# cgisky1980/Qwen3-TTS-Rust

Measured on AMD Instinct MI355X. Metric: audio_sec_per_s, higher is better.
Workload: dtype bf16

## Files before the change

### include/q3tts.h

```cpp
#ifndef Q3TTS_H
#define Q3TTS_H

#include <stdint.h>

#ifdef __cplusplus
extern "C" {
#endif

#define Q3TTS_OK 0
#define Q3TTS_ERR_INVALID (-1)
#define Q3TTS_ERR_DEVICE (-2)
#define Q3TTS_ERR_OOM (-3)
#define Q3TTS_ERR_IO (-4)
#define Q3TTS_ERR_STATE (-5)
#define Q3TTS_ERR_UNSUPPORTED (-6)
#define Q3TTS_MAX_BATCH 256

#define Q3TTS_MAX_UPSAMPLE 4
#define Q3TTS_MAX_DEC_BLOCKS 8


typedef struct q3tts_model_config {
    int32_t t_n_layer, t_d_model, t_n_head, t_n_kv_head, t_head_dim, t_d_ffn, t_vocab;
    float t_rope_theta;
// ... 229 lines not shown
int q3tts_clone_audio_encode(q3tts_engine* e, const float* audio, int64_t n_samples, int64_t* codes, int32_t cap_frames,
                             int32_t* n_frames);
int q3tts_clone_speaker_encode(q3tts_engine* e, const float* audio, int64_t n_samples, float* spk_emb);
int q3tts_k_speaker_from_mel(q3tts_engine* e, const float* mel, int32_t n_frames, float* spk_emb);
int q3tts_k_audio_latent(q3tts_engine* e, const float* audio, int64_t n_samples, float* latent, int32_t cap_frames,
                         int32_t* n_frames);

typedef struct q3tts_tokenizer q3tts_tokenizer;
int q3tts_tokenizer_load(const char* tokenizer_json_path, q3tts_tokenizer** out, char* err, int32_t err_cap);
void q3tts_tokenizer_free(q3tts_tokenizer* t);
int32_t q3tts_tokenizer_vocab_size(const q3tts_tokenizer* t);
int q3tts_tokenizer_encode(const q3tts_tokenizer* t, const char* utf8, int64_t n_bytes, uint32_t* ids, int32_t cap,
                           int32_t* n_ids, char* err, int32_t err_cap);
int q3tts_tokenizer_decode(const q3tts_tokenizer* t, const uint32_t* ids, int32_t n, char* out, int64_t cap, int64_t* n_bytes,
                           char* err, int32_t err_cap);

int q3tts_k_gemm_exact(int32_t device, const float* x, int32_t B, int32_t K, const uint16_t* w_bf16, int32_t N,
                       const float* norm_w , float eps, const float* bias ,
                       int32_t epilogue , float* y, uint64_t* argmax_keys,
                       int32_t iters, float* mean_kernel_ms);
int q3tts_k_attention(int32_t device, const float* qkv , int32_t n_rows, int32_t pos0,
                      int32_t n_head, int32_t n_kv_head, int32_t head_dim, const float* q_norm_w, const float* k_norm_w,
                      float eps, float rope_theta, const int32_t* mrope_sections, float* out );
int q3tts_k_attention_decode(int32_t device, const float* qkv, int32_t n_slots, const int32_t* lens, int32_t n_ctx, int32_t n_head,
                             int32_t n_kv_head, int32_t head_dim, const float* q_norm_w, const float* k_norm_w, float eps, float rope_theta,
                             const int32_t* mrope_sections, int32_t policy, float* out_f32, uint16_t* out_bf16);
int q3tts_k_attention_runs(int32_t device, const float* qkv, int32_t n_runs, const int32_t* run_n, const int32_t* run_pos0, int32_t n_ctx,
                           int32_t n_head, int32_t n_kv_head, int32_t head_dim, const float* q_norm_w, const float* k_norm_w, float eps,
                           float rope_theta, const int32_t* mrope_sections, int32_t policy, int32_t out_form, void* out, float* out_scale,
                           uint16_t* k_cache, uint16_t* v_cache);
int q3tts_k_attention_decode_ex(int32_t device, const float* qkv, int32_t n_slots, const int32_t* lens, int32_t n_ctx, int32_t n_head,
                                int32_t n_kv_head, int32_t head_dim, const float* q_norm_w, const float* k_norm_w, float eps,
                                float rope_theta, const int32_t* mrope_sections, int32_t policy, int32_t row_indexed, int32_t out_form,
                                void* out, float* out_scale, uint16_t* k_cache, uint16_t* v_cache);
int q3tts_k_attention_pair(int32_t device, const float* qkv, int32_t n_slots, int32_t n_ctx, int32_t n_head, int32_t n_kv_head,
                           int32_t head_dim, const float* q_norm_w, const float* k_norm_w, float eps, float rope_theta,
                           const int32_t* mrope_sections, int32_t out_form, void* out, float* out_scale, uint16_t* k_cache, uint16_t* v_cache);
int q3tts_k_attend_pick(int32_t fused, int32_t gqa_ratio, int32_t n_ctx, int32_t n_seg, int32_t seg_max_n, int32_t seg_max_t,
                        int32_t n_kv_head, int32_t* kernel);
int q3tts_k_attention_runs_kv8(int32_t device, const float* qkv, int32_t n_runs, const int32_t* run_n, const int32_t* run_pos0, int32_t n_ctx,
                               int32_t n_head, int32_t n_kv_head, int32_t head_dim, const float* q_norm_w, const float* k_norm_w, float eps,
                               float rope_theta, const int32_t* mrope_sections, int32_t policy, int32_t out_form, void* out, float* out_scale,
                               int8_t* k_q, int8_t* v_q, uint16_t* k_d, uint16_t* v_d);
int q3tts_k_attention_decode_kv8(int32_t device, const float* qkv, int32_t n_slots, const int32_t* lens, int32_t n_ctx, int32_t n_head,
                                 int32_t n_kv_head, int32_t head_dim, const float* q_norm_w, const float* k_norm_w, float eps,
                                 float rope_theta, const int32_t* mrope_sections, int32_t policy, int32_t out_form, void* out,
                                 float* out_scale, int8_t* k_q, int8_t* v_q, uint16_t* k_d, uint16_t* v_d);
int q3tts_k_attend_pick_kv8(int32_t fused, int32_t gqa_ratio, int32_t n_ctx, int32_t n_seg, int32_t seg_max_n, int32_t seg_max_t,
                            int32_t n_kv_head, int32_t* kernel);
int q3tts_k_pred_table_row(q3tts_engine* e, int32_t q, int32_t code, float* out);
typedef struct q3tts_k_pred_step {
    int32_t n_rows, q, n_codebooks, n_key_parts, rows_q, d_embed, d_proj, max_steps_cap;
    const uint64_t* keys;
    const int32_t* active;
    const int32_t* n_frames;
    const float* codec_q;
    const float* pproj_q;
    const float* proj_b;
    float* fb;
    float* px;
    int32_t* codes;
} q3tts_k_pred_step;
int q3tts_k_pred_next(int32_t device, q3tts_k_pred_step* st, const float* norm_w, uint16_t* xb, float* ssp);
int q3tts_k_attention_gather(int32_t device, q3tts_k_pred_step* st, const float* table, const float* qkv, int32_t len, int32_t n_ctx,
                             int32_t n_head, int32_t n_kv_head, int32_t head_dim, const float* q_norm_w, const float* k_norm_w, float eps,
                             float rope_theta, const int32_t* mrope_sections, int32_t out_form, void* out, float* out_scale,
                             uint16_t* k_cache, uint16_t* v_cache);
int q3tts_k_sample(int32_t device, const float* logits, int32_t n, int32_t ld, int32_t limit, float temperature,
                   int32_t top_k, float top_p, const float* r_uniform, int32_t* out_ids);
int q3tts_k_talker_prefill(q3tts_engine* e, const float* embd, int32_t n_tok, float* hidden_out, float* logits_out);
int q3tts_k_talker_prefill_prefix(q3tts_engine* e, const q3tts_prefix* prefix, const float* embd, int32_t n_tok, float* hidden_out,
                                  float* logits_out);
int q3tts_k_prefix_read(const q3tts_prefix* x, void* k, void* v, int64_t cap, int64_t* bytes);
int q3tts_k_vocoder(q3tts_engine* e, const int32_t* codes, int32_t n_frames, int32_t chunk_frames, float* pcm_out,
                    int32_t* n_samples_out);
int q3tts_k_vocoder_latent(q3tts_engine* e, const int32_t* codes, int32_t n_frames, int32_t chunk_frames, float* out);
typedef struct q3tts_voc_tap {
    char name[32];
    int32_t dtype, layout, hist_rows, rows, channels, reserved;
    uint64_t offset;
} q3tts_voc_tap;
int q3tts_k_vocoder_taps(q3tts_engine* e, const int32_t* codes, int32_t n_frames, int32_t chunk_frames, int32_t tap_call, void* buf,
                         uint64_t buf_bytes, q3tts_voc_tap* recs, int32_t rec_cap, int32_t* n_recs);
int q3tts_k_vocoder_bench(q3tts_engine* e, int32_t n_slots, int32_t chunks, float* ms_per_chunk);
int q3tts_k_gguf_read(const char* path, const char* tensor, float* out, int64_t cap, int64_t* nelem, int64_t* dims4, int32_t* ggml_type);
int q3tts_k_gguf_meta(const char* path, const char* key, int32_t* value_type, int32_t* elem_type, int64_t* count, double* values,
                      int64_t values_cap, char* str, int64_t str_cap, int64_t* str_bytes);
int q3tts_k_probe(q3tts_engine* e, int32_t enable);
int q3tts_k_mfma_bf16(int32_t device, const uint16_t* a, const uint16_t* b, const float* c, float* d, int32_t n_cases, int32_t chain);
int q3tts_k_bgemm(int32_t device, const uint16_t* xb, int32_t B, int32_t K, const uint16_t* w_bf16, int32_t N, const float* ssp, int32_t ntiles,
                  int32_t d_norm, float eps, int32_t epilogue, const float* nw_next, float* y, uint16_t* yb, float* ssp_out, uint64_t* keys,
                  int32_t iters, float* mean_kernel_ms);
int q3tts_k_bgemm_policy(int32_t big);
int q3tts_k_attend_policy(int32_t decode, int32_t prefill);
int q3tts_k_pred_variant(q3tts_engine* e, int32_t force);
int q3tts_k_text_ready(int32_t n_text, int32_t closed, int32_t n_frames);
int q3tts_k_credit_ready(int64_t credit, int32_t n_frames);
int q3tts_k_request_rules(const q3tts_request* r, int32_t keep, int32_t keep_rows, char* msg, int32_t cap);
int q3tts_k_swap_arena(int64_t cap, const int64_t* ops, int32_t n, int64_t* offsets);
int q3tts_k_swap_phase_ms(const q3tts_session* s, double out[3]);
int q3tts_k_bgemm_pick(int32_t B, int32_t K, int32_t N, int32_t epilogue, int32_t w_once, int32_t q8, int32_t* out5);
int q3tts_k_bgemm_q8(int32_t device, const uint16_t* xb, int32_t B, int32_t K, const int8_t* q, const uint16_t* d_f16, int32_t N, const float* ssp,
                     int32_t ntiles, int32_t d_norm, float eps, int32_t epilogue, const float* nw_next, float* y, uint16_t* yb, float* ssp_out,
                     uint64_t* keys, int32_t iters, float* mean_kernel_ms);
int q3tts_k_bgemm_q8a8(int32_t device, const int8_t* aq, const float* ad, int32_t B, int32_t K, const int8_t* q, const uint16_t* d_f16, int32_t N,
                       const float* ssp, int32_t ntiles, int32_t d_norm, float eps, int32_t epilogue, const float* nw_next, float* y, int8_t* yq,
                       float* yd, float* ssp_out, int32_t iters, float* mean_kernel_ms);
int q3tts_k_bgemm_q8a8_argmax(int32_t device, const int8_t* aq, const float* ad, int32_t B, int32_t K, const int8_t* q, const uint16_t* d_f16, int32_t N,
                              const float* ssp, int32_t ntiles, int32_t d_norm, float eps, int32_t* ids_out);
int q3tts_k_bgemm_voc(int32_t device, const uint16_t* xb, int32_t B, int32_t K, const uint16_t* w_bf16, int32_t N, int32_t epilogue, const float* bias,
                      int32_t bias_n, const float* col_scale, int32_t seg_rows, int32_t gap_rows, float* y, uint16_t* yb, int32_t want_yb);
int q3tts_k_project(int32_t device, const float* x, int32_t rows, int32_t n_in, const float* w, const float* bias, int32_t n_out, const float* nw,
                    float* y, uint16_t* xb, float* ssp);
int q3tts_k_norm_inputs(int32_t device, const float* x, int32_t rows, int32_t d, const float* nw, uint16_t* xb, float* ssp);
int q3tts_k_alloc_upload(q3tts_engine* e, int64_t bytes, int64_t* mismatches);
int q3tts_k_pcm_pack(int32_t device, const float* src, int32_t rows, int64_t stride, const int32_t* ent_row, const int32_t* ent_first,
                     const int32_t* ent_count, const int64_t* ent_dst, int32_t n_ent, int32_t format, void* out, int64_t out_n);
int q3tts_k_resample_table(int32_t rate_in, int32_t rate_out, int32_t* L, int32_t* M, int32_t* H, float* tab, int64_t cap, int64_t* n);
int q3tts_k_pcm_resample(int32_t device, const float* src, int32_t rows, int64_t stride, const int32_t* row_len, const int32_t* row_final,
                         const int32_t* ent_row, const int32_t* ent_first, const int32_t* ent_count, const int64_t* ent_dst, int32_t n_ent,
                         int32_t rate_in, int32_t rate_out, int32_t format, void* out, int64_t out_n, int32_t iters, float* mean_ms);
int q3tts_k_tempo_counts(int64_t n, int32_t permille, int64_t* N, int64_t* D);
int q3tts_k_pcm_tempo(int32_t device, const float* src, int32_t rows, int64_t stride, const int32_t* lens, int32_t n_steps, const int32_t* row_final,
                      int32_t permille, float* out, int64_t out_stride, int32_t* n_valid, int32_t* delta, int64_t delta_stride, int32_t iters, float* mean_ms);
int q3tts_k_row_buckets(int32_t max_batch, int32_t* out, int32_t cap);
int q3tts_k_bucket_steps(const q3tts_engine* e, int64_t* out, int32_t cap);
int q3tts_k_prefix_stats(const q3tts_engine* e, int64_t* out2);
int q3tts_k_engine_footprint(const q3tts_engine_config* cfg, int64_t* bytes);
int q3tts_k_device_bytes(const q3tts_engine* e, int64_t* bytes);
int q3tts_k_rng_f32(uint64_t seed, int32_t n, float* out);

#define Q3TTS_BREAK_END 0
#define Q3TTS_BREAK_HARD 1
#define Q3TTS_BREAK_CLAUSE 2
#define Q3TTS_BREAK_SENTENCE 3
#define Q3TTS_BREAK_PARAGRAPH 4
typedef struct q3tts_text_span { int64_t begin, end; int32_t kind; } q3tts_text_span;
int q3tts_text_split(const char* utf8, int64_t n_bytes, int32_t target_bytes , int32_t max_bytes ,
                     q3tts_text_span* spans, int32_t cap, int32_t* n_spans, char* err, int32_t err_cap);

typedef struct q3tts_join_opts {
    int32_t trim;
    float threshold;
    int32_t keep;
    int32_t fade;
    int32_t pause_ms[5];
} q3tts_join_opts;

typedef struct q3tts_long_segment { const uint32_t* ids; int32_t n_ids; int32_t kind; int32_t max_steps ; } q3tts_long_segment;
typedef struct q3tts_long_opts { q3tts_join_opts join; int32_t speed_permille ; int32_t output_rate ; } q3tts_long_opts;
typedef struct q3tts_long_info {
    int32_t status, n_frames, hit_eos; int64_t n_native, lo, hi;
    int64_t begin, end;
    int64_t out_begin, out_end;
} q3tts_long_info;
typedef struct q3tts_long_result { int32_t status, n_segments, n_truncated , sample_rate; int64_t n_samples; float* pcm ;
    q3tts_long_info* info; float generate_ms, join_ms, total_ms; } q3tts_long_result;
void q3tts_long_default_opts(q3tts_long_opts*);
int q3tts_generate_long(q3tts_engine* e, const q3tts_request* tmpl, const q3tts_prompt_desc* voice, const q3tts_prefix* prefix,
                        const q3tts_long_segment* segs, int32_t n_segs, const q3tts_long_opts* opts, q3tts_long_result* out);
void q3tts_long_result_free(q3tts_long_result*);
int q3tts_pcm_join(q3tts_engine* e, const float* const* clips, const int64_t* n, const int32_t* kinds, int32_t n_clips,
                   const q3tts_join_opts* opts, float* out, int64_t cap, int64_t* n_out, int64_t* edges );
int q3tts_k_pcm_edges(int32_t device, const float* src, int32_t rows, int64_t stride, const int32_t* lens, float threshold, int32_t* edges,
                      int32_t iters, float* mean_ms);
int q3tts_k_pcm_join(int32_t device, const float* src, int32_t rows, int64_t stride, const int32_t* lens, const int32_t* kinds, const int32_t* edges,
// ... 7 lines not shown
```

### qwen3-tts-rust_amd/csrc/q3_vocoder.hip

```cpp
#include <algorithm>
#include <cmath>
#include <map>
#include <set>
#include <tuple>
#include <vector>

#include "q3_engine.h"

typedef __bf16 bf16x8 __attribute__((ext_vector_type(8)));

#define VOC_MAX_NS 64
#define VOC_FCAP 4

enum { VC_CODEBOOK = 0, VC_PRE = 32, VC_TFM = 40, VC_FINAL_NORM = 60, VC_UP = 64, VC_DEC_IN = 72, VC_BLK = 80, VC_OUT = 120 };
enum { VW_W = 0, VW_B = 1, VW_IN_NORM = 2, VW_Q = 3, VW_K = 4, VW_V = 5, VW_O = 6, VW_LS_ATTN = 7, VW_POST_NORM = 8, VW_GATE = 9,
       VW_UP = 10, VW_DOWN = 11, VW_LS_MLP = 12, VW_DW_W = 13, VW_DW_B = 14, VW_LN_W = 15, VW_LN_B = 16, VW_PW1 = 17, VW_PW1_B = 18,
       VW_PW2 = 19, VW_PW2_B = 20, VW_GAMMA = 21, VW_ALPHA = 22, VW_BETA = 23, VW_W2 = 24, VW_B2 = 25, VW_ALPHA2 = 26, VW_BETA2 = 27 };
#define VTID(l, w) Q3_TID(Q3G_VOC, l, w)

struct VCall {
    int ns, nf;
    int slot[VOC_MAX_NS];
    int pos[VOC_MAX_NS];
};

struct VConv { int ntap = 1, dil = 1, cin = 0, nout = 0, bias_n = 0; uint16_t* w = nullptr; float* b = nullptr; };
struct VRows { float* p = nullptr; size_t stride = 0; int off = 0; int bf16 = 0;
               VRows as_bf16() const { return {p, stride, off, 1}; } };
struct VBuf { float* p = nullptr; float* hist = nullptr; int H = 0, C = 0, Tcap = 0; int bf16 = 0;
              size_t stride() const { return (size_t)(H + Tcap) * C; }
              VRows rows() const { return {p, stride(), H * C, bf16}; }
              static VRows flat(float* q, int T, int C) { return {q, (size_t)T * C, 0, 0}; } };

struct VLayer { float *in_norm, *post_norm, *ls_attn, *ls_mlp; VConv q, k, v, o, gate, up, down;
                uint4 *qkv_t = nullptr, *o_t = nullptr, *gu_t = nullptr, *down_t = nullptr;
                VConv qkv, gu; };
struct VUp { VConv ct, pw1, pw2; float *dw_w, *dw_b, *ln_w, *ln_b, *gamma; int r; VBuf dw_in;
             uint4 *ct_t = nullptr, *pw1_t = nullptr, *pw2_t = nullptr; };
struct VRes { float *ea, *ib, *ea2, *ib2; VConv c1, c2; VBuf c1_in; };
struct VBlk { float *ea, *ib; VConv ct; VRes res[3]; int r, cin, cout; VBuf ct_in; };

struct VLaunch {
    bool polite = false;
    bool no_ring = false, no_tap = false, no_fuse = false;
    bool out_old = false, attn_old = false;
    long tap_min = 128;
    auto tie() const { return std::tie(polite, no_ring, no_tap, tap_min, no_fuse, out_old, attn_old); }
    bool operator<(const VLaunch& o) const { return tie() < o.tie(); }
};
typedef std::tuple<int, int, VLaunch> VCallKey;
static size_t voc_lds_floor(const VLaunch& vl, size_t lds) { return vl.polite ? std::max(lds, (size_t)81 * 1024) : lds; }

struct VTapSink { uint8_t* buf = nullptr; size_t cap = 0, used = 0; q3tts_voc_tap* recs = nullptr; int rec_cap = 0, n = 0; bool overflow = false; };

struct Q3Voc {
    q3tts_vocoder_config c;
    VTapSink* taps = nullptr;
    int spf = 1, B = 0, RW = 0;
    std::vector<float*> cb; const float** cb_dev = nullptr;
    VConv pre; VBuf pre_in;
    std::vector<VLayer> L; float* final_norm = nullptr;
    std::vector<VUp> U;
    VConv dec_in; VBuf dec_in_in;
    std::vector<VBlk> Bk;
    float *oea = nullptr, *oib = nullptr, *out_w = nullptr, *out_b = nullptr; VBuf out_in; int out_c = 0;
    float *kring = nullptr, *vring = nullptr;
    float* rope = nullptr; int rope_rows = 0;
    struct ZeroEnt { char* base; unsigned long long bytes; };
    ZeroEnt* zero_tab = nullptr; int n_zero = 0;
    bool tfm_bg = false;
    bool up_bg = false; uint16_t* upb = nullptr;
    float *x = nullptr, *xn = nullptr, *xnb = nullptr, *qkv = nullptr, *att = nullptr, *g = nullptr;
    float *t1 = nullptr, *t2 = nullptr;
    float* pcm = nullptr; size_t pcm_stride = 0;
    std::vector<int> frames_done, last_flag;
    VCall* call_dev = nullptr;
    VCall* call_host = nullptr; hipEvent_t call_ev[16] = {}; unsigned call_i = 0;
    std::map<VCallKey, hipGraphExec_t> call_graphs;
    std::set<VCallKey> call_seen;
    std::vector<void*> allocs;
};

enum VEpi { VEPI_STORE = 0, VEPI_SCALE_ADD = 1, VEPI_ADD = 2, VEPI_GELU = 3, VEPI_SWIGLU = 4 };
struct VGemm {
    const float* x; size_t x_stride; int x_off;
    int T, M;
    VConv c;
    float* y; size_t y_stride; int y_off;
    const float* scale;
    int scale_n;
    int epi;
    int store;
    int a_bf16;
    int y_bf16;
    float* y2; size_t y2_stride; int y2_off;
    const float *ea, *ib; int snake_n;
    int y2_bf16;
    int chunked;
};
__device__ __forceinline__ void vstep(const VGemm& g, int step, int kpt, int& tap, int& k0) {
    if (g.chunked) { const int ch = step / g.c.ntap; tap = step - ch * g.c.ntap; k0 = ch << 5; }
    else { tap = step / kpt; k0 = (step - tap * kpt) << 5; }
}

__device__ __forceinline__ float gelu_erf(float x) { return 0.5f * x * (1.0f + erff(x * 0.70710678118654752f)); }

__device__ __forceinline__ void vepi(const VGemm& g, float v, int s, int t, int n, float yold) {
    const int nout = g.c.nout;
    if (g.c.b) v += g.c.b[n % g.c.bias_n];
    float* yp = g.y + (size_t)s * g.y_stride + g.y_off + (size_t)t * nout + n;
    if (g.epi == 1) v = yold + g.scale[n % g.scale_n] * v;
    else if (g.epi == 2) v = yold + v;
    else if (g.epi == 3) v = gelu_erf(v);
    if (g.store) *yp = v;
    if (g.y2) {
        const int c = n % g.snake_n;
        const float sn = __sinf(v * g.ea[c]);
        const float sv = v + g.ib[c] * (sn * sn);
        const size_t o2 = (size_t)s * g.y2_stride + g.y2_off + (size_t)t * nout + n;
        if (g.y2_bf16) ((__bf16*)g.y2)[o2] = (__bf16)sv; else g.y2[o2] = sv;
    }
}

#define VS_PF 8
template <int NJ, bool ABF>
__global__ __launch_bounds__(256) void k_vgemm_small(VGemm g) {
    const int wave = threadIdx.x >> 6, lane = threadIdx.x & 63;
    const int m0 = blockIdx.y * 64 + wave * 16, n0 = blockIdx.x * (NJ * 16);
    if (m0 >= g.M) return;
    const int lr = lane & 15, kq = lane >> 4;
    const int cin = g.c.cin, nout = g.c.nout, kpt = cin >> 5, steps = g.c.ntap * kpt;
    const float* xrow; const uint16_t* xrow16;
    {
        int m = m0 + lr; if (m >= g.M) m = g.M - 1;
        const int s = m / g.T, t = m - s * g.T;
        const size_t eo = (size_t)s * g.x_stride + g.x_off + (size_t)t * cin + kq * 8;
        xrow = g.x + eo; xrow16 = (const uint16_t*)g.x + eo;
    }
    const uint16_t* wrow[NJ];
#pragma unroll
    for (int j = 0; j < NJ; ++j) { int n = n0 + j * 16 + lr; if (n >= nout) n = nout - 1; wrow[j] = g.c.w + (size_t)n * cin + kq * 8; }
    float4 ra[VS_PF][ABF ? 1 : 2]; uint4 rb[VS_PF][NJ];
    f32x4 acc[NJ];
#pragma unroll
    for (int j = 0; j < NJ; ++j) acc[j] = (f32x4){0.f, 0.f, 0.f, 0.f};
#define VS_ISSUE(slot_, step_)                                                                        \
    do {                                                                                              \
        const int st__ = min((step_), steps - 1);                                                     \
        int tap__, k0__; vstep(g, st__, kpt, tap__, k0__);                                            \
        const long sh__ = (long)(g.c.ntap - 1 - tap__) * g.c.dil * cin - k0__;                          \
        if (ABF) ra[slot_][0] = *(const float4*)(xrow16 - sh__);                                      \
        else { ra[slot_][0] = *(const float4*)(xrow - sh__); ra[slot_][ABF ? 0 : 1] = *(const float4*)(xrow - sh__ + 4); } \
        const size_t wo__ = (size_t)tap__ * nout * cin + k0__;                                        \
        _Pragma("unroll") for (int jj__ = 0; jj__ < NJ; ++jj__) rb[slot_][jj__] = *(const uint4*)(wrow[jj__] + wo__); \
    } while (0)
#pragma unroll
    for (int j = 0; j < VS_PF; ++j) VS_ISSUE(j, j);
    __builtin_amdgcn_sched_barrier(0);
    for (int s0 = 0; s0 < steps; s0 += VS_PF) {
#pragma unroll
        for (int j = 0; j < VS_PF; ++j) {
            const int step = s0 + j;
            const float live = step < steps ? 1.0f : 0.0f;
            bf16x8 a;
            if (ABF) {
                float4 v0 = ra[j][0];
                if (step >= steps) v0 = make_float4(0.f, 0.f, 0.f, 0.f);
                a = *(const bf16x8*)&v0;
            } else {
                const float4 v0 = ra[j][0], v1 = ra[j][ABF ? 0 : 1];
                a[0] = (__bf16)(v0.x * live); a[1] = (__bf16)(v0.y * live); a[2] = (__bf16)(v0.z * live); a[3] = (__bf16)(v0.w * live);
                a[4] = (__bf16)(v1.x * live); a[5] = (__bf16)(v1.y * live); a[6] = (__bf16)(v1.z * live); a[7] = (__bf16)(v1.w * live);
            }
            bf16x8 bfr[NJ];
#pragma unroll
            for (int jj = 0; jj < NJ; ++jj) { const uint4 u = rb[j][jj]; bfr[jj] = *(const bf16x8*)&u; }
            __builtin_amdgcn_sched_barrier(0);
            VS_ISSUE(j, step + VS_PF);
            __builtin_amdgcn_sched_barrier(0);
#pragma unroll
            for (int jj = 0; jj < NJ; ++jj) acc[jj] = __builtin_amdgcn_mfma_f32_16x16x32_bf16(a, bfr[jj], acc[jj], 0, 0, 0);
        }
    }
#undef VS_ISSUE
#pragma unroll
    for (int e = 0; e < 4; ++e) {
        const int m = m0 + 4 * kq + e;
        if (m >= g.M) continue;
        const int s = m / g.T, t = m - s * g.T;
        if (NJ == 2 && g.epi == 4) {
            const int n = blockIdx.x * 16 + lr;
            if (n0 + 16 + lr < nout) {
                const float gt = acc[0][e], up = acc[NJ - 1][e];
                const float sv = (gt / (1.0f + expf(-gt))) * up;
                const size_t yo = (size_t)s * g.y_stride + g.y_off + (size_t)t * (nout >> 1) + n;
                if (g.y_bf16) ((__bf16*)g.y)[yo] = (__bf16)sv; else g.y[yo] = sv;
            }
        } else {
#pragma unroll
            for (int j = 0; j < NJ; ++j) {
                const int n = n0 + j * 16 + lr;
// ... 78 lines not shown
    __syncthreads();
    for (int step = 0; step < steps; step += 2) {
        sstore(R0, 1);
        gload(R0, step + 3);
        VT_COMPUTE(0);
        Q3_LDS_BARRIER();
        sstore(R1, 0);
        gload(R1, step + 4);
        VT_COMPUTE(1);
        Q3_LDS_BARRIER();
    }
    const bool rmw = g.epi == 1 || g.epi == 2;
#pragma unroll
    for (int i = 0; i < 4; ++i) {
        float yv[4][NJ];
        if (rmw) {
#pragma unroll
            for (int e = 0; e < 4; ++e) {
                const int m = min(m0 + wm * 64 + i * 16 + 4 * kq + e, g.M - 1);
                const int s = m / g.T, t = m - s * g.T;
                const float* yp = g.y + (size_t)s * g.y_stride + g.y_off + (size_t)t * nout;
#pragma unroll
                for (int j = 0; j < NJ; ++j) yv[e][j] = yp[min(n0 + wn * NJ * 16 + j * 16 + lr, nout - 1)];
            }
        }
#pragma unroll
        for (int e = 0; e < 4; ++e) {
            const int m = m0 + wm * 64 + i * 16 + 4 * kq + e;
            if (m >= g.M) continue;
            const int s = m / g.T, t = m - s * g.T;
#pragma unroll
            for (int j = 0; j < NJ; ++j) {
                const int n = n0 + wn * NJ * 16 + j * 16 + lr;
                if (n < nout) vepi(g, acc[i][j][e], s, t, n, rmw ? yv[e][j] : 0.0f);
            }
        }
    }
}

template <int BN, int ROWS, int NTHR, bool LITE>
__device__ __forceinline__ void vepi_tile(const VGemm& g, const float* Ot, const int* rinfo, int n0) {
    constexpr int LDO = BN + 4, C4 = BN / 4, RPP = NTHR / C4, PER = (ROWS + RPP - 1) / RPP, PB = 8;
    const int tid = threadIdx.x, cg = tid % C4, r0 = tid / C4, nout = g.c.nout, n = n0 + cg * 4;
    const bool act = r0 < RPP && n < nout;
    const int epi = g.epi;
    const bool rmw = epi == 2 || (!LITE && epi == 1), has_b = g.c.b != nullptr, has_y2 = g.y2 != nullptr;
    float b4[4], sc4[4], ea4[4], ib4[4];
    {
        const int nc = min(n, nout - 4);
        auto base = [&](int P) { return P >= nout ? nc : nc % P; };
        auto at = [&](const float* p, int P, int b0, int q) { return (P & 3) == 0 ? p[b0 + q] : p[(nc + q) % P]; };
        const int bb = has_b ? base(g.c.bias_n) : 0, bs = (!LITE && epi == 1) ? base(g.scale_n) : 0, bk = has_y2 ? base(g.snake_n) : 0;
#pragma unroll
        for (int q = 0; q < 4; ++q) {
            b4[q] = has_b ? at(g.c.b, g.c.bias_n, bb, q) : 0.0f;
            sc4[q] = (!LITE && epi == 1) ? at(g.scale, g.scale_n, bs, q) : 1.0f;
            ea4[q] = has_y2 ? at(g.ea, g.snake_n, bk, q) : 0.0f;
            ib4[q] = has_y2 ? at(g.ib, g.snake_n, bk, q) : 0.0f;
        }
    }
    const float* ybase = g.y + g.y_off + n;
    for (int u0 = 0; u0 < PER; u0 += PB) {
        float4 yo[PB]; int info[PB];
#pragma unroll
        for (int u = 0; u < PB; ++u) {
            const int row = r0 + (u0 + u) * RPP;
            info[u] = (act && u0 + u < PER && row < ROWS) ? rinfo[row] : -1;
            if (rmw && info[u] >= 0) yo[u] = *(const float4*)(ybase + (size_t)(info[u] >> 20) * g.y_stride + (size_t)(info[u] & 0xFFFFF) * nout);
        }
#pragma unroll
        for (int u = 0; u < PB; ++u) {
            if (info[u] < 0) continue;
            const int row = r0 + (u0 + u) * RPP, sl = info[u] >> 20, t = info[u] & 0xFFFFF;
            const float4 a4 = *(const float4*)&Ot[(size_t)row * LDO + cg * 4];
            float v[4] = {a4.x, a4.y, a4.z, a4.w};
            const float yv[4] = {rmw ? yo[u].x : 0.f, rmw ? yo[u].y : 0.f, rmw ? yo[u].z : 0.f, rmw ? yo[u].w : 0.f};
            float sv[4];
#pragma unroll
            for (int q = 0; q < 4; ++q) {
                if (has_b) v[q] += b4[q];
                if (!LITE && epi == 1) v[q] = yv[q] + sc4[q] * v[q];
                else if (epi == 2) v[q] = yv[q] + v[q];
                else if (!LITE && epi == 3) v[q] = gelu_erf(v[q]);
                if (has_y2) {
                    const float sn = __sinf(v[q] * ea4[q]);
                    sv[q] = v[q] + ib4[q] * (sn * sn);
                }
            }
            if (g.store) *(float4*)(g.y + g.y_off + n + (size_t)sl * g.y_stride + (size_t)t * nout) = make_float4(v[0], v[1], v[2], v[3]);
            if (has_y2) {
                const size_t o2 = (size_t)sl * g.y2_stride + g.y2_off + (size_t)t * nout + n;
                if (g.y2_bf16) {
                    __bf16 hh[4] = {(__bf16)sv[0], (__bf16)sv[1], (__bf16)sv[2], (__bf16)sv[3]};
                    *(uint2*)((__bf16*)g.y2 + o2) = *(const uint2*)hh;
                } else *(float4*)(g.y2 + o2) = make_float4(sv[0], sv[1], sv[2], sv[3]);
            }
        }
    }
}

#ifdef Q3_VOC_STAMPS
__device__ unsigned long long g_ring_stamps[4][8];
#define VG_STAMP(i_) do { if (NJ == 3 && vg_wg >= 0 && threadIdx.x == 0) g_ring_stamps[vg_wg][i_] = __builtin_amdgcn_s_memrealtime(); } while (0)
#else
#define VG_STAMP(i_) do { } while (0)
#endif
template <int NJ, int VR_NS>
__global__ __launch_bounds__(256) void k_vgemm_ring(VGemm g) {
#ifdef Q3_VOC_STAMPS
    const int vg_wg = blockIdx.x == 1 && blockIdx.y == 100 ? 0 : (blockIdx.x == 0 && blockIdx.y == 700 ? 1 : (blockIdx.x == 2 && blockIdx.y == 1200 ? 2 : -1));
#endif
    VG_STAMP(0);
    constexpr int BN = NJ * 32, LA = 2, LB = (BN / 16 + 3) / 4, L = LA + LB;
    constexpr int STAGE = (128 + BN) * 64;
    extern __shared__ __attribute__((aligned(16))) char ring[];
    const int tid = threadIdx.x, wave = tid >> 6, lane = tid & 63;
    const int wm = wave >> 1, wn = wave & 1, lr = lane & 15, kq = lane >> 4;
    int bx = blockIdx.x, by = blockIdx.y;
    {
        const int total = gridDim.x * gridDim.y;
        if ((total & 7) == 0) {
            const int id = blockIdx.x + gridDim.x * blockIdx.y, t = (id & 7) * (total >> 3) + (id >> 3);
            bx = t % gridDim.x; by = t / gridDim.x;
        }
    }
    const int m0 = by * 128, n0 = bx * BN;
    const int cin = g.c.cin, nout = g.c.nout, kpt = cin >> 5, steps = g.c.ntap * kpt;
    const int lrow = lane >> 2;
    const uint16_t* arow[LA]; int achunk[LA];
#pragma unroll
    for (int i = 0; i < LA; ++i) {
        const int row = (wave * LA + i) * 16 + lrow;
        int m = m0 + row; if (m >= g.M) m = g.M - 1;
        const int s = m / g.T, t = m - s * g.T;
        achunk[i] = ((lane & 3) ^ VR_SW(row)) * 8;
        arow[i] = (const uint16_t*)g.x + (size_t)s * g.x_stride + g.x_off + (size_t)t * cin + achunk[i];
    }
    const uint16_t* brow[LB]; int bgrp[LB];
#pragma unroll
    for (int i = 0; i < LB; ++i) {
        bgrp[i] = min(wave * LB + i, BN / 16 - 1);
        const int row = bgrp[i] * 16 + lrow;
        int n = n0 + row; if (n >= nout) n = nout - 1;
        brow[i] = g.c.w + (size_t)n * cin + ((lane & 3) ^ VR_SW(row)) * 8;
    }
    auto issue = [&](int step) {
        int tap, k0; vstep(g, step, kpt, tap, k0);
        const long sh = (long)(g.c.ntap - 1 - tap) * g.c.dil * cin - k0;
        char* st = ring + (size_t)(step % VR_NS) * STAGE;
#pragma unroll
        for (int i = 0; i < LA; ++i)
            __builtin_amdgcn_global_load_lds((const __attribute__((address_space(1))) void*)(arow[i] - sh),
                                             (__attribute__((address_space(3))) void*)(st + (wave * LA + i) * 1024), 16, 0, 0);
        const size_t wo = (size_t)tap * nout * cin + k0;
#pragma unroll
        for (int i = 0; i < LB; ++i)
            __builtin_amdgcn_global_load_lds((const __attribute__((address_space(1))) void*)(brow[i] + wo),
                                             (__attribute__((address_space(3))) void*)(st + 128 * 64 + bgrp[i] * 1024), 16, 0, 0);
    };
    f32x4 acc[4][NJ];
#pragma unroll
    for (int i = 0; i < 4; ++i)
#pragma unroll
        for (int j = 0; j < NJ; ++j) acc[i][j] = (f32x4){0.f, 0.f, 0.f, 0.f};
    int aoff[4], boff[NJ];
#pragma unroll
    for (int i = 0; i < 4; ++i) { const int R = wm * 64 + i * 16 + lr; aoff[i] = R * 64 + ((kq ^ VR_SW(R)) << 4); }
#pragma unroll
    for (int j = 0; j < NJ; ++j) { const int R = wn * NJ * 16 + j * 16 + lr; boff[j] = 128 * 64 + R * 64 + ((kq ^ VR_SW(R)) << 4); }
#pragma unroll
// ... 105 lines not shown
        const int st = min(step, steps - 1), ch = st / NTAP, tap = st - ch * NTAP;
#pragma unroll
        for (int h = 0; h < BP; ++h)
            __builtin_amdgcn_global_load_lds((const __attribute__((address_space(1))) void*)(bp[h] + (size_t)tap * nout * cin + ch * 32),
                                             (__attribute__((address_space(3))) void*)(Bring + (step % NS) * (BN * 64) + (wave * BP + h) * 16 * 64), 16, 0, 0);
    };
    f32x4 acc[4][4];
#pragma unroll
    for (int i = 0; i < 4; ++i)
#pragma unroll
        for (int j = 0; j < 4; ++j) acc[i][j] = (f32x4){0.f, 0.f, 0.f, 0.f};
    const int arow0 = sub * RA + wm * 64 + lr;
    int boff[4];
#pragma unroll
    for (int j = 0; j < 4; ++j) { const int R = wn * 64 + j * 16 + lr; boff[j] = R * 64 + ((kq ^ ((R >> 1) & 3)) << 4); }
    issue_a(0);
#pragma unroll
    for (int p = 0; p < LA; ++p) { issue_b(2 * p); issue_b(2 * p + 1); }
    for (int c0 = 0; c0 < nchunk; c0 += 2) {
#pragma unroll
        for (int j = 0; j < 7; ++j) {
            if (j == 0) vc_waitcnt<vc_wait(0, LA, BP)>();
            else if (j == 1) vc_waitcnt<vc_wait(1, LA, BP)>();
            else if (j == 2) vc_waitcnt<vc_wait(2, LA, BP)>();
            else if (j == 3) vc_waitcnt<vc_wait(3, LA, BP)>();
            else if (j == 4) vc_waitcnt<vc_wait(4, LA, BP)>();
            else if (j == 5) vc_waitcnt<vc_wait(5, LA, BP)>();
            else vc_waitcnt<vc_wait(6, LA, BP)>();
            Q3_LDS_BARRIER();
            const int s0 = c0 * NTAP + 2 * j;
            if (j == 0) issue_a(c0 + 1);
            if (j == 4) issue_a(c0 + 2);
            issue_b(s0 + 2 * LA); issue_b(s0 + 2 * LA + 1);
#pragma unroll
            for (int h = 0; h < 2; ++h) {
                const int sl = 2 * j + h, cc = sl >= NTAP ? 1 : 0, tap = sl - cc * NTAP;
                const char* img = tlds + cc * abytes;
                const char* st = Bring + ((s0 + h) % NS) * (BN * 64);
                bf16x8 a_[4], b_[4];
#pragma unroll
                for (int i = 0; i < 4; ++i) { const int R = arow0 + i * 16 + tap * dil; a_[i] = *(const bf16x8*)(img + R * 64 + ((kq ^ ((R >> 1) & 3)) << 4)); }
#pragma unroll
                for (int jj = 0; jj < 4; ++jj) b_[jj] = *(const bf16x8*)(st + boff[jj]);
#pragma unroll
                for (int i = 0; i < 4; ++i)
#pragma unroll
                    for (int jj = 0; jj < 4; ++jj) acc[i][jj] = __builtin_amdgcn_mfma_f32_16x16x32_bf16(a_[i], b_[jj], acc[i][jj], 0, 0, 0);
            }
        }
    }
    asm volatile("s_waitcnt vmcnt(0)" ::: "memory");
    constexpr int LDO = BN + 4, ROWS = 128 * NSUB;
    float* Ot = (float*)tlds;
    __syncthreads();
#pragma unroll
    for (int i = 0; i < 4; ++i)
#pragma unroll
        for (int j = 0; j < 4; ++j)
#pragma unroll
            for (int e = 0; e < 4; ++e) Ot[(size_t)(sub * 128 + wm * 64 + i * 16 + 4 * kq + e) * LDO + wn * 64 + j * 16 + lr] = acc[i][j][e];
    int* rinfo = (int*)(Ot + ROWS * LDO);
    if (tid < ROWS) {
        const int q = by * NSUB + (tid >> 7), sl = q / tps, t = ((q - sl * tps) << 7) + (tid & 127);
        rinfo[tid] = (q < nsub && t < g.T) ? (sl << 20) | t : -1;
    }
    __syncthreads();
    if (g.epi == 0 || g.epi == 2) vepi_tile<BN, ROWS, 64 * NW, true>(g, Ot, rinfo, n0);
    else vepi_tile<BN, ROWS, 64 * NW, false>(g, Ot, rinfo, n0);
}
template <int NSUB>
static void launch_vconv_tap(const VLaunch& vl, hipStream_t s, const VGemm& g) {
    constexpr int NS = NSUB == 2 ? 12 : 8;
    const int halo = (g.c.ntap - 1) * g.c.dil, RA = (128 + halo + 15) & ~15;
    const size_t lds_main = (size_t)2 * NSUB * RA * 64 + (size_t)NS * 128 * 64, lds_out = (size_t)128 * NSUB * (128 + 4) * 4 + 128 * NSUB * 4;
    const size_t lds = voc_lds_floor(vl, std::max(lds_main, lds_out));
    static Q3PerDevice pd;
    pd.ensure(1, []() { hipFuncSetAttribute((const void*)k_vconv_tap<7, NSUB>, hipFuncAttributeMaxDynamicSharedMemorySize, 160 * 1024 - 1024); });
    const int tps = (g.T + 127) / 128, nsub = (g.M / g.T) * tps;
    hipLaunchKernelGGL((k_vconv_tap<7, NSUB>), dim3(g.c.nout / 128, (nsub + NSUB - 1) / NSUB), dim3(256 * NSUB), lds, s, g);
}

struct VResUnit {
    const float* xin; size_t xin_stride;
    int T, dil;
    const uint16_t *w1, *w2; const float *b1, *b2;
    const float *ea2, *ib2;
    float* o; size_t o_stride; int store_o;
    float* y2; size_t y2_stride; int y2_off; const float *ea3, *ib3;
};
#if defined(Q3_STAMPS) || defined(Q3_VOC_STAMPS)
__device__ unsigned long long g_voc_stamps[2][4][16];
#define VR_STAMP(i_) do { if (stamp_wg >= 0 && threadIdx.x == 0) g_voc_stamps[NT == 12 ? 0 : 1][stamp_wg][i_] = __builtin_amdgcn_s_memrealtime(); } while (0)
#else
#define VR_STAMP(i_) do { } while (0)
#endif
#define VR_BARRIER() __syncthreads()
template <int NT, int MT, int NWV>
__global__ __launch_bounds__(64 * NWV) void k_voc_resunit(VResUnit g) {
#if defined(Q3_STAMPS) || defined(Q3_VOC_STAMPS)
    const int stamp_wg = (blockIdx.y == 5 && (blockIdx.x == 3 || blockIdx.x == 20)) ? (blockIdx.x == 3 ? 0 : 1) : ((blockIdx.y == 40 && blockIdx.x == 11) ? 2 : -1);
#endif
    VR_STAMP(0);
    constexpr int C = NT * 16, KS = C / 32, R = 64 * MT, LDA = C + 16, S1 = 7 * KS, S = 8 * KS;
    constexpr int NTHR = 64 * NWV, BROWS = NTHR / 4, BPASS = (C + BROWS - 1) / BROWS;
    extern __shared__ __attribute__((aligned(16))) __bf16 lds[];
    const int halo = 6 * g.dil;
    __bf16* At = lds;
    __bf16* Zt = lds;
    __bf16* Bs = At + (size_t)(R + halo) * LDA;
    const int tid = threadIdx.x, wave = tid >> 6, lane = tid & 63, lr = lane & 15, kq = lane >> 4;
    const int sidx = blockIdx.y, t0 = blockIdx.x * R, T = g.T;
    const int bn = tid >> 2, bpart = tid & 3;
#define VR_DECL(X_) uint4 X_##0, X_##1, X_##2; X_##0 = X_##1 = X_##2 = make_uint4(0, 0, 0, 0)
    VR_DECL(ra); VR_DECL(rb); VR_DECL(rc); VR_DECL(rd);
#define VR_GLOADB(X_, step_)                                                                                            \
    do {                                                                                                                \
        const int st__ = min((step_), S - 1);                                                                           \
        const uint16_t* base__ = (st__ < S1 ? g.w1 + (size_t)(st__ / KS) * C * C + (st__ % KS) * 32 : g.w2 + (st__ - S1) * 32) + bpart * 8; \
        X_##0 = *(const uint4*)(base__ + (size_t)min(bn, C - 1) * C);                                                    \
        if (BPASS > 1) X_##1 = *(const uint4*)(base__ + (size_t)min(bn + BROWS, C - 1) * C);                                \
        if (BPASS > 2) X_##2 = *(const uint4*)(base__ + (size_t)min(bn + 2 * BROWS, C - 1) * C);                               \
    } while (0)
#define VR_SSTOREB(X_, buf_)                                                                                            \
    do {                                                                                                                \
        __bf16* d__ = &Bs[((size_t)(buf_) * C + bn) * 32 + ((bpart ^ VR_SW(bn)) << 3)];       \
        if (bn < C) *(uint4*)d__ = X_##0;                                                                               \
        if (BPASS > 1 && bn + BROWS < C) *(uint4*)(d__ + BROWS * 32) = X_##1;                                                 \
        if (BPASS > 2 && bn + 2 * BROWS < C) *(uint4*)(d__ + 2 * BROWS * 32) = X_##2;                                               \
    } while (0)
    VR_GLOADB(ra, 0);
    VR_STAMP(1);
    {
        const uint16_t* xp = (const uint16_t*)g.xin + (size_t)sidx * g.xin_stride + (size_t)t0 * C;
        const int nrow = R + halo, c8 = C / 8, total = nrow * c8;
        for (int base = tid; base < total; base += 12 * NTHR) {
            uint4 v[12];
#pragma unroll
            for (int u = 0; u < 12; ++u) {
                const int i = min(base + u * NTHR, total - 1), r = i / c8, c = (i - r * c8) * 8;
                v[u] = *(const uint4*)(xp + (size_t)min(r, T + halo - 1 - t0) * C + c);
            }
#pragma unroll
            for (int u = 0; u < 12; ++u) {
                const int i = base + u * NTHR;
                if (i < total) {
                    const int r = i / c8, c = (i - r * c8) * 8;
                    const bool live = t0 + r < T + halo;
                    *(uint4*)(At + (size_t)r * LDA + c) = live ? v[u] : make_uint4(0, 0, 0, 0);
                }
            }
        }
    }
    VR_SSTOREB(ra, 0);
    constexpr int LK = BPASS > 2 ? 3 : 4;
    VR_GLOADB(rb, 1); VR_GLOADB(rc, 2);
    if (LK == 4) { VR_GLOADB(rd, 3); VR_GLOADB(ra, 4); } else { VR_GLOADB(ra, 3); }
    __syncthreads();
    VR_STAMP(2);
    constexpr int WN = ((MT == 1 || NWV == 8) && NT >= 8) ? 2 : 1, MTW = (R / 16) / (NWV / WN), NTW = NT / WN;
    f32x4 acc[MTW][NTW];
#pragma unroll
    for (int i = 0; i < MTW; ++i)
#pragma unroll
        for (int j = 0; j < NTW; ++j) acc[i][j] = (f32x4){0.f, 0.f, 0.f, 0.f};
    const int wrow0 = (wave / WN) * MTW * 16, ncol0 = (wave % WN) * NTW * 16;
#define VR_BETWEEN()                                                                                                    \
    do {                                                                                                                \
        _Pragma("unroll") for (int i = 0; i < MTW; ++i)                                                                  \
            _Pragma("unroll") for (int j = 0; j < NTW; ++j) {                                                            \
                const int n = ncol0 + j * 16 + lr;                                                                      \
                const float bb = g.b1[n], ea = g.ea2[n], ib = g.ib2[n];                                                 \
                _Pragma("unroll") for (int e = 0; e < 4; ++e) {                                                         \
                    const float v = acc[i][j][e] + bb;                                                                  \
                    const float sn = __sinf(v * ea);                                                                    \
                    Zt[(size_t)(wrow0 + i * 16 + 4 * kq + e) * LDA + n] = (__bf16)(v + ib * (sn * sn));                 \
                    acc[i][j][e] = 0.0f;                                                                                \
                }                                                                                                       \
            }                                                                                                           \
        VR_BARRIER();                                                                                                \
    } while (0)
#define VR_STEP(step_, X_)                                                    \
    do {                                                                                                                \
        const int sp__ = (step_), buf__ = sp__ & 1, tap__ = sp__ / KS, koff__ = (sp__ - tap__ * KS) * 32;               \
        const int rowoff__ = sp__ < S1 ? tap__ * g.dil : 0;      \
        bf16x8 a__[MTW], b__[NTW];                                                                                      \
        _Pragma("unroll") for (int i = 0; i < MTW; ++i)                                                                  \
            a__[i] = *(const bf16x8*)&At[(size_t)(wrow0 + i * 16 + lr + rowoff__) * LDA + koff__ + kq * 8];             \
        _Pragma("unroll") for (int j = 0; j < NTW; ++j)                                                                  \
            b__[j] = *(const bf16x8*)&Bs[((size_t)buf__ * C + ncol0 + j * 16 + lr) * 32 + ((kq ^ VR_SW(lr)) << 3)];     \
        _Pragma("unroll") for (int i = 0; i < MTW; ++i)                                                                  \
            _Pragma("unroll") for (int j = 0; j < NTW; ++j)                                                              \
                acc[i][j] = __builtin_amdgcn_mfma_f32_16x16x32_bf16(a__[i], b__[j], acc[i][j], 0, 0, 0);                \
        VR_SSTOREB(X_, buf__ ^ 1);                                                                                      \
        VR_GLOADB(X_, sp__ + 1 + LK);                                                                                        \
        VR_BARRIER();                                                                                                \
    } while (0)
    static_assert(S % LK == 0, "the step loop is unrolled by the number of register sets");
    for (int step0 = 0; step0 < S; step0 += LK) {
#define VR_SUB(u_, X_)                                                                                                  \
        if ((S1 % LK) == (u_) && step0 + (u_) == S1) {                                                                  \
            VR_STAMP(3); VR_BETWEEN(); VR_STAMP(4);                                                                     \
        }                                                                                                               \
        VR_STEP(step0 + (u_), X_)
        if (LK == 4) { VR_SUB(0, rb); VR_SUB(1, rc); VR_SUB(2, rd); VR_SUB(3, ra); }
        else { VR_SUB(0, rb); VR_SUB(1, rc); VR_SUB(2, ra); }
    }
#undef VR_SUB
#undef VR_BETWEEN
    VR_STAMP(5);
#undef VR_STEP
#undef VR_GLOADB
#undef VR_SSTOREB
#undef VR_DECL
    constexpr int LDO = C + 4;
    float* Ot = (float*)lds;
#pragma unroll
    for (int i = 0; i < MTW; ++i)
#pragma unroll
        for (int j = 0; j < NTW; ++j) {
            const int n = ncol0 + j * 16 + lr;
            const float bb = g.b2[n];
#pragma unroll
            for (int e = 0; e < 4; ++e) Ot[(size_t)(wrow0 + i * 16 + 4 * kq + e) * LDO + n] = acc[i][j][e] + bb;
        }
    __syncthreads();
    {
        constexpr int c4n = C / 4, RPP = NTHR / c4n, PER = (R + RPP - 1) / RPP;
        float* ob = g.o + (size_t)sidx * g.o_stride;
        __bf16* yb = (__bf16*)g.y2 + (size_t)sidx * g.y2_stride + g.y2_off;
        const int cg = tid % c4n, r0 = tid / c4n, c = cg * 4;
        const bool act = r0 < RPP;
        const float4 ea = *(const float4*)(g.ea3 + c), ib = *(const float4*)(g.ib3 + c);
        constexpr int PB = PER < 13 ? PER : 13;
        for (int p0 = 0; p0 < PER; p0 += PB) {
            float4 ov[PB];
#pragma unroll
            for (int u = 0; u < PB; ++u) {
                const int row = min(r0 + (p0 + u) * RPP, R - 1);
                ov[u] = *(const float4*)(ob + (size_t)min(t0 + row, T - 1) * C + c);
            }
#pragma unroll
            for (int u = 0; u < PB; ++u) {
                const int row = r0 + (p0 + u) * RPP, t = t0 + row;
                if (!act || p0 + u >= PER || row >= R || t >= T) continue;
                const float4 a = *(const float4*)&Ot[(size_t)row * LDO + c];
                float4 v; v.x = ov[u].x + a.x; v.y = ov[u].y + a.y; v.z = ov[u].z + a.z; v.w = ov[u].w + a.w;
                if (g.store_o) *(float4*)(ob + (size_t)t * C + c) = v;
                float sn; __bf16 h[4];
                sn = __sinf(v.x * ea.x); h[0] = (__bf16)(v.x + ib.x * (sn * sn));
                sn = __sinf(v.y * ea.y); h[1] = (__bf16)(v.y + ib.y * (sn * sn));
                sn = __sinf(v.z * ea.z); h[2] = (__bf16)(v.z + ib.z * (sn * sn));
                sn = __sinf(v.w * ea.w); h[3] = (__bf16)(v.w + ib.w * (sn * sn));
                *(uint2*)(yb + (size_t)t * C + c) = *(const uint2*)h;
            }
        }
    }
    VR_STAMP(6);
}

__global__ void k_voc_embed(const VCall* __restrict__ clp, const int* codes, int max_steps_cap, int ncb_model, const float* const* cb, int ncb, int cbs, int cd,
                            float* out, size_t out_stride, int out_off) {
    const VCall& cl = *clp;
    const int s = blockIdx.y, t = blockIdx.x;
    const int slot = cl.slot[s], frame = min(cl.pos[s] + t, max_steps_cap - 1);
    const int* cp = codes + ((size_t)slot * max_steps_cap + frame) * ncb_model;
    constexpr int QB = 16;
    for (int q0 = 0; q0 < ncb; q0 += QB) {
        const float* row[QB];
#pragma unroll
        for (int u = 0; u < QB; ++u) {
            const int q = min(q0 + u, ncb - 1);
            int code = cp[q];
            code = code < 0 ? 0 : (code >= cbs ? cbs - 1 : code);
            row[u] = cb[q] + (size_t)code * cd;
        }
        for (int i = threadIdx.x; i < cd; i += blockDim.x) {
            float v[QB];
#pragma unroll
            for (int u = 0; u < QB; ++u) v[u] = row[u][i];
            float* op = out + (size_t)s * out_stride + out_off + (size_t)t * cd + i;
            float acc = q0 ? *op : 0.0f;
#pragma unroll
            for (int u = 0; u < QB; ++u) if (q0 + u < ncb) acc += v[u];
            *op = acc;
        }
    }
}

__global__ void k_voc_rows_bf16(const float* src, size_t src_stride, uint16_t* dst, size_t dst_stride, int n) {
    const int s = blockIdx.y, i = (blockIdx.x * blockDim.x + threadIdx.x) * 4;
    if (i >= n) return;
    const float4 v = *(const float4*)(src + (size_t)s * src_stride + i);
    __bf16 h[4] = {(__bf16)v.x, (__bf16)v.y, (__bf16)v.z, (__bf16)v.w};
    *(uint2*)(dst + (size_t)s * dst_stride + i) = *(const uint2*)h;
}

template <class E>
__global__ void k_voc_hist(const VCall* __restrict__ clp, E* work, size_t stride, E* hist, int H, int C, int T, int save) {
    const VCall& cl = *clp;
    const int s = blockIdx.y, slot = cl.slot[s];
    const size_t n = (size_t)H * C;
    E* w = work + (size_t)s * stride + (save ? (size_t)T * C : 0);
    E* h = hist + (size_t)slot * n;
    for (size_t i = (size_t)blockIdx.x * blockDim.x + threadIdx.x; i < n; i += (size_t)gridDim.x * blockDim.x) {
        if (save) h[i] = w[i]; else w[i] = h[i];
    }
}

struct VHistTab {
    int n;
    struct Ent { char* work; char* hist; unsigned long long stride_b, block_b, tail_b; } e[24];
};
__global__ void k_voc_hist_all(const VCall* __restrict__ clp, VHistTab tab, int save) {
    const VCall& cl = *clp;
    const VHistTab::Ent z = tab.e[blockIdx.z];
    const int s = blockIdx.y, slot = cl.slot[s];
    uint32_t* w = (uint32_t*)(z.work + (size_t)s * z.stride_b + (save ? z.tail_b : 0));
    uint32_t* h = (uint32_t*)(z.hist + (size_t)slot * z.block_b);
    const size_t n = z.block_b / 4;
    for (size_t i = (size_t)blockIdx.x * blockDim.x + threadIdx.x; i < n; i += (size_t)gridDim.x * blockDim.x) {
        if (save) h[i] = w[i]; else w[i] = h[i];
    }
}

__global__ __launch_bounds__(64) void k_voc_rmsnorm(const float* x, const float* w, float eps, int d, float* y, int out_bf16) {
    const int r = blockIdx.x, lane = threadIdx.x;
    const float* xr = x + (size_t)r * d;
    float ss = 0.0f;
    for (int i0 = lane; i0 < d; i0 += 8 * 64) {
        float v[8];
#pragma unroll
        for (int u = 0; u < 8; ++u) v[u] = xr[min(i0 + u * 64, d - 1)];
#pragma unroll
        for (int u = 0; u < 8; ++u) if (i0 + u * 64 < d) ss += v[u] * v[u];
    }
#pragma unroll
    for (int m = 32; m >= 1; m >>= 1) ss += __shfl_xor(ss, m);
    const float rinv = 1.0f / sqrtf(ss / (float)d + eps);
    for (int i0 = lane; i0 < d; i0 += 8 * 64) {
        float v[8], wv[8];
#pragma unroll
        for (int u = 0; u < 8; ++u) { const int i = min(i0 + u * 64, d - 1); v[u] = xr[i]; wv[u] = w[i]; }
#pragma unroll
        for (int u = 0; u < 8; ++u)
            if (i0 + u * 64 < d) {
                const float o = (v[u] * rinv) * wv[u];
                if (out_bf16 == 2) ((__bf16*)y)[q3_atile_off(r, i0 + u * 64, d >> 5)] = (__bf16)o;
                else if (out_bf16) ((__bf16*)y)[(size_t)r * d + i0 + u * 64] = (__bf16)o;
                else y[(size_t)r * d + i0 + u * 64] = o;
            }
    }
}

__global__ __launch_bounds__(64 * VOC_FCAP) void k_voc_attn(const VCall* __restrict__ clp, const float* qkv, float* kring, float* vring, const float* rope,
                                                            int H, int hd, int RW, int W, float* att, int tiled) {
    __shared__ float sc_s[VOC_FCAP][512];
    __shared__ float qs_s[VOC_FCAP][128];
    const VCall& cl = *clp;
    const int s = blockIdx.y, h = blockIdx.x, t = threadIdx.x >> 6, lane = threadIdx.x & 63, HH = H * hd, half = hd >> 1;
    const int slot = cl.slot[s], T = cl.nf;
    float* kr = kring + (size_t)slot * RW * HH + h * hd;
    float* vr = vring + (size_t)slot * RW * HH + h * hd;
    float* sc = sc_s[t]; float* qs = qs_s[t];
    const float scale = 1.0f / sqrtf((float)hd);
    const int pos = cl.pos[s] + t, m = s * T + t;
    {
        const float* qp = qkv + (size_t)m * 3 * HH + h * hd;
        const float* kp0 = qp + HH; const float* vp = qp + 2 * HH;
        if (lane < half) {
            const float2 csn = ((const float2*)rope)[(size_t)pos * half + lane];
            const float cs = csn.x, sn = csn.y;
            float a = qp[lane], b = qp[lane + half];
            qs[lane] = a * cs - b * sn; qs[lane + half] = b * cs + a * sn;
            a = kp0[lane]; b = kp0[lane + half];
            float* kd = kr + (size_t)(pos % RW) * HH;
            kd[lane] = a * cs - b * sn; kd[lane + half] = b * cs + a * sn;
        }
        for (int i = lane; i < hd; i += 64) vr[(size_t)(pos % RW) * HH + i] = vp[i];
    }
    __syncthreads();
    const int j0 = pos - W + 1 > 0 ? pos - W + 1 : 0, nk = pos - j0 + 1;
    for (int j = lane; j < nk; j += 64) {
        const float4* kp = (const float4*)(kr + (size_t)((j0 + j) % RW) * HH);
        float a = 0.0f;
        for (int i0 = 0; i0 < hd; i0 += 64) {
            float4 kk[16];
#pragma unroll
            for (int u = 0; u < 16; ++u) kk[u] = kp[min(i0 / 4 + u, hd / 4 - 1)];
#pragma unroll
            for (int u = 0; u < 16; ++u)
                if (i0 + 4 * u < hd) {
                    const float* qp2 = qs + i0 + 4 * u;
                    a += qp2[0] * kk[u].x; a += qp2[1] * kk[u].y; a += qp2[2] * kk[u].z; a += qp2[3] * kk[u].w;
                }
// ... 197 lines not shown
#pragma unroll
                    for (int c = 0; c < 8; ++c) acc[o] = fmaf(xv[c], wr[tap][c], acc[o]);
                }
            }
        }
#pragma unroll
        for (int o = 0; o < 8; ++o) part[k * R + g * 8 + o] = acc[o];
    }
    __syncthreads();
    if (tid < R && t0 + tid < T) {
        float r = 0.0f;
        for (int kk = 0; kk < NS; ++kk) r += part[kk * R + tid];
        r += b[0];
        pcm[(size_t)slot * pcm_stride + (size_t)cl.pos[s] * spf + t0 + tid] = fminf(1.0f, fmaxf(-1.0f, r));
    }
}

template <class T>
static int valloc(q3tts_engine* e, Q3Voc* v, T** p, size_t n) {
    void* q = nullptr;
    const int rc = q3_dev_alloc_zeroed(e, &q, n * sizeof(T) + 256);
    if (rc != Q3TTS_OK) return rc;
    v->allocs.push_back(q);
    *p = (T*)q;
    return Q3TTS_OK;
}
#define VTRY(x) do { int rc__ = (x); if (rc__ != Q3TTS_OK) return rc__; } while (0)

static int gen_vec(q3tts_engine* e, Q3Voc* v, float** p, uint32_t tid, size_t n, float base, float std) {
    VTRY(valloc(e, v, p, n));
    q3_launch_fill_f32(*p, n, e->cfg.synth_seed, tid, base, std / Q3_IH4_STD, 0, e->stream);
    return Q3TTS_OK;
}
__global__ void k_fill_bf16(uint16_t* dst, size_t n, uint64_t seed, uint32_t tid, float scale) {
    for (size_t i = (size_t)blockIdx.x * blockDim.x + threadIdx.x; i < n; i += (size_t)gridDim.x * blockDim.x)
        dst[i] = q3_bf16(q3_synth(seed, tid, i, scale));
}
static int gen_conv(q3tts_engine* e, Q3Voc* v, VConv* c, int comp, int ww, int wb, int ntap, int dil, int cin, int nout, int bias_n, float gain) {
    c->ntap = ntap; c->dil = dil; c->cin = cin; c->nout = nout; c->bias_n = bias_n;
    const size_t n = (size_t)ntap * nout * cin;
    VTRY(valloc(e, v, &c->w, n));
    const float scale = (gain / sqrtf((float)(ntap * cin))) / Q3_IH4_STD;
    hipLaunchKernelGGL(k_fill_bf16, dim3((unsigned)std::min<size_t>((n + 255) / 256, 65536)), dim3(256), 0, e->stream, c->w, n,
                       e->cfg.synth_seed, VTID(comp, ww), scale);
    c->b = nullptr;
    if (bias_n) VTRY(gen_vec(e, v, &c->b, VTID(comp, wb), bias_n, 0.0f, 0.02f));
    return Q3TTS_OK;
}
static int gen_snake(q3tts_engine* e, Q3Voc* v, uint32_t ta, uint32_t tb, int C, float** ea, float** ib) {
    std::vector<float> a(C), b(C);
    const float scale = 0.1f / Q3_IH4_STD;
    for (int i = 0; i < C; ++i) {
        const float al = 0.0f + q3_synth(e->cfg.synth_seed, ta, i, scale), be = 0.0f + q3_synth(e->cfg.synth_seed, tb, i, scale);
        a[i] = (float)exp((double)al); b[i] = (float)(1.0 / (exp((double)be) + 1e-9));
    }
    VTRY(valloc(e, v, ea, (size_t)C)); VTRY(valloc(e, v, ib, (size_t)C));
    Q3_HIP(e, hipMemcpy(*ea, a.data(), (size_t)C * 4, hipMemcpyHostToDevice));
    Q3_HIP(e, hipMemcpy(*ib, b.data(), (size_t)C * 4, hipMemcpyHostToDevice));
    return Q3TTS_OK;
}
static int mk_buf(q3tts_engine* e, Q3Voc* v, VBuf* b, int H, int C, int Tcap, int bf16 = 0) {
    b->H = H; b->C = C; b->Tcap = Tcap; b->bf16 = bf16;
    VTRY(valloc(e, v, &b->p, (size_t)VOC_MAX_NS * b->stride()));
    VTRY(valloc(e, v, &b->hist, (size_t)v->B * std::max(1, H) * C));
    return Q3TTS_OK;
}

int q3_voc_samples_per_frame(const q3tts_engine* e) { return e->voc ? e->voc->spf : 0; }

int q3_voc_create(q3tts_engine* e) {
    const q3tts_vocoder_config& c = e->cfg.vocoder;
#define REQ(cond) do { if (!(cond)) return q3_set_err(e, Q3TTS_ERR_INVALID, "vocoder config check failed: " #cond); } while (0)
    REQ(c.n_codebooks >= 1 && c.n_codebooks <= 16 && c.n_codebooks <= e->cfg.model.n_codebooks);
    REQ(c.codebook_dim % 32 == 0 && c.latent_dim % 32 == 0 && c.d_ffn % 32 == 0 && (c.n_head * c.head_dim) % 32 == 0);
    REQ(c.d_ffn % 16 == 0);
    REQ(c.head_dim <= 128 && c.head_dim % 4 == 0 && c.sliding_window >= 1 && c.sliding_window + VOC_FCAP <= 512);
    REQ(c.n_upsample >= 0 && c.n_upsample <= Q3TTS_MAX_UPSAMPLE && c.n_dec_blocks >= 1 && c.n_dec_blocks <= Q3TTS_MAX_DEC_BLOCKS);
    REQ(c.pre_conv_kernel >= 1 && c.lookahead_frames >= 0);
    { int ch = c.decoder_dim; for (int b = 0; b < c.n_dec_blocks; ++b) { REQ(ch % 64 == 0); ch /= 2; } REQ(ch >= 1); }
#undef REQ
    Q3Voc* v = new Q3Voc();
    e->voc = v;
    v->c = c; v->B = e->B;
    const int d = c.latent_dim, HH = c.n_head * c.head_dim;
    v->RW = c.sliding_window + VOC_FCAP;
    v->cb.resize(c.n_codebooks);
    for (int q = 0; q < c.n_codebooks; ++q) {
        VTRY(valloc(e, v, &v->cb[q], (size_t)c.codebook_size * c.codebook_dim));
        q3_launch_fill_f32(v->cb[q], (size_t)c.codebook_size * c.codebook_dim, e->cfg.synth_seed, VTID(VC_CODEBOOK + q, VW_W), 0.0f,
                           (1.0f / sqrtf(16.0f)) / Q3_IH4_STD, 1, e->stream);
    }
    { float** cd = nullptr; VTRY(valloc(e, v, &cd, (size_t)16)); v->cb_dev = (const float**)cd;
      Q3_HIP(e, hipMemcpy((void*)cd, v->cb.data(), sizeof(float*) * c.n_codebooks, hipMemcpyHostToDevice)); }
    VTRY(gen_conv(e, v, &v->pre, VC_PRE, VW_W, VW_B, c.pre_conv_kernel, 1, c.codebook_dim, d, d, 1.0f));
    VTRY(mk_buf(e, v, &v->pre_in, c.pre_conv_kernel - 1, c.codebook_dim, VOC_FCAP));
    v->L.resize(c.n_layer);
    for (int l = 0; l < c.n_layer; ++l) {
        VLayer& y = v->L[l]; const int comp = VC_TFM + l;
        VTRY(gen_vec(e, v, &y.in_norm, VTID(comp, VW_IN_NORM), d, 1.0f, 0.05f));
        VTRY(gen_vec(e, v, &y.post_norm, VTID(comp, VW_POST_NORM), d, 1.0f, 0.05f));
        VTRY(gen_vec(e, v, &y.ls_attn, VTID(comp, VW_LS_ATTN), d, c.layer_scale_init, 0.1f * c.layer_scale_init));
        VTRY(gen_vec(e, v, &y.ls_mlp, VTID(comp, VW_LS_MLP), d, c.layer_scale_init, 0.1f * c.layer_scale_init));
        VTRY(gen_conv(e, v, &y.q, comp, VW_Q, 0, 1, 1, d, HH, 0, 1.0f)); VTRY(gen_conv(e, v, &y.k, comp, VW_K, 0, 1, 1, d, HH, 0, 1.0f));
        VTRY(gen_conv(e, v, &y.v, comp, VW_V, 0, 1, 1, d, HH, 0, 1.0f)); VTRY(gen_conv(e, v, &y.o, comp, VW_O, 0, 1, 1, HH, d, 0, 1.0f));
        VTRY(gen_conv(e, v, &y.gate, comp, VW_GATE, 0, 1, 1, d, c.d_ffn, 0, 1.0f)); VTRY(gen_conv(e, v, &y.up, comp, VW_UP, 0, 1, 1, d, c.d_ffn, 0, 1.0f));
        VTRY(gen_conv(e, v, &y.down, comp, VW_DOWN, 0, 1, 1, c.d_ffn, d, 0, 1.0f));
        y.qkv = y.q; y.qkv.nout = 3 * HH;
        VTRY(valloc(e, v, &y.qkv.w, (size_t)3 * HH * d));
        Q3_HIP(e, hipMemcpyAsync(y.qkv.w, y.q.w, (size_t)HH * d * 2, hipMemcpyDeviceToDevice, e->stream));
        Q3_HIP(e, hipMemcpyAsync(y.qkv.w + (size_t)HH * d, y.k.w, (size_t)HH * d * 2, hipMemcpyDeviceToDevice, e->stream));
        Q3_HIP(e, hipMemcpyAsync(y.qkv.w + (size_t)2 * HH * d, y.v.w, (size_t)HH * d * 2, hipMemcpyDeviceToDevice, e->stream));
        y.gu = y.gate; y.gu.nout = 2 * c.d_ffn;
        VTRY(valloc(e, v, &y.gu.w, (size_t)2 * c.d_ffn * d));
        Q3_HIP(e, hipMemcpy2DAsync(y.gu.w, (size_t)32 * d * 2, y.gate.w, (size_t)16 * d * 2, (size_t)16 * d * 2, c.d_ffn / 16, hipMemcpyDeviceToDevice, e->stream));
        Q3_HIP(e, hipMemcpy2DAsync(y.gu.w + (size_t)16 * d, (size_t)32 * d * 2, y.up.w, (size_t)16 * d * 2, (size_t)16 * d * 2, c.d_ffn / 16, hipMemcpyDeviceToDevice, e->stream));
    }
    v->tfm_bg = d % 256 == 0 && HH % 256 == 0 && c.d_ffn % 256 == 0 && (3 * HH) % 16 == 0 && c.d_ffn % 32 == 0;
    if (v->tfm_bg)
        for (int l = 0; l < c.n_layer; ++l) {
            VLayer& y = v->L[l];
            VTRY(valloc(e, v, &y.qkv_t, (size_t)3 * HH * d / 8)); VTRY(valloc(e, v, &y.o_t, (size_t)d * HH / 8));
            VTRY(valloc(e, v, &y.gu_t, (size_t)2 * c.d_ffn * d / 8)); VTRY(valloc(e, v, &y.down_t, (size_t)d * c.d_ffn / 8));
            Q3Fill f{};
            f.mode = 0; f.row0 = 0;
            f.dst = y.qkv_t; f.N = 3 * HH; f.K = d; f.rows = 3 * HH; f.src_a = y.qkv.w; q3_launch_fill_tiled(f, e->stream);
            f.dst = y.o_t; f.N = d; f.K = HH; f.rows = d; f.src_a = y.o.w; q3_launch_fill_tiled(f, e->stream);
            f.dst = y.down_t; f.N = d; f.K = c.d_ffn; f.rows = d; f.src_a = y.down.w; q3_launch_fill_tiled(f, e->stream);
            f.mode = 1; f.dst = y.gu_t; f.N = 2 * c.d_ffn; f.K = d; f.src_a = y.gate.w; f.src_b = y.up.w; q3_launch_fill_tiled(f, e->stream);
        }
    {
        v->rope_rows = e->cfg.max_steps_cap + VOC_FCAP;
        const int half = c.head_dim / 2;
        std::vector<float> tab((size_t)v->rope_rows * half * 2);
        for (int i = 0; i < half; ++i) {
            const double inv = pow((double)c.rope_theta, -2.0 * (double)i / (double)c.head_dim);
            for (int p = 0; p < v->rope_rows; ++p) {
                const double ang = (double)p * inv;
                tab[((size_t)p * half + i) * 2] = (float)cos(ang); tab[((size_t)p * half + i) * 2 + 1] = (float)sin(ang);
            }
        }
        VTRY(valloc(e, v, &v->rope, tab.size()));
        Q3_HIP(e, hipMemcpy(v->rope, tab.data(), tab.size() * 4, hipMemcpyHostToDevice));
    }
    VTRY(gen_vec(e, v, &v->final_norm, VTID(VC_FINAL_NORM, VW_W), d, 1.0f, 0.05f));
    int rows = VOC_FCAP;
    v->spf = 1;
    v->U.resize(c.n_upsample);
    for (int s = 0; s < c.n_upsample; ++s) {
        VUp& p = v->U[s]; const int comp = VC_UP + s, r = c.upsample_ratios[s]; p.r = r; v->spf *= r;
        VTRY(gen_conv(e, v, &p.ct, comp, VW_W, VW_B, 1, 1, d, r * d, d, 1.0f));
        rows *= r;
        VTRY(mk_buf(e, v, &p.dw_in, 6, d, rows));
        VTRY(gen_vec(e, v, &p.dw_w, VTID(comp, VW_DW_W), (size_t)7 * d, 0.0f, 0.3f)); VTRY(gen_vec(e, v, &p.dw_b, VTID(comp, VW_DW_B), d, 0.0f, 0.02f));
        VTRY(gen_vec(e, v, &p.ln_w, VTID(comp, VW_LN_W), d, 1.0f, 0.05f)); VTRY(gen_vec(e, v, &p.ln_b, VTID(comp, VW_LN_B), d, 0.0f, 0.02f));
        VTRY(gen_conv(e, v, &p.pw1, comp, VW_PW1, VW_PW1_B, 1, 1, d, 4 * d, 4 * d, 1.0f));
        VTRY(gen_conv(e, v, &p.pw2, comp, VW_PW2, VW_PW2_B, 1, 1, 4 * d, d, d, 1.0f));
        if (d % 256 == 0) {
            v->up_bg = true;
            VTRY(valloc(e, v, &p.ct_t, (size_t)r * d * d / 8)); VTRY(valloc(e, v, &p.pw1_t, (size_t)4 * d * d / 8)); VTRY(valloc(e, v, &p.pw2_t, (size_t)4 * d * d / 8));
            Q3Fill f{}; f.mode = 0; f.row0 = 0;
            f.dst = p.ct_t; f.N = r * d; f.K = d; f.rows = r * d; f.src_a = p.ct.w; q3_launch_fill_tiled(f, e->stream);
            f.dst = p.pw1_t; f.N = 4 * d; f.K = d; f.rows = 4 * d; f.src_a = p.pw1.w; q3_launch_fill_tiled(f, e->stream);
            f.dst = p.pw2_t; f.N = d; f.K = 4 * d; f.rows = d; f.src_a = p.pw2.w; q3_launch_fill_tiled(f, e->stream);
        }
        VTRY(gen_vec(e, v, &p.gamma, VTID(comp, VW_GAMMA), d, 0.1f, 0.01f));
    }
    VTRY(gen_conv(e, v, &v->dec_in, VC_DEC_IN, VW_W, VW_B, 7, 1, d, c.decoder_dim, c.decoder_dim, 1.0f));
    VTRY(mk_buf(e, v, &v->dec_in_in, 6, d, rows, 1));
    size_t scratch = (size_t)rows * std::max(4 * d, c.decoder_dim);
    v->Bk.resize(c.n_dec_blocks);
    int ch = c.decoder_dim;
    for (int b = 0; b < c.n_dec_blocks; ++b) {
        VBlk& k = v->Bk[b]; const int comp = VC_BLK + 4 * b, r = c.dec_rates[b]; k.r = r; k.cin = ch; k.cout = ch / 2; v->spf *= r;
        VTRY(gen_snake(e, v, VTID(comp, VW_ALPHA), VTID(comp, VW_BETA), ch, &k.ea, &k.ib));
        VTRY(gen_conv(e, v, &k.ct, comp, VW_W, VW_B, 2, 1, ch, r * k.cout, k.cout, 1.0f));
        VTRY(mk_buf(e, v, &k.ct_in, 1, ch, rows, 1));
        rows *= r;
        scratch = std::max(scratch, (size_t)rows * k.cout);
        const int dil[3] = {1, 3, 9};
        for (int u = 0; u < 3; ++u) {
            VRes& s = k.res[u]; const int rc = comp + 1 + u;
            VTRY(gen_snake(e, v, VTID(rc, VW_ALPHA), VTID(rc, VW_BETA), k.cout, &s.ea, &s.ib));
            VTRY(gen_conv(e, v, &s.c1, rc, VW_W, VW_B, 7, dil[u], k.cout, k.cout, k.cout, 0.5f));
            VTRY(mk_buf(e, v, &s.c1_in, 6 * dil[u], k.cout, rows, 1));
            VTRY(gen_snake(e, v, VTID(rc, VW_ALPHA2), VTID(rc, VW_BETA2), k.cout, &s.ea2, &s.ib2));
            VTRY(gen_conv(e, v, &s.c2, rc, VW_W2, VW_B2, 1, 1, k.cout, k.cout, k.cout, 0.5f));
        }
        ch = k.cout;
    }
    v->out_c = ch;
    VTRY(gen_snake(e, v, VTID(VC_OUT, VW_ALPHA), VTID(VC_OUT, VW_BETA), ch, &v->oea, &v->oib));
    VTRY(valloc(e, v, &v->out_w, (size_t)7 * ch)); VTRY(gen_vec(e, v, &v->out_b, VTID(VC_OUT, VW_B), 1, 0.0f, 0.02f));
    q3_launch_fill_f32(v->out_w, (size_t)7 * ch, e->cfg.synth_seed, VTID(VC_OUT, VW_W), 0.0f, (0.1f / sqrtf((float)(7 * ch))) / Q3_IH4_STD, 1, e->stream);
    VTRY(mk_buf(e, v, &v->out_in, 6, ch, rows, 1));
    const size_t M = (size_t)VOC_MAX_NS * VOC_FCAP;
    VTRY(valloc(e, v, &v->x, M * d)); VTRY(valloc(e, v, &v->xn, M * d)); VTRY(valloc(e, v, &v->xnb, M * d)); VTRY(valloc(e, v, &v->qkv, M * 3 * HH));
    VTRY(valloc(e, v, &v->att, M * HH)); VTRY(valloc(e, v, &v->g, M * c.d_ffn));
    VTRY(valloc(e, v, &v->kring, (size_t)c.n_layer * v->B * v->RW * HH)); VTRY(valloc(e, v, &v->vring, (size_t)c.n_layer * v->B * v->RW * HH));
    VTRY(valloc(e, v, &v->t1, (size_t)VOC_MAX_NS * scratch)); VTRY(valloc(e, v, &v->t2, (size_t)VOC_MAX_NS * scratch));
    if (v->up_bg) { size_t rows_up = (size_t)VOC_MAX_NS * VOC_FCAP; for (auto& u : v->U) rows_up *= u.r; VTRY(valloc(e, v, &v->upb, rows_up * d)); }
    v->pcm_stride = (size_t)(e->cfg.max_steps_cap + VOC_FCAP) * v->spf;
    VTRY(valloc(e, v, &v->pcm, (size_t)v->B * v->pcm_stride));
    v->frames_done.assign(v->B, 0); v->last_flag.assign(v->B, 0);
    VTRY(valloc(e, v, &v->call_dev, 1));
    Q3_HIP(e, hipHostMalloc((void**)&v->call_host, 16 * sizeof(VCall)));
    Q3_HIP(e, hipStreamSynchronize(e->stream));
    return Q3TTS_OK;
}

void q3_voc_destroy(q3tts_engine* e) {
    Q3Voc* v = e->voc;
    if (!v) return;
    for (auto& kv : v->call_graphs) hipGraphExecDestroy(kv.second);
    for (auto& ev : v->call_ev) if (ev) hipEventDestroy(ev);
    if (v->call_host) hipHostFree(v->call_host);
    for (void* p : v->allocs) hipFree(p);
    delete v;
    e->voc = nullptr;
}

static std::vector<Q3SlotBlock> voc_hist_blocks(const Q3Voc* v) {
    std::vector<Q3SlotBlock> tab;
    auto add = [&](const VBuf& b) { if (b.H > 0) { const unsigned long long n = (unsigned long long)b.H * b.C * (b.bf16 ? 2 : 4); tab.push_back({(char*)b.hist, n, n}); } };
    add(v->pre_in);
    for (auto& u : v->U) add(u.dw_in);
    add(v->dec_in_in);
    for (auto& b : v->Bk) { add(b.ct_in); for (auto& r : b.res) add(r.c1_in); }
    add(v->out_in);
    return tab;
}
void q3_voc_slot_blocks(q3tts_engine* e, std::vector<Q3SlotBlock>& out) {
    const Q3Voc* v = e->voc;
    out = voc_hist_blocks(v);
    const unsigned long long ring = (unsigned long long)v->RW * v->c.n_head * v->c.head_dim * 4;
    for (int l = 0; l < v->c.n_layer; ++l)
        for (float* r : {v->kring, v->vring}) out.push_back({(char*)r + (unsigned long long)l * v->B * ring, ring, ring});
}
void q3_voc_host_state(q3tts_engine* e, int slot, int* frames_done, int* last_flag, bool set) {
    Q3Voc* v = e->voc;
    if (set) { v->frames_done[slot] = *frames_done; v->last_flag[slot] = *last_flag; }
    else { *frames_done = v->frames_done[slot]; *last_flag = v->last_flag[slot]; }
}

__global__ void k_voc_zero(const Q3Voc::ZeroEnt* tab, int slot) {
    const Q3Voc::ZeroEnt z = tab[blockIdx.x];
    uint32_t* p = (uint32_t*)(z.base + (size_t)slot * z.bytes);
    const size_t n = z.bytes / 4;
    for (size_t i = (size_t)blockIdx.y * blockDim.x + threadIdx.x; i < n; i += (size_t)gridDim.y * blockDim.x) p[i] = 0u;
}
int q3_voc_reset(q3tts_engine* e, int slot) {
    Q3Voc* v = e->voc;
    if (!v) return Q3TTS_OK;
    if (!v->zero_tab) {
        std::vector<Q3Voc::ZeroEnt> tab;
        for (const Q3SlotBlock& h : voc_hist_blocks(v)) tab.push_back({h.base, h.bytes});
        v->n_zero = (int)tab.size();
        VTRY(valloc(e, v, &v->zero_tab, tab.size()));
        Q3_HIP(e, hipMemcpy(v->zero_tab, tab.data(), tab.size() * sizeof(Q3Voc::ZeroEnt), hipMemcpyHostToDevice));
    }
    if (v->n_zero) hipLaunchKernelGGL(k_voc_zero, dim3(v->n_zero, 4), dim3(256), 0, e->stream, v->zero_tab, slot);
    v->frames_done[slot] = 0; v->last_flag[slot] = 0;
    q3_tempo_forget(e, slot);
    return Q3TTS_OK;
}

struct VSnake { VRows to; const float* ea = nullptr; const float* ib = nullptr; int n = 1; };
static VSnake snake_into(const VBuf& dst, const float* ea, const float* ib, int C) { return {dst.rows(), ea, ib, C}; }
struct VOpt {
    const float* scale = nullptr; int scale_n = 1;
    VSnake snake;
    int store = 1;
    VOpt& layer_scale(const float* v, int n) { scale = v; scale_n = n; return *this; }
    VOpt& snake_to(const VSnake& k) { snake = k; return *this; }
    VOpt& no_store() { store = 0; return *this; }
};
static bool vconv_chunked(const VConv& c) { return c.ntap == 7 && c.cin % 64 == 0 && c.cin >= 256; }
static bool voc_ring_ok(const VLaunch& vl, const VGemm& g) { return !vl.no_ring && g.c.nout % 4 == 0 && g.y_off % 4 == 0 && g.y_stride % 4 == 0 && g.y2_off % 4 == 0 && g.y2_stride % 4 == 0; }
template <int NJ>
static void launch_vgemm_small(hipStream_t s, const VGemm& g) {
    const dim3 grid((g.c.nout + 16 * NJ - 1) / (16 * NJ), (g.M + 63) / 64);
    if (g.a_bf16) hipLaunchKernelGGL((k_vgemm_small<NJ, true>), grid, dim3(256), 0, s, g);
    else hipLaunchKernelGGL((k_vgemm_small<NJ, false>), grid, dim3(256), 0, s, g);
}
template <int NJ>
static void launch_vgemm_tile(const VLaunch& vl, hipStream_t s, const VGemm& g) {
    const dim3 grid((g.c.nout + 32 * NJ - 1) / (32 * NJ), (g.M + 127) / 128);
    if (g.a_bf16 && voc_ring_ok(vl, g)) launch_vgemm_ring<NJ>(vl, s, g, grid);
    else if (g.a_bf16) hipLaunchKernelGGL((k_vgemm_lds<NJ, true>), grid, dim3(256), 0, s, g);
    else hipLaunchKernelGGL((k_vgemm_lds<NJ, false>), grid, dim3(256), 0, s, g);
}
static void vgemm(const VLaunch& vl, hipStream_t s, const VConv& c, const VRows& x, int ns, int T, const VRows& y, VEpi epi = VEPI_STORE, const VOpt& o = VOpt()) {
    VGemm g; g.x = x.p; g.x_stride = x.stride; g.x_off = x.off; g.T = T; g.M = ns * T; g.c = c; g.y = y.p; g.y_stride = y.stride; g.y_off = y.off;
    g.scale = o.scale; g.scale_n = o.scale_n; g.epi = epi; g.store = o.store; g.a_bf16 = x.bf16; g.y_bf16 = y.bf16;
    g.y2 = o.snake.to.p; g.y2_stride = o.snake.to.stride; g.y2_off = o.snake.to.off; g.ea = o.snake.ea; g.ib = o.snake.ib; g.snake_n = o.snake.n; g.y2_bf16 = o.snake.to.bf16;
    g.chunked = vconv_chunked(c) ? 1 : 0;
    const long tap_wgs = (long)(c.nout / 128) * ((ns * ((T + 127) / 128) + 1) / 2);
    if (g.chunked && g.a_bf16 && !vl.no_tap && voc_ring_ok(vl, g) && c.nout % 128 == 0 && 6 * c.dil <= 64 && epi != VEPI_SWIGLU &&
        ((T + 127) / 128) * 128 * 3 <= T * 4 &&
        tap_wgs >= vl.tap_min) {
        if (vl.polite) launch_vconv_tap<1>(vl, s, g); else launch_vconv_tap<2>(vl, s, g);
    } else if (g.M <= 512 || epi == VEPI_SWIGLU) {
        const long wg32 = (long)((c.nout + 31) / 32) * ((g.M + 63) / 64);
        if (epi != VEPI_SWIGLU && wg32 < 256) launch_vgemm_small<1>(s, g); else launch_vgemm_small<2>(s, g);
    } else if (c.nout % 128 != 0 && c.nout % 96 == 0) launch_vgemm_tile<3>(vl, s, g);
    else if (c.nout % 64 == 0 && (long)((c.nout + 127) / 128) * ((g.M + 127) / 128) < 192) launch_vgemm_tile<2>(vl, s, g);
    else launch_vgemm_tile<4>(vl, s, g);
}
static bool resunit_ok(const VLaunch& vl, int C) { return !vl.no_fuse && (C == 32 || C == 64 || C == 96 || C == 128 || C == 192); }
template <int NT, int MT, int NWV = 4>
static void launch_resunit_t(const VLaunch& vl, hipStream_t s, const VResUnit& g, int ns) {
    constexpr int C = NT * 16, R = 64 * MT, LDA = C + 16;
    const size_t lds = voc_lds_floor(vl, std::max(((size_t)(R + 6 * g.dil) * LDA + (size_t)2 * C * 32) * 2, (size_t)R * (C + 4) * 4));
    static Q3PerDevice pd;
    pd.ensure(1, []() { hipFuncSetAttribute((const void*)k_voc_resunit<NT, MT, NWV>, hipFuncAttributeMaxDynamicSharedMemorySize, 160 * 1024 - 1024); });
    hipLaunchKernelGGL((k_voc_resunit<NT, MT, NWV>), dim3((g.T + R - 1) / R, ns), dim3(64 * NWV), lds, s, g);
}
static void launch_resunit(const VLaunch& vl, hipStream_t s, const VRes& r, int ns, int T, int C, float* o, int store_o, const VSnake& sk) {
    VResUnit g;
    g.xin = r.c1_in.p; g.xin_stride = r.c1_in.stride(); g.T = T; g.dil = r.c1.dil;
    g.w1 = r.c1.w; g.w2 = r.c2.w; g.b1 = r.c1.b; g.b2 = r.c2.b; g.ea2 = r.ea2; g.ib2 = r.ib2;
    g.o = o; g.o_stride = (size_t)T * C; g.store_o = store_o;
    g.y2 = sk.to.p; g.y2_stride = sk.to.stride; g.y2_off = sk.to.off; g.ea3 = sk.ea; g.ib3 = sk.ib;
    switch (C) {
        case 32: launch_resunit_t<2, 4>(vl, s, g, ns); break;
        case 64: launch_resunit_t<4, 3>(vl, s, g, ns); break;
        case 96: launch_resunit_t<6, 2>(vl, s, g, ns); break;
        case 128: launch_resunit_t<8, 1>(vl, s, g, ns); break;
        default: if (vl.polite) launch_resunit_t<12, 1>(vl, s, g, ns); else launch_resunit_t<12, 2, 8>(vl, s, g, ns); break;
    }
}
static void hist(hipStream_t s, const VCall& cl, const VCall* cld, VBuf& b, int T, int save) {
    if (b.H == 0) return;
    const size_t n = (size_t)b.H * b.C;
    const dim3 grid((unsigned)std::min<size_t>((n + 255) / 256, 64), cl.ns);
    if (b.bf16) hipLaunchKernelGGL((k_voc_hist<uint16_t>), grid, dim3(256), 0, s, cld, (uint16_t*)b.p, b.stride(), (uint16_t*)b.hist, b.H, b.C, T, save);
    else hipLaunchKernelGGL((k_voc_hist<float>), grid, dim3(256), 0, s, cld, b.p, b.stride(), b.hist, b.H, b.C, T, save);
}
static void hist_all(hipStream_t s, const VCall& cl, const VCall* cld, Q3Voc* v, int nf, int save) {
    VHistTab tab; tab.n = 0;
    auto add = [&](const VBuf& b, int T, bool with_save) {
        if (b.H == 0 || (save && !with_save) || tab.n >= 24) return;
        const size_t es = b.bf16 ? 2 : 4;
        tab.e[tab.n++] = {(char*)b.p, (char*)b.hist, (unsigned long long)(b.stride() * es), (unsigned long long)((size_t)b.H * b.C * es), (unsigned long long)((size_t)T * b.C * es)};
    };
    int T = nf;
    add(v->pre_in, T, true);
    for (auto& p : v->U) { T *= p.r; add(p.dw_in, T, false); }
    add(v->dec_in_in, T, true);
    for (auto& k : v->Bk) { add(k.ct_in, T, true); T *= k.r; for (auto& r : k.res) add(r.c1_in, T, true); }
    add(v->out_in, T, true);
    if (tab.n) hipLaunchKernelGGL(k_voc_hist_all, dim3(16, cl.ns, tab.n), dim3(256), 0, s, cld, tab, save);
}
static void voc_launch_attn(const VLaunch& vl, hipStream_t s, const VCall* cld, Q3Voc* v, float* kr, float* vr, int ns, int nf, int tiled) {
    const q3tts_vocoder_config& c = v->c;
    const size_t lds = (size_t)(c.sliding_window + nf - 1) * (2 * c.head_dim + 1) * sizeof(float);
    if (!vl.attn_old && c.head_dim <= 64 && c.head_dim % 4 == 0 && lds <= 48 * 1024) {
        hipLaunchKernelGGL(k_voc_attn_lds, dim3(c.n_head, ns), dim3(64 * nf), lds, s, cld, v->qkv, kr, vr, v->rope, c.n_head, c.head_dim, v->RW, c.sliding_window, v->att, tiled);
        return;
    }
    hipLaunchKernelGGL(k_voc_attn, dim3(c.n_head, ns), dim3(64 * nf), 0, s, cld, v->qkv, kr, vr, v->rope, c.n_head, c.head_dim, v->RW, c.sliding_window, v->att, tiled);
}
enum VTapKind { VT_F32, VT_BF16, VT_BF16_TILED };
static void vtap_rows(Q3Voc* v, hipStream_t s, const void* p, VTapKind kind, int H, int T, int C, const char* fmt, int a, int b) {
    VTapSink* k = v->taps;
    if (!k || k->overflow) return;
    const int dtype = kind != VT_F32, layout = kind == VT_BF16_TILED;
    const size_t rows = layout ? (size_t)((H + T + 15) / 16) * 16 : (size_t)(H + T), bytes = rows * C * (dtype ? 2 : 4);
    if (k->n >= k->rec_cap || k->used + bytes > k->cap) { k->overflow = true; return; }
    q3tts_voc_tap& r = k->recs[k->n++];
    memset(&r, 0, sizeof(r));
    snprintf(r.name, sizeof(r.name), fmt, a, b);
    r.dtype = dtype; r.layout = layout; r.hist_rows = H; r.rows = T; r.channels = C; r.offset = k->used;
    if (hipMemcpyAsync(k->buf + k->used, p, bytes, hipMemcpyDeviceToHost, s) != hipSuccess) k->overflow = true;
    k->used += (bytes + 15) & ~(size_t)15;
}
static void vtap(Q3Voc* v, hipStream_t s, const void* p, VTapKind kind, int T, int C, const char* fmt, int a = 0, int b = 0) {
    vtap_rows(v, s, p, kind, 0, T, C, fmt, a, b);
}
static void vtap_buf(Q3Voc* v, hipStream_t s, const VBuf& b, int T, const char* fmt, int a = 0, int c = 0) {
    vtap_rows(v, s, b.p, b.bf16 ? VT_BF16 : VT_F32, b.H, T, b.C, fmt, a, c);
}
struct VBg : Q3BGemm {
    VBg(const void* a_, int rows, const uint4* w_, int K_, int N_, int epi_) : Q3BGemm{} { a = (const uint16_t*)a_; B = rows; w = w_; K = K_; N = N_; epi = epi_; }
    VBg& to(float* y_, int ldy_) { y = y_; ldy = ldy_; return *this; }
    VBg& to_slots(const VRows& r, int T, int ldy_) { y = r.p + r.off; ldy = ldy_; seg_rows = T; seg_stride = r.stride; return *this; }
    VBg& to_tiled(void* p) { yb = (uint16_t*)p; return *this; }
    VBg& bias_of(const VConv& c) { bias = c.b; bias_n = c.bias_n; return *this; }
    VBg& scaled(const float* cs) { col_scale = cs; return *this; }
};
static int vbgemm(q3tts_engine* e, hipStream_t s, const Q3BGemm& g, const char* msg) {
    return q3_launch_bgemm(g, s) ? q3_set_err(e, Q3TTS_ERR_INVALID, msg) : Q3TTS_OK;
}

static void voc_embed_pre(q3tts_engine* e, const VLaunch& vl, const VCall& cl, hipStream_t s) {
    Q3Voc* v = e->voc; const q3tts_vocoder_config& c = v->c;
    hipLaunchKernelGGL(k_voc_embed, dim3(cl.nf, cl.ns), dim3(128), 0, s, v->call_dev, e->codes, e->cfg.max_steps_cap, e->cfg.model.n_codebooks, v->cb_dev,
                       c.n_codebooks, c.codebook_size, c.codebook_dim, v->pre_in.p, v->pre_in.stride(), v->pre_in.H * v->pre_in.C);
    vgemm(vl, s, v->pre, v->pre_in.rows(), cl.ns, cl.nf, VBuf::flat(v->x, cl.nf, c.latent_dim));
}
static int voc_tfm_layer(q3tts_engine* e, const VLaunch& vl, const VCall& cl, hipStream_t s, int l) {
    Q3Voc* v = e->voc; const q3tts_vocoder_config& c = v->c; VLayer& L = v->L[l];
    const int d = c.latent_dim, HH = c.n_head * c.head_dim, M = cl.ns * cl.nf, one_slot = 1, tiled = v->tfm_bg ? 1 : 0;
    float* kr = v->kring + (size_t)l * v->B * v->RW * HH; float* vr = v->vring + (size_t)l * v->B * v->RW * HH;
    const VRows x = VBuf::flat(v->x, M, d), xnb = VBuf::flat(v->xnb, M, d).as_bf16(), att = VBuf::flat(v->att, M, HH).as_bf16();
    const VRows g = VBuf::flat(v->g, M, c.d_ffn).as_bf16();
    hipLaunchKernelGGL(k_voc_rmsnorm, dim3(M), dim3(64), 0, s, v->x, L.in_norm, c.rms_eps, d, v->xnb, tiled ? 2 : 1);
    if (tiled) VTRY(vbgemm(e, s, VBg(v->xnb, M, L.qkv_t, d, 3 * HH, Q3_EPI_STORE).to(v->qkv, 3 * HH), "vocoder: qkv GEMM shape"));
    else vgemm(vl, s, L.qkv, xnb, one_slot, M, VBuf::flat(v->qkv, M, 3 * HH));
    voc_launch_attn(vl, s, v->call_dev, v, kr, vr, cl.ns, cl.nf, tiled);
    if (tiled) VTRY(vbgemm(e, s, VBg(v->att, M, L.o_t, HH, d, Q3_EPI_RESID).to(v->x, d).scaled(L.ls_attn), "vocoder: o GEMM shape"));
    else vgemm(vl, s, L.o, att, one_slot, M, x, VEPI_SCALE_ADD, VOpt().layer_scale(L.ls_attn, d));
    hipLaunchKernelGGL(k_voc_rmsnorm, dim3(M), dim3(64), 0, s, v->x, L.post_norm, c.rms_eps, d, v->xnb, tiled ? 2 : 1);
    if (tiled) VTRY(vbgemm(e, s, VBg(v->xnb, M, L.gu_t, d, 2 * c.d_ffn, Q3_EPI_SWIGLU).to_tiled(v->g), "vocoder: gate/up GEMM shape"));
    else vgemm(vl, s, L.gu, xnb, one_slot, M, g, VEPI_SWIGLU);
    if (tiled) VTRY(vbgemm(e, s, VBg(v->g, M, L.down_t, c.d_ffn, d, Q3_EPI_RESID).to(v->x, d).scaled(L.ls_mlp), "vocoder: down GEMM shape"));
    else vgemm(vl, s, L.down, g, one_slot, M, x, VEPI_SCALE_ADD, VOpt().layer_scale(L.ls_mlp, d));
    return Q3TTS_OK;
}
static int voc_up_stage(q3tts_engine* e, const VLaunch& vl, const VCall& cl, hipStream_t s, size_t ui, VRows& cur, int& T) {
    Q3Voc* v = e->voc; VUp& p = v->U[ui];
    const int ns = cl.ns, d = v->c.latent_dim, i = (int)ui, bg = v->up_bg ? 1 : 0;
    const VTapKind kind = bg ? VT_BF16_TILED : VT_F32;
    const uint16_t* a_in = ui ? v->upb : (const uint16_t*)v->xnb;
    const VRows raw = p.dw_in.rows();
    vtap(v, s, bg ? (const void*)a_in : (const void*)(cur.p + cur.off), kind, T, d, "up%d.in", i);
    if (bg) VTRY(vbgemm(e, s, VBg(a_in, ns * T, p.ct_t, d, p.r * d, Q3_EPI_STORE).bias_of(p.ct).to_slots(raw, T, p.r * d), "vocoder: upsample ConvTranspose GEMM shape"));
    else vgemm(vl, s, p.ct, cur, ns, T, raw);
    T *= p.r;
    vtap_buf(v, s, p.dw_in, T, "up%d.raw", i);
    hipLaunchKernelGGL(k_voc_dw_ln, dim3(T, ns), dim3(64), (size_t)d * 4, s, p.dw_in.p, p.dw_in.stride(), p.dw_in.H, T, d, p.dw_w, p.dw_b, p.ln_w, p.ln_b, v->t1, bg);
    vtap(v, s, v->t1, kind, T, d, "up%d.ln", i);
    hist(s, cl, v->call_dev, p.dw_in, T, 1);
    if (bg) VTRY(vbgemm(e, s, VBg(v->t1, ns * T, p.pw1_t, d, 4 * d, Q3_EPI_GELU).bias_of(p.pw1).to_tiled(v->t2), "vocoder: pointwise-1 GEMM shape"));
    else vgemm(vl, s, p.pw1, VBuf::flat(v->t1, T, d), ns, T, VBuf::flat(v->t2, T, 4 * d), VEPI_GELU);
    vtap(v, s, v->t2, kind, T, 4 * d, "up%d.gelu", i);
    if (bg) {
        VBg r(v->t2, ns * T, p.pw2_t, 4 * d, d, Q3_EPI_RESID);
        r.bias_of(p.pw2).scaled(p.gamma).to_slots(raw, T, d).to_tiled(ui + 1 < v->U.size() ? v->upb : nullptr);
        VTRY(vbgemm(e, s, r, "vocoder: pointwise-2 GEMM shape"));
    } else vgemm(vl, s, p.pw2, VBuf::flat(v->t2, T, 4 * d), ns, T, raw, VEPI_SCALE_ADD, VOpt().layer_scale(p.gamma, d));
    vtap_buf(v, s, p.dw_in, T, "up%d.out", i);
    cur = raw;
    return Q3TTS_OK;
}
static VSnake snake_next(Q3Voc* v, size_t bi, int u) {
    VBlk& k = v->Bk[bi];
    if (u < 2) return snake_into(k.res[u + 1].c1_in, k.res[u + 1].ea, k.res[u + 1].ib, k.cout);
    if (bi + 1 < v->Bk.size()) { VBlk& nx = v->Bk[bi + 1]; return snake_into(nx.ct_in, nx.ea, nx.ib, k.cout); }
    return snake_into(v->out_in, v->oea, v->oib, k.cout);
}
static void voc_dec_blocks(q3tts_engine* e, const VLaunch& vl, const VCall& cl, hipStream_t s, const VRows& cur, int& T) {
    Q3Voc* v = e->voc;
    const int ns = cl.ns, d = v->c.latent_dim;
    hipLaunchKernelGGL(k_voc_rows_bf16, dim3((unsigned)(((size_t)T * d / 4 + 255) / 256), ns), dim3(256), 0, s, cur.p + cur.off, cur.stride,
                       (uint16_t*)v->dec_in_in.p + (size_t)v->dec_in_in.H * d, v->dec_in_in.stride(), T * d);
    int ch = v->c.decoder_dim;
    float* z = v->t1; float* o = v->t2;
    vgemm(vl, s, v->dec_in, v->dec_in_in.rows(), ns, T, VBuf::flat(z, T, ch), VEPI_STORE,
          VOpt().snake_to(snake_into(v->Bk[0].ct_in, v->Bk[0].ea, v->Bk[0].ib, ch)).no_store());
    for (size_t bi = 0; bi < v->Bk.size(); ++bi) {
        VBlk& k = v->Bk[bi]; const int b = (int)bi;
        vgemm(vl, s, k.ct, k.ct_in.rows(), ns, T, VBuf::flat(o, T * k.r, k.cout), VEPI_STORE, VOpt().snake_to(snake_into(k.res[0].c1_in, k.res[0].ea, k.res[0].ib, k.cout)));
        T *= k.r; ch = k.cout;
        vtap(v, s, o, VT_F32, T, ch, "b%d.o_ct", b);
        for (int u = 0; u < 3; ++u) {
            VRes& r = k.res[u];
            const VSnake next = snake_next(v, bi, u);
            const int store_o = u < 2 ? 1 : 0;
            if (resunit_ok(vl, ch)) launch_resunit(vl, s, r, ns, T, ch, o, store_o, next);
            else {
                const VRows zf = VBuf::flat(z, T, ch), zb = zf.as_bf16(), orows = VBuf::flat(o, T, ch);
                vgemm(vl, s, r.c1, r.c1_in.rows(), ns, T, zf, VEPI_STORE, VOpt().snake_to({zb, r.ea2, r.ib2, ch}).no_store());
                vtap(v, s, z, VT_BF16, T, ch, "b%d.r%d.z", b, u);
                VOpt opt; opt.snake = next; opt.store = store_o;
                vgemm(vl, s, r.c2, zb, ns, T, orows, VEPI_ADD, opt);
            }
            if (store_o) vtap(v, s, o, VT_F32, T, ch, "b%d.r%d.o", b, u);
        }
    }
}
static void voc_out(q3tts_engine* e, const VLaunch& vl, const VCall& cl, hipStream_t s, int T) {
    Q3Voc* v = e->voc; const VCall* cld = v->call_dev;
    const int ns = cl.ns, ch = v->out_c;
    if (ch % 8 == 0 && ch / 8 <= 32 && !vl.out_old) {
        const int NS = ch / 8, G = std::min(16, 256 / NS), R = G * 8;
        static Q3PerDevice pd8;
        pd8.ensure(1, []() { hipFuncSetAttribute((const void*)k_voc_out8, hipFuncAttributeMaxDynamicSharedMemorySize, 96 * 1024); });
        hipLaunchKernelGGL(k_voc_out8, dim3((T + R - 1) / R, ns), dim3(256), (size_t)(R + 6) * (ch * 2 + 16) + (size_t)NS * R * 4, s,   cld, (const uint16_t*)v->out_in.p,
                           v->out_in.stride(), v->out_in.H, T, ch, v->out_w, v->out_b, v->pcm, v->pcm_stride, v->spf, G);
    } else
        hipLaunchKernelGGL(k_voc_out, dim3((T + 63) / 64, ns), dim3(256), (size_t)(70 * (ch + 1) + 7 * ch) * 4, s, cld, v->out_in.p, v->out_in.stride(), v->out_in.H, T, ch, v->out_w, v->out_b,
                           v->pcm, v->pcm_stride, v->spf);
}
static int voc_call_body(q3tts_engine* e, const VLaunch& vl, const VCall& cl, hipStream_t s) {
    Q3Voc* v = e->voc;
    const q3tts_vocoder_config& c = v->c;
    const int nf = cl.nf, d = c.latent_dim, M = cl.ns * nf;
    hist_all(s, cl, v->call_dev, v, nf, 0);
    voc_embed_pre(e, vl, cl, s);
    for (int l = 0; l < c.n_layer; ++l) VTRY(voc_tfm_layer(e, vl, cl, s, l));
    hipLaunchKernelGGL(k_voc_rmsnorm, dim3(M), dim3(64), 0, s, v->x, v->final_norm, c.rms_eps, d, v->up_bg ? v->xnb : v->xn, v->up_bg ? 2 : 0);
    VRows cur = VBuf::flat(v->xn, nf, d); int T = nf;
    for (size_t ui = 0; ui < v->U.size(); ++ui) VTRY(voc_up_stage(e, vl, cl, s, ui, cur, T));
    {
        static const int exp_skip = getenv("Q3TTS_EXP_VOC_SKIP") ? atoi(getenv("Q3TTS_EXP_VOC_SKIP")) : 0;
        if (exp_skip == 2) { Q3_HIP(e, hipGetLastError()); return Q3TTS_OK; }
    }
    const int Tup = T;
    voc_dec_blocks(e, vl, cl, s, cur, T);
    voc_out(e, vl, cl, s, T);
    if (v->taps) {
        int Tb = Tup;
        vtap_buf(v, s, v->dec_in_in, Tb, "dec_in.in");
        for (size_t bi = 0; bi < v->Bk.size(); ++bi) {
            VBlk& k = v->Bk[bi];
            vtap_buf(v, s, k.ct_in, Tb, "b%d.ct_in", (int)bi);
            Tb *= k.r;
            for (int u = 0; u < 3; ++u) vtap_buf(v, s, k.res[u].c1_in, Tb, "b%d.r%d.c1_in", (int)bi, u);
        }
        vtap_buf(v, s, v->out_in, Tb, "out.in");
        vtap(v, s, v->pcm + (size_t)cl.slot[0] * v->pcm_stride + (size_t)cl.pos[0] * v->spf, VT_F32, Tb, 1, "pcm");
    }
    hist_all(s, cl, v->call_dev, v, nf, 1);
    Q3_HIP(e, hipGetLastError());
    return Q3TTS_OK;
}

static int voc_call(q3tts_engine* e, const VCall& cl, hipStream_t s, bool polite_call) {
    Q3Voc* v = e->voc;
    {
        const unsigned i = v->call_i++ & 15;
        if (v->call_ev[i]) Q3_HIP(e, hipEventSynchronize(v->call_ev[i]));
        else Q3_HIP(e, hipEventCreateWithFlags(&v->call_ev[i], hipEventDisableTiming));
        v->call_host[i] = cl;
        Q3_HIP(e, hipMemcpyAsync(v->call_dev, &v->call_host[i], sizeof(VCall), hipMemcpyHostToDevice, s));
        Q3_HIP(e, hipEventRecord(v->call_ev[i], s));
    }
    VLaunch vl;
    auto on = [](const char* name) { const char* ev = getenv(name); return ev && atoi(ev); };
    const char* pol = getenv("Q3TTS_VOC_POLITE"); const char* tmin = getenv("Q3TTS_VOC_TAP_MIN");
    vl.polite = pol ? atoi(pol) != 0 : polite_call;
    vl.no_ring = on("Q3TTS_VOC_NORING"); vl.no_tap = on("Q3TTS_VOC_NOTAP"); vl.no_fuse = on("Q3TTS_VOC_NOFUSE"); vl.attn_old = on("Q3TTS_VOC_ATTN_OLD");
    vl.tap_min = tmin ? atol(tmin) : 128;
    vl.out_old = getenv("Q3TTS_VOC_OUT_OLD") != nullptr;
    static const bool no_graph = [] { const char* ev = getenv("Q3TTS_VOC_NO_GRAPH"); return ev && atoi(ev); }();
    if (no_graph || v->taps) return voc_call_body(e, vl, cl, s);
    const VCallKey key(cl.ns, cl.nf, vl);
    auto it = v->call_graphs.find(key);
    if (it == v->call_graphs.end()) {
        if (v->call_seen.insert(key).second) return voc_call_body(e, vl, cl, s);
        hipGraph_t graph = nullptr; hipGraphExec_t exec = nullptr;
        Q3_HIP(e, hipStreamBeginCapture(s, hipStreamCaptureModeThreadLocal));
        const int rc = voc_call_body(e, vl, cl, s);
        const hipError_t er = hipStreamEndCapture(s, &graph);
        if (rc != Q3TTS_OK) { if (graph) hipGraphDestroy(graph); return rc; }
        if (er != hipSuccess || !graph) return q3_set_err(e, Q3TTS_ERR_DEVICE, std::string("vocoder call capture: ") + hipGetErrorString(er));
        const hipError_t ei = hipGraphInstantiate(&exec, graph, nullptr, nullptr, 0);
        hipGraphDestroy(graph);
        if (ei != hipSuccess) return q3_set_err(e, Q3TTS_ERR_DEVICE, std::string("vocoder call graph: ") + hipGetErrorString(ei));
        it = v->call_graphs.emplace(key, exec).first;
    }
    Q3_HIP(e, hipGraphLaunch(it->second, s));
    return Q3TTS_OK;
}

int q3_voc_decode(q3tts_engine* e, int slot, int f0, int nf, int is_last, hipStream_t s) {
    Q3Voc* v = e->voc;
    if (!v) return q3_set_err(e, Q3TTS_ERR_STATE, "engine has no vocoder");
    if (f0 != v->frames_done[slot]) return q3_set_err(e, Q3TTS_ERR_STATE, "vocoder frames must be consumed in order");
    while (nf > 0) {
        const int n = std::min(nf, VOC_FCAP);
        VCall cl; memset(&cl, 0, sizeof(cl));
        cl.ns = 1; cl.nf = n; cl.slot[0] = slot; cl.pos[0] = v->frames_done[slot];
        VTRY(voc_call(e, cl, s, false));
        v->frames_done[slot] += n; nf -= n;
    }
    if (is_last) v->last_flag[slot] = 1;
    return Q3TTS_OK;
}
int q3_voc_decode_batch(q3tts_engine* e, const int* slots, const int* real, int ns, int nf, hipStream_t s, int beside_decoder) {
    Q3Voc* v = e->voc;
    if (!v) return q3_set_err(e, Q3TTS_ERR_STATE, "engine has no vocoder");
    if (ns <= 0 || ns > v->B || nf <= 0 || nf > VOC_FCAP) return q3_set_err(e, Q3TTS_ERR_INVALID, "vocoder batch shape");
    for (int g0 = 0; g0 < ns; g0 += VOC_MAX_NS) {
        const int n = std::min(ns - g0, VOC_MAX_NS);
        VCall cl; memset(&cl, 0, sizeof(cl));
        cl.ns = n; cl.nf = nf;
        for (int i = 0; i < n; ++i) { cl.slot[i] = slots[g0 + i]; cl.pos[i] = v->frames_done[slots[g0 + i]]; }
        VTRY(voc_call(e, cl, s, beside_decoder && n >= 16));
        for (int i = g0; i < g0 + n; ++i) v->frames_done[slots[i]] += real ? real[i] : nf;
    }
    return Q3TTS_OK;
}
void q3_voc_mark_last(q3tts_engine* e, int slot) { if (e->voc) e->voc->last_flag[slot] = 1; }

float* q3_voc_pcm(q3tts_engine* e, int slot) { return e->voc->pcm + (size_t)slot * e->voc->pcm_stride; }
size_t q3_voc_pcm_stride(const q3tts_engine* e) { return e->voc ? e->voc->pcm_stride : 0; }
int q3_voc_samples(q3tts_engine* e, int slot) {
    Q3Voc* v = e->voc;
    int fr = v->frames_done[slot];
    if (!v->last_flag[slot]) fr = std::max(0, fr - v->c.lookahead_frames);
    return fr * v->spf;
}

struct VDriveCall { int index, f0, n; bool last; };
static const int VOC_DRIVE_STOP = 1;
template <class Step>
static int voc_drive(q3tts_engine* e, const int32_t* codes, int n_frames, int chunk_frames, bool args_ok, Step step) {
    Q3_NOT_IN_SESSION(e);
    if (!e || !codes || !args_ok || n_frames <= 0) return q3_set_err(e, Q3TTS_ERR_INVALID, "null argument");
    if (!e->voc) return q3_set_err(e, Q3TTS_ERR_STATE, "engine created with with_vocoder = 0");
    if (n_frames > e->cfg.max_steps_cap) return q3_set_err(e, Q3TTS_ERR_INVALID, "n_frames exceeds max_steps_cap");
    Q3_HIP(e, hipSetDevice(e->cfg.device));
    hipStream_t s = e->stream;
    Q3_HIP(e, hipMemcpyAsync(e->codes, codes, sizeof(int32_t) * (size_t)n_frames * e->cfg.model.n_codebooks, hipMemcpyHostToDevice, s));
    VTRY(q3_voc_reset(e, 0));
    const int chunk = chunk_frames > 0 ? chunk_frames : n_frames;
    int rc = Q3TTS_OK; VDriveCall c = {0, 0, 0, false};
    for (int f = 0; f < n_frames && rc == Q3TTS_OK; f += chunk) {
        const int end = std::min(f + chunk, n_frames);
        for (c.f0 = f; c.f0 < end && rc == Q3TTS_OK; c.f0 += c.n, ++c.index) {
            c.n = std::min(VOC_FCAP, end - c.f0); c.last = c.f0 + c.n >= n_frames;
            rc = step(c, false);
            if (rc == Q3TTS_OK) rc = q3_voc_decode(e, 0, c.f0, c.n, c.last, s);
            if (rc == Q3TTS_OK) rc = step(c, true);
        }
    }
    const hipError_t er = hipStreamSynchronize(s);
    if (rc < 0) return rc;
    Q3_HIP(e, er);
    return rc;
}

extern "C" int q3tts_k_vocoder(q3tts_engine* e, const int32_t* codes, int32_t n_frames, int32_t chunk_frames, float* pcm_out, int32_t* n_samples_out) {
    int ns = 0;
    VTRY(voc_drive(e, codes, n_frames, chunk_frames, pcm_out && n_samples_out, [&](const VDriveCall& c, bool after) {
        if (!after || !c.last) return Q3TTS_OK;
        ns = q3_voc_samples(e, 0);
        Q3_HIP(e, hipMemcpyAsync(pcm_out, q3_voc_pcm(e, 0), sizeof(float) * (size_t)ns, hipMemcpyDeviceToHost, e->stream));
        return Q3TTS_OK;
    }));
    *n_samples_out = ns;
    return Q3TTS_OK;
}

extern "C" int q3tts_k_vocoder_latent(q3tts_engine* e, const int32_t* codes, int32_t n_frames, int32_t chunk_frames, float* out) {
    return voc_drive(e, codes, n_frames, chunk_frames, out != nullptr, [&](const VDriveCall& c, bool after) {
        const int d = e->voc->c.latent_dim;
        if (after) Q3_HIP(e, hipMemcpyAsync(out + (size_t)c.f0 * d, e->voc->x, sizeof(float) * (size_t)c.n * d, hipMemcpyDeviceToHost, e->stream));
        return Q3TTS_OK;
    });
}

extern "C" int q3tts_k_vocoder_taps(q3tts_engine* e, const int32_t* codes, int32_t n_frames, int32_t chunk_frames, int32_t tap_call, void* buf,
                                    uint64_t buf_bytes, q3tts_voc_tap* recs, int32_t rec_cap, int32_t* n_recs) {
    VTapSink sink; sink.buf = (uint8_t*)buf; sink.cap = (size_t)buf_bytes; sink.recs = recs; sink.rec_cap = rec_cap;
    bool tapped = false;
    const int rc = voc_drive(e, codes, n_frames, chunk_frames, buf && recs && n_recs && tap_call >= 0, [&](const VDriveCall& c, bool after) {
        if (c.index != tap_call) return Q3TTS_OK;
        if (!after) { e->voc->taps = &sink; tapped = true; }
        return after ? VOC_DRIVE_STOP : Q3TTS_OK;
    });
    if (tapped) e->voc->taps = nullptr;
    if (rc < 0) return rc;
    if (rc != VOC_DRIVE_STOP) return q3_set_err(e, Q3TTS_ERR_INVALID, "tap_call is past the last call of this drive");
    if (sink.overflow) return q3_set_err(e, Q3TTS_ERR_INVALID, "tap buffer or record table too small");
    *n_recs = sink.n;
    return Q3TTS_OK;
}

#if defined(Q3_STAMPS) || defined(Q3_VOC_STAMPS)
static void voc_print_stamps() {
    unsigned long long st[2][4][16];
    if (hipMemcpyFromSymbol(st, HIP_SYMBOL(g_voc_stamps), sizeof(st)) != hipSuccess) return;
    for (int k = 0; k < 2; ++k)
        for (int w = 0; w < 3; ++w)
            fprintf(stderr, "resunit stamps (%s) wg %d (100 MHz ticks from entry): first weights requested %llu | input staged + barrier %llu | conv1 done %llu | snake tile done %llu | conv2 done %llu | stores issued %llu\n",
                    k == 0 ? "192 channels" : "96 channels", w, st[k][w][1] - st[k][w][0], st[k][w][2] - st[k][w][0], st[k][w][3] - st[k][w][0], st[k][w][4] - st[k][w][0], st[k][w][5] - st[k][w][0], st[k][w][6] - st[k][w][0]);
}
#endif
extern "C" int q3tts_k_vocoder_bench(q3tts_engine* e, int32_t n_slots, int32_t chunks, float* ms_per_chunk) {
    Q3_NOT_IN_SESSION(e);
    if (!e || !ms_per_chunk || n_slots <= 0 || chunks <= 0) return q3_set_err(e, Q3TTS_ERR_INVALID, "vocoder bench: bad argument");
    if (!e->voc) return q3_set_err(e, Q3TTS_ERR_STATE, "engine created with with_vocoder = 0");
    if (n_slots > e->B || (chunks + 2) * 4 > e->cfg.max_steps_cap) return q3_set_err(e, Q3TTS_ERR_INVALID, "vocoder bench: shape exceeds the engine's");
    Q3_HIP(e, hipSetDevice(e->cfg.device));
    const int ncb = e->cfg.model.n_codebooks, cap = e->cfg.max_steps_cap, cbs = e->cfg.vocoder.codebook_size;
    hipStream_t s = e->stream;
    std::vector<int32_t> codes((size_t)n_slots * cap * ncb);
    uint64_t st = 0x9E3779B97F4A7C15ULL;
    for (auto& c : codes) { st = q3_mix64(st + 0x1234567); c = (int32_t)(st % (uint64_t)cbs); }
    Q3_HIP(e, hipMemcpyAsync(e->codes, codes.data(), codes.size() * 4, hipMemcpyHostToDevice, s));
    Q3_HIP(e, hipStreamSynchronize(s));
    std::vector<int> slots(n_slots);
    for (int i = 0; i < n_slots; ++i) { slots[i] = i; VTRY(q3_voc_reset(e, i)); }
    for (int w = 0; w < 2; ++w) VTRY(q3_voc_decode_batch(e, slots.data(), nullptr, n_slots, 4, s, 0));
    Q3_HIP(e, hipEventRecord(e->ev0, s));
    for (int c = 0; c < chunks; ++c) VTRY(q3_voc_decode_batch(e, slots.data(), nullptr, n_slots, 4, s, 0));
    Q3_HIP(e, hipEventRecord(e->ev2, s));
    Q3_HIP(e, hipStreamSynchronize(s));
    float ms = 0.0f;
    Q3_HIP(e, hipEventElapsedTime(&ms, e->ev0, e->ev2));
    *ms_per_chunk = ms / (float)chunks;
#if defined(Q3_STAMPS) || defined(Q3_VOC_STAMPS)
    voc_print_stamps();
#endif
#ifdef Q3_VOC_STAMPS
    {
        unsigned long long st[4][8];
        if (hipMemcpyFromSymbol(st, HIP_SYMBOL(g_ring_stamps), sizeof(st)) == hipSuccess)
            for (int w = 0; w < 3; ++w)
                fprintf(stderr, "ring<3> stamps wg %d (10 ns ticks from entry): prologue issued %llu | first stage in LDS %llu | main loop done %llu | tile in LDS %llu | stores issued %llu | stores done %llu\n",
                        w, st[w][1] - st[w][0], st[w][2] - st[w][0], st[w][3] - st[w][0], st[w][4] - st[w][0], st[w][5] - st[w][0], st[w][6] - st[w][0]);
    }
#endif
    for (int i = 0; i < n_slots; ++i) VTRY(q3_voc_reset(e, i));
    return Q3TTS_OK;
}
```

### qwen3-tts-rust_amd/q3tts/_abi.py

```python
import ctypes as C
import os

HERE = os.path.dirname(os.path.abspath(__file__))
PKG_ROOT = os.path.dirname(HERE)
REPO_ROOT = os.path.dirname(PKG_ROOT)
LIB_PATH = os.path.join(PKG_ROOT, "csrc", "libq3tts.so")

Q3TTS_MAX_UPSAMPLE = 4
Q3TTS_MAX_DEC_BLOCKS = 8


class ModelConfig(C.Structure):
    _fields_ = [
        ("t_n_layer", C.c_int32), ("t_d_model", C.c_int32), ("t_n_head", C.c_int32), ("t_n_kv_head", C.c_int32),
        ("t_head_dim", C.c_int32), ("t_d_ffn", C.c_int32), ("t_vocab", C.c_int32),
        ("t_rope_theta", C.c_float),
        ("t_mrope_sections", C.c_int32 * 4),
        ("p_n_layer", C.c_int32), ("p_d_model", C.c_int32), ("p_n_head", C.c_int32), ("p_n_kv_head", C.c_int32),
        ("p_head_dim", C.c_int32), ("p_d_ffn", C.c_int32),
        ("p_rope_theta", C.c_float),
        ("n_codebooks", C.c_int32), ("codebook_size", C.c_int32),
        ("rms_eps", C.c_float),
        ("d_embed", C.c_int32), ("text_vocab", C.c_int32), ("codec0_rows", C.c_int32), ("codecq_rows", C.c_int32),
        ("sample_limit", C.c_int32), ("eos_code", C.c_int32), ("tts_pad_id", C.c_int32),
    ]


class VocoderConfig(C.Structure):
    _fields_ = [
        ("n_codebooks", C.c_int32), ("codebook_size", C.c_int32), ("codebook_dim", C.c_int32),
        ("latent_dim", C.c_int32), ("pre_conv_kernel", C.c_int32),
        ("n_layer", C.c_int32), ("n_head", C.c_int32), ("head_dim", C.c_int32), ("d_ffn", C.c_int32),
        ("sliding_window", C.c_int32),
        ("rope_theta", C.c_float), ("rms_eps", C.c_float), ("layer_scale_init", C.c_float),
        ("n_upsample", C.c_int32), ("upsample_ratios", C.c_int32 * Q3TTS_MAX_UPSAMPLE),
        ("decoder_dim", C.c_int32), ("n_dec_blocks", C.c_int32), ("dec_rates", C.c_int32 * Q3TTS_MAX_DEC_BLOCKS),
        ("lookahead_frames", C.c_int32), ("sample_rate", C.c_int32),
    ]


class EngineConfig(C.Structure):
    _fields_ = [
        ("model", ModelConfig), ("vocoder", VocoderConfig),
        ("device", C.c_int32), ("max_batch", C.c_int32), ("n_ctx", C.c_int32), ("max_steps_cap", C.c_int32),
        ("with_vocoder", C.c_int32),
        ("synth_seed", C.c_uint64),
        ("weights_path", C.c_char_p),
        ("talker_q8_0", C.c_int32),
        ("vocoder_flush_tail", C.c_int32),
        ("predictor_q8_0", C.c_int32),
    ]
    _tail_fields_ = ("kv_q8_0",)

    @property
    def kv_q8_0(self):
        return C.c_int32.from_buffer(self, C.sizeof(EngineConfig) - 4).value

    @kv_q8_0.setter
    def kv_q8_0(self, v):
        C.c_int32.from_buffer(self, C.sizeof(EngineConfig) - 4).value = int(v)


assert EngineConfig.predictor_q8_0.offset + 8 == C.sizeof(EngineConfig) and C.sizeof(EngineConfig) % 8 == 0, "q3tts_engine_config: kv_q8_0 no longer sits in the tail"
ENGINE_CONFIG_FIELD_ORDER = [f[0] for f in EngineConfig._fields_] + list(EngineConfig._tail_fields_)
KV_Q8_0_OFFSET = C.sizeof(EngineConfig) - 4


class PromptDesc(C.Structure):
    _fields_ = [
        ("text_ids", C.POINTER(C.c_uint32)), ("n_text", C.c_int32),
        ("instruct_ids", C.POINTER(C.c_uint32)), ("n_instruct", C.c_int32),
        ("lang_id", C.c_int32), ("spk_id", C.c_int32),
        ("spk_emb", C.POINTER(C.c_float)),
        ("ref_codes", C.POINTER(C.c_int32)), ("n_ref_frames", C.c_int32),
        ("ref_text_ids", C.POINTER(C.c_uint32)), ("n_ref_text", C.c_int32),
    ]


class Request(C.Structure):
    _fields_ = [
        ("prompt_embd", C.POINTER(C.c_float)), ("n_tok", C.c_int32),
        ("text_stream", C.c_int32),
        ("prompt", C.POINTER(PromptDesc)),
        ("use_engine_sampler", C.c_int32),
        ("temperature", C.c_float), ("top_k", C.c_int32), ("top_p", C.c_float), ("has_seed", C.c_int32),
        ("text_open", C.c_int32),
        ("seed", C.c_uint64),
        ("max_steps", C.c_int32), ("min_frames", C.c_int32), ("force_eos_at", C.c_int32), ("want_pcm", C.c_int32),
        ("prefix", C.c_void_p),
    ]


class Result(C.Structure):
    _fields_ = [
        ("status", C.c_int32), ("n_frames", C.c_int32), ("hit_eos", C.c_int32),
        ("codes", C.POINTER(C.c_int32)), ("pcm", C.POINTER(C.c_float)),
        ("n_samples", C.c_int32), ("sample_rate", C.c_int32),
        ("first_chunk_ms", C.c_float), ("total_ms", C.c_float),
    ]


class VocTap(C.Structure):
    _fields_ = [
        ("name", C.c_char * 32), ("dtype", C.c_int32), ("layout", C.c_int32), ("hist_rows", C.c_int32), ("rows", C.c_int32),
        ("channels", C.c_int32), ("reserved", C.c_int32), ("offset", C.c_uint64),
    ]


class SessionEvent(C.Structure):
    _fields_ = [
        ("id", C.c_uint64), ("kind", C.c_int32), ("status", C.c_int32), ("pcm", C.c_void_p), ("n_samples", C.c_int32),
        ("is_final", C.c_int32), ("result", Result),
    ]


EV_NONE, EV_CHUNK, EV_DONE, EV_FAILED, EV_CANCELLED = 0, 1, 2, 3, 4
EV_PREFIX = 5
PCM_F32, PCM_I16 = 0, 1
SESSION_RING_DEPTH = 4


class Timings(C.Structure):
    _fields_ = [
        ("prefill_ms", C.c_float), ("decode_ms", C.c_float), ("vocoder_ms", C.c_float), ("total_ms", C.c_float),
        ("frame_step_ms", C.c_float), ("probe_kernel_ms", C.c_float),
        ("frame_steps", C.c_int64), ("algo_bytes_per_step", C.c_int64), ("algo_flops_per_step", C.c_int64),
        ("mean_live_slots", C.c_float), ("mean_rows", C.c_float), ("probe_count", C.c_int64), ("probe_empty_ms", C.c_float),
        ("mean_ctx_tokens", C.c_float),
    ]


class NodeTimings(C.Structure):
    _fields_ = [("generate_ms", C.c_float), ("gather_ms", C.c_float), ("total_ms", C.c_float), ("gathered_bytes", C.c_int64), ("n_devices", C.c_int32)]


class CloneConfig(C.Structure):
    _fields_ = [
        ("mel_dim", C.c_int32),
        ("se_channels", C.c_int32 * 5), ("se_kernels", C.c_int32 * 5), ("se_dilations", C.c_int32 * 5),
        ("se_attn_channels", C.c_int32), ("se_res2net_scale", C.c_int32), ("se_se_channels", C.c_int32), ("se_dim", C.c_int32),
        ("ae_filters", C.c_int32), ("ae_kernel", C.c_int32), ("ae_res_kernel", C.c_int32), ("ae_last_kernel", C.c_int32),
        ("ae_n_ratios", C.c_int32), ("ae_ratios", C.c_int32 * 4),
        ("ae_hidden", C.c_int32), ("ae_n_layer", C.c_int32), ("ae_n_head", C.c_int32), ("ae_head_dim", C.c_int32),
        ("ae_d_ffn", C.c_int32), ("ae_window", C.c_int32),
        ("ae_rope_theta", C.c_float), ("ae_ln_eps", C.c_float), ("ae_layer_scale", C.c_float),
        ("ae_down_stride", C.c_int32), ("ae_vq_dim", C.c_int32), ("ae_n_codebooks", C.c_int32), ("ae_codebook_size", C.c_int32),
    ]


SYMBOLS = [
    "q3tts_default_config", "q3tts_engine_create", "q3tts_engine_destroy", "q3tts_last_error", "q3tts_set_sampler",
    "q3tts_set_max_steps", "q3tts_build_prompt", "q3tts_free", "q3tts_generate", "q3tts_generate_batch",
    "q3tts_result_free", "q3tts_stream_begin", "q3tts_stream_poll", "q3tts_stream_end",
    "q3tts_get_timings", "q3tts_k_gemm_exact", "q3tts_k_attention", "q3tts_k_attention_decode", "q3tts_k_sample", "q3tts_k_talker_prefill",
    "q3tts_k_vocoder", "q3tts_k_vocoder_latent", "q3tts_k_vocoder_taps", "q3tts_k_vocoder_bench", "q3tts_set_device_pcm", "q3tts_get_device_pcm", "q3tts_k_rng_f32", "q3tts_k_probe", "q3tts_k_gguf_read", "q3tts_mel_frames", "q3tts_mel",
    "q3tts_clone_default_config", "q3tts_clone_init", "q3tts_clone_audio_frames", "q3tts_clone_audio_encode",
    "q3tts_clone_speaker_encode", "q3tts_k_speaker_from_mel", "q3tts_k_audio_latent",
    "q3tts_node_create", "q3tts_node_destroy", "q3tts_node_generate_batch", "q3tts_node_get_timings", "q3tts_node_last_error", "q3tts_node_size", "q3tts_node_engine", "q3tts_node_shard", "q3tts_k_bgemm_q8", "q3tts_k_bgemm_q8a8_argmax", "q3tts_k_bgemm_q8a8", "q3tts_k_alloc_upload", "q3tts_k_bgemm_policy", "q3tts_k_attend_policy", "q3tts_k_bgemm_pick", "q3tts_k_mfma_bf16", "q3tts_k_bgemm", "q3tts_k_bgemm_voc", "q3tts_k_project", "q3tts_k_norm_inputs", "q3tts_tokenizer_load", "q3tts_tokenizer_free", "q3tts_tokenizer_vocab_size", "q3tts_tokenizer_encode", "q3tts_tokenizer_decode",
    "q3tts_session_create", "q3tts_session_submit", "q3tts_session_cancel", "q3tts_session_next", "q3tts_session_close",
    "q3tts_session_last_error", "q3tts_k_pcm_pack",
    "q3tts_prefix_create", "q3tts_prefix_rows", "q3tts_prefix_destroy", "q3tts_k_talker_prefill_prefix",
    "q3tts_config_from_model_dir", "q3tts_k_gguf_meta",
    "q3tts_set_predictor_sampler", "q3tts_get_predictor_sampler", "q3tts_set_repetition_penalty", "q3tts_get_repetition_penalty",
    "q3tts_k_pred_variant",
    "q3tts_set_output_rate", "q3tts_get_output_rate", "q3tts_resample", "q3tts_k_resample_table", "q3tts_k_pcm_resample",
    "q3tts_session_append_text", "q3tts_k_text_ready",
    "q3tts_k_attention_runs", "q3tts_k_attention_decode_ex", "q3tts_k_attention_pair", "q3tts_k_attend_pick",
    "q3tts_k_attention_runs_kv8", "q3tts_k_attention_decode_kv8", "q3tts_k_attend_pick_kv8",
    "q3tts_k_pred_table_row", "q3tts_k_pred_next", "q3tts_k_attention_gather",
    "q3tts_k_row_buckets", "q3tts_k_bucket_steps", "q3tts_k_device_bytes", "q3tts_k_engine_footprint", "q3tts_k_prefix_stats",
    "q3tts_session_prefix_create", "q3tts_session_submit_keep_voice", "q3tts_session_prefix_release", "q3tts_session_clone",
    "q3tts_prefix_state", "q3tts_k_prefix_read",
    "q3tts_session_submit_paced", "q3tts_session_grant", "q3tts_session_set_swap", "q3tts_session_swap_stats",
    "q3tts_k_credit_ready", "q3tts_k_swap_arena", "q3tts_k_swap_phase_ms",
    "q3tts_k_request_rules",
    "q3tts_set_speed", "q3tts_get_speed", "q3tts_time_stretch", "q3tts_k_tempo_counts", "q3tts_k_pcm_tempo",
    "q3tts_text_split", "q3tts_long_default_opts", "q3tts_generate_long", "q3tts_long_result_free", "q3tts_pcm_join",
    "q3tts_k_pcm_edges", "q3tts_k_pcm_join",
]

BREAK_END, BREAK_HARD, BREAK_CLAUSE, BREAK_SENTENCE, BREAK_PARAGRAPH = 0, 1, 2, 3, 4
JOIN_W = 240
LONG_MAX_SEGMENTS = 1024


class TextSpan(C.Structure):
    _fields_ = [("begin", C.c_int64), ("end", C.c_int64), ("kind", C.c_int32)]


class JoinOpts(C.Structure):
    _fields_ = [("trim", C.c_int32), ("threshold", C.c_float), ("keep", C.c_int32), ("fade", C.c_int32), ("pause_ms", C.c_int32 * 5)]


class LongSegment(C.Structure):
    _fields_ = [("ids", C.POINTER(C.c_uint32)), ("n_ids", C.c_int32), ("kind", C.c_int32), ("max_steps", C.c_int32)]


class LongOpts(C.Structure):
    _fields_ = [("join", JoinOpts), ("speed_permille", C.c_int32), ("output_rate", C.c_int32)]


class LongInfo(C.Structure):
    _fields_ = [
        ("status", C.c_int32), ("n_frames", C.c_int32), ("hit_eos", C.c_int32),
        ("n_native", C.c_int64), ("lo", C.c_int64), ("hi", C.c_int64),
        ("begin", C.c_int64), ("end", C.c_int64), ("out_begin", C.c_int64), ("out_end", C.c_int64),
    ]


class LongResult(C.Structure):
    _fields_ = [
        ("status", C.c_int32), ("n_segments", C.c_int32), ("n_truncated", C.c_int32), ("sample_rate", C.c_int32),
        ("n_samples", C.c_int64), ("pcm", C.POINTER(C.c_float)), ("info", C.POINTER(LongInfo)),
        ("generate_ms", C.c_float), ("join_ms", C.c_float), ("total_ms", C.c_float),
    ]


class PredStep(C.Structure):
    _fields_ = [
        ("n_rows", C.c_int32), ("q", C.c_int32), ("n_codebooks", C.c_int32), ("n_key_parts", C.c_int32), ("rows_q", C.c_int32),
        ("d_embed", C.c_int32), ("d_proj", C.c_int32), ("max_steps_cap", C.c_int32),
        ("keys", C.c_void_p), ("active", C.c_void_p), ("n_frames", C.c_void_p), ("codec_q", C.c_void_p), ("pproj_q", C.c_void_p),
        ("proj_b", C.c_void_p), ("fb", C.c_void_p), ("px", C.c_void_p), ("codes", C.c_void_p),
    ]


class Q3Error(RuntimeError):
    pass


_lib = None


def load_library(path=None):
    global _lib
    if _lib is not None and path is None:
        return _lib
    p = path or os.environ.get("Q3TTS_LIB") or LIB_PATH
# ... 32 lines not shown
    lib.q3tts_session_close.argtypes = [vp]
    lib.q3tts_session_last_error.argtypes = [vp]
    lib.q3tts_session_last_error.restype = C.c_char_p
    lib.q3tts_session_append_text.argtypes = [vp, C.c_uint64, u32p, C.c_int32, C.c_int32]
    lib.q3tts_session_prefix_create.argtypes = [vp, C.POINTER(PromptDesc), f32p, C.c_int32, C.POINTER(vp), C.POINTER(C.c_uint64)]
    lib.q3tts_session_submit_keep_voice.argtypes = [vp, C.POINTER(Request), C.c_int32, C.POINTER(C.c_uint64), C.POINTER(vp)]
    lib.q3tts_session_prefix_release.argtypes = [vp, vp]
    lib.q3tts_session_clone.argtypes = [vp, f32p, C.c_int64, C.c_int32, C.POINTER(C.c_int64), C.c_int32, C.POINTER(C.c_int32), f32p]
    lib.q3tts_prefix_state.argtypes = [vp]
    lib.q3tts_prefix_state.restype = C.c_int32
    lib.q3tts_k_prefix_read.argtypes = [vp, vp, vp, C.c_int64, C.POINTER(C.c_int64)]
    lib.q3tts_k_text_ready.argtypes = [C.c_int32, C.c_int32, C.c_int32]
    lib.q3tts_session_submit_paced.argtypes = [vp, C.POINTER(Request), C.c_int32, C.POINTER(C.c_uint64)]
    lib.q3tts_session_grant.argtypes = [vp, C.c_uint64, C.c_int32]
    lib.q3tts_session_set_swap.argtypes = [vp, C.c_int64]
    lib.q3tts_session_swap_stats.argtypes = [vp, C.POINTER(C.c_int64)]
    lib.q3tts_k_credit_ready.argtypes = [C.c_int64, C.c_int32]
    lib.q3tts_k_request_rules.argtypes = [C.POINTER(Request), C.c_int32, C.c_int32, C.c_char_p, C.c_int32]
    lib.q3tts_k_swap_phase_ms.argtypes = [vp, C.POINTER(C.c_double)]
    lib.q3tts_k_swap_arena.argtypes = [C.c_int64, C.POINTER(C.c_int64), C.c_int32, C.POINTER(C.c_int64)]
    lib.q3tts_k_pcm_pack.argtypes = [C.c_int32, f32p, C.c_int32, C.c_int64, i32p, i32p, i32p, C.POINTER(C.c_int64), C.c_int32, C.c_int32, vp,
                                     C.c_int64]
    lib.q3tts_set_output_rate.argtypes = [vp, C.c_int32]
    lib.q3tts_get_output_rate.argtypes = [vp, i32p]
    lib.q3tts_resample.argtypes = [vp, f32p, C.c_int64, C.c_int32, C.c_int32, f32p, C.c_int64, C.POINTER(C.c_int64)]
    lib.q3tts_k_resample_table.argtypes = [C.c_int32, C.c_int32, i32p, i32p, i32p, f32p, C.c_int64, C.POINTER(C.c_int64)]
    lib.q3tts_k_pcm_resample.argtypes = [C.c_int32, f32p, C.c_int32, C.c_int64, i32p, i32p, i32p, i32p, i32p, C.POINTER(C.c_int64), C.c_int32,
                                         C.c_int32, C.c_int32, C.c_int32, vp, C.c_int64, C.c_int32, f32p]
    lib.q3tts_set_speed.argtypes = [vp, C.c_int32]
    lib.q3tts_get_speed.argtypes = [vp, i32p]
    lib.q3tts_time_stretch.argtypes = [vp, f32p, C.c_int64, C.c_int32, f32p, C.c_int64, C.POINTER(C.c_int64)]
    lib.q3tts_k_tempo_counts.argtypes = [C.c_int64, C.c_int32, C.POINTER(C.c_int64), C.POINTER(C.c_int64)]
    lib.q3tts_k_pcm_tempo.argtypes = [C.c_int32, f32p, C.c_int32, C.c_int64, i32p, C.c_int32, i32p, C.c_int32, f32p, C.c_int64, i32p, i32p, C.c_int64,
                                      C.c_int32, f32p]
    i64p = C.POINTER(C.c_int64)
    lib.q3tts_text_split.argtypes = [C.c_char_p, C.c_int64, C.c_int32, C.c_int32, C.POINTER(TextSpan), C.c_int32, i32p, C.c_char_p, C.c_int32]
    lib.q3tts_long_default_opts.argtypes = [C.POINTER(LongOpts)]
    lib.q3tts_long_default_opts.restype = None
    lib.q3tts_generate_long.argtypes = [vp, C.POINTER(Request), C.POINTER(PromptDesc), vp, C.POINTER(LongSegment), C.c_int32, C.POINTER(LongOpts),
                                        C.POINTER(LongResult)]
    lib.q3tts_long_result_free.argtypes = [C.POINTER(LongResult)]
    lib.q3tts_long_result_free.restype = None
    lib.q3tts_pcm_join.argtypes = [vp, C.POINTER(f32p), i64p, i32p, C.c_int32, C.POINTER(JoinOpts), f32p, C.c_int64, i64p, i64p]
    lib.q3tts_k_pcm_edges.argtypes = [C.c_int32, f32p, C.c_int32, C.c_int64, i32p, C.c_float, i32p, C.c_int32, f32p]
    lib.q3tts_k_pcm_join.argtypes = [C.c_int32, f32p, C.c_int32, C.c_int64, i32p, i32p, i32p, C.POINTER(JoinOpts), C.c_int32, f32p, C.c_int64, i64p, i64p,
                                     C.c_int32, f32p]
    lib.q3tts_stream_begin.argtypes = [vp, C.POINTER(Request), C.POINTER(vp)]
    lib.q3tts_stream_poll.argtypes = [vp, C.POINTER(f32p), i32p, i32p]
    lib.q3tts_stream_end.argtypes = [vp, C.POINTER(Result)]
    lib.q3tts_get_timings.argtypes = [vp, C.POINTER(Timings)]
    lib.q3tts_k_gemm_exact.argtypes = [C.c_int32, f32p, C.c_int32, C.c_int32, C.POINTER(C.c_uint16), C.c_int32, f32p,
                                       C.c_float, f32p, C.c_int32, f32p, C.POINTER(C.c_uint64), C.c_int32, f32p]
    lib.q3tts_k_attention.argtypes = [C.c_int32, f32p, C.c_int32, C.c_int32, C.c_int32, C.c_int32, C.c_int32, f32p, f32p,
                                      C.c_float, C.c_float, i32p, f32p]
    lib.q3tts_k_attention_decode.argtypes = [C.c_int32, f32p, C.c_int32, i32p, C.c_int32, C.c_int32, C.c_int32, C.c_int32, f32p, f32p,
                                             C.c_float, C.c_float, i32p, C.c_int32, f32p, C.POINTER(C.c_uint16)]
    lib.q3tts_k_attention_runs.argtypes = [C.c_int32, f32p, C.c_int32, i32p, i32p, C.c_int32, C.c_int32, C.c_int32, C.c_int32, f32p, f32p, C.c_float,
                                           C.c_float, i32p, C.c_int32, C.c_int32, C.c_void_p, C.c_void_p, C.c_void_p, C.c_void_p]
    lib.q3tts_k_attention_decode_ex.argtypes = [C.c_int32, f32p, C.c_int32, i32p, C.c_int32, C.c_int32, C.c_int32, C.c_int32, f32p, f32p, C.c_float,
                                                C.c_float, i32p, C.c_int32, C.c_int32, C.c_int32, C.c_void_p, C.c_void_p, C.c_void_p, C.c_void_p]
    lib.q3tts_k_attention_pair.argtypes = [C.c_int32, f32p, C.c_int32, C.c_int32, C.c_int32, C.c_int32, C.c_int32, f32p, f32p, C.c_float, C.c_float,
                                           i32p, C.c_int32, C.c_void_p, C.c_void_p, C.c_void_p, C.c_void_p]
    lib.q3tts_k_attend_pick.argtypes = [C.c_int32, C.c_int32, C.c_int32, C.c_int32, C.c_int32, C.c_int32, C.c_int32, i32p]
    lib.q3tts_k_attention_runs_kv8.argtypes = [C.c_int32, f32p, C.c_int32, i32p, i32p, C.c_int32, C.c_int32, C.c_int32, C.c_int32, f32p, f32p, C.c_float,
                                               C.c_float, i32p, C.c_int32, C.c_int32, C.c_void_p, C.c_void_p, C.c_void_p, C.c_void_p, C.c_void_p, C.c_void_p]
    lib.q3tts_k_attention_decode_kv8.argtypes = [C.c_int32, f32p, C.c_int32, i32p, C.c_int32, C.c_int32, C.c_int32, C.c_int32, f32p, f32p, C.c_float,
                                                 C.c_float, i32p, C.c_int32, C.c_int32, C.c_void_p, C.c_void_p, C.c_void_p, C.c_void_p, C.c_void_p, C.c_void_p]
    lib.q3tts_k_attend_pick_kv8.argtypes = [C.c_int32, C.c_int32, C.c_int32, C.c_int32, C.c_int32, C.c_int32, C.c_int32, i32p]
    lib.q3tts_k_pred_table_row.argtypes = [vp, C.c_int32, C.c_int32, f32p]
    lib.q3tts_k_pred_next.argtypes = [C.c_int32, C.POINTER(PredStep), C.c_void_p, C.c_void_p, C.c_void_p]
    lib.q3tts_k_attention_gather.argtypes = [C.c_int32, C.POINTER(PredStep), C.c_void_p, C.c_void_p, C.c_int32, C.c_int32, C.c_int32, C.c_int32, C.c_int32,
                                             f32p, f32p, C.c_float, C.c_float, i32p, C.c_int32, C.c_void_p, C.c_void_p, C.c_void_p, C.c_void_p]
    lib.q3tts_k_sample.argtypes = [C.c_int32, f32p, C.c_int32, C.c_int32, C.c_int32, C.c_float, C.c_int32, C.c_float,
                                   f32p, i32p]
    lib.q3tts_k_talker_prefill.argtypes = [vp, f32p, C.c_int32, f32p, f32p]
    lib.q3tts_k_talker_prefill_prefix.argtypes = [vp, vp, f32p, C.c_int32, f32p, f32p]
    lib.q3tts_prefix_create.argtypes = [vp, C.POINTER(PromptDesc), f32p, C.c_int32, C.POINTER(vp)]
    lib.q3tts_prefix_rows.argtypes = [vp]
    lib.q3tts_prefix_rows.restype = C.c_int32
    lib.q3tts_prefix_destroy.argtypes = [vp]
    lib.q3tts_k_vocoder.argtypes = [vp, i32p, C.c_int32, C.c_int32, f32p, i32p]
    lib.q3tts_k_vocoder_latent.argtypes = [vp, i32p, C.c_int32, C.c_int32, f32p]
    lib.q3tts_k_vocoder_taps.argtypes = [vp, i32p, C.c_int32, C.c_int32, C.c_int32, C.c_void_p, C.c_uint64, C.POINTER(VocTap), C.c_int32, i32p]
    lib.q3tts_k_vocoder_bench.argtypes = [vp, C.c_int32, C.c_int32, f32p]
    lib.q3tts_set_device_pcm.argtypes = [vp, C.c_int32]
    lib.q3tts_get_device_pcm.argtypes = [vp, C.POINTER(f32p), C.POINTER(C.c_int64), i32p]
    lib.q3tts_k_rng_f32.argtypes = [C.c_uint64, C.c_int32, f32p]
    lib.q3tts_k_probe.argtypes = [C.c_void_p, C.c_int32]
    lib.q3tts_mel_frames.argtypes = [C.c_int64]
    lib.q3tts_mel_frames.restype = C.c_int32
    lib.q3tts_mel.argtypes = [C.c_void_p, f32p, C.c_int64, f32p, C.c_int32, C.POINTER(C.c_int32)]
    lib.q3tts_k_gguf_read.argtypes = [C.c_char_p, C.c_char_p, f32p, C.c_int64, C.POINTER(C.c_int64), C.POINTER(C.c_int64), C.POINTER(C.c_int32)]
    lib.q3tts_k_gguf_meta.argtypes = [C.c_char_p, C.c_char_p, i32p, i32p, C.POINTER(C.c_int64), C.POINTER(C.c_double), C.c_int64, C.c_char_p, C.c_int64,
                                      C.POINTER(C.c_int64)]
    lib.q3tts_config_from_model_dir.argtypes = [C.c_char_p, C.c_char_p, C.POINTER(EngineConfig), C.c_char_p, C.c_int32, C.c_char_p, C.c_int32]
    lib.q3tts_clone_default_config.argtypes = [C.POINTER(CloneConfig)]
    lib.q3tts_clone_default_config.restype = None
    lib.q3tts_clone_init.argtypes = [vp, C.POINTER(CloneConfig)]
    lib.q3tts_clone_audio_frames.argtypes = [vp, C.c_int64]
    lib.q3tts_clone_audio_frames.restype = C.c_int32
    lib.q3tts_clone_audio_encode.argtypes = [vp, f32p, C.c_int64, C.POINTER(C.c_int64), C.c_int32, i32p]
    lib.q3tts_clone_speaker_encode.argtypes = [vp, f32p, C.c_int64, f32p]
    lib.q3tts_k_speaker_from_mel.argtypes = [vp, f32p, C.c_int32, f32p]
    lib.q3tts_k_audio_latent.argtypes = [vp, f32p, C.c_int64, f32p, C.c_int32, i32p]
    lib.q3tts_k_mfma_bf16.argtypes = [C.c_int32, C.c_void_p, C.c_void_p, C.c_void_p, C.c_void_p, C.c_int32, C.c_int32]
    lib.q3tts_k_bgemm.argtypes = [C.c_int32, C.c_void_p, C.c_int32, C.c_int32, C.c_void_p, C.c_int32, C.c_void_p, C.c_int32, C.c_int32, C.c_float,
                                  C.c_int32, C.c_void_p, C.c_void_p, C.c_void_p, C.c_void_p, C.c_void_p, C.c_int32, f32p]
    lib.q3tts_k_project.argtypes = [C.c_int32, C.c_void_p, C.c_int32, C.c_int32, C.c_void_p, C.c_void_p, C.c_int32, C.c_void_p, C.c_void_p, C.c_void_p, C.c_void_p]
    lib.q3tts_k_norm_inputs.argtypes = [C.c_int32, C.c_void_p, C.c_int32, C.c_int32, C.c_void_p, C.c_void_p, C.c_void_p]
    lib.q3tts_k_bgemm_voc.argtypes = [C.c_int32, C.c_void_p, C.c_int32, C.c_int32, C.c_void_p, C.c_int32, C.c_int32, C.c_void_p, C.c_int32, C.c_void_p,
                                      C.c_int32, C.c_int32, C.c_void_p, C.c_void_p, C.c_int32]
    lib.q3tts_node_create.argtypes = [C.POINTER(EngineConfig), i32p, C.c_int32, C.POINTER(vp)]
    lib.q3tts_node_destroy.argtypes = [vp]
    lib.q3tts_node_destroy.restype = None
    lib.q3tts_node_generate_batch.argtypes = [vp, C.POINTER(Request), C.c_int32, C.POINTER(Result), C.POINTER(C.POINTER(C.c_int16))]
    lib.q3tts_node_get_timings.argtypes = [vp, C.POINTER(NodeTimings)]
    lib.q3tts_node_last_error.argtypes = [vp]
    lib.q3tts_node_last_error.restype = C.c_char_p
    lib.q3tts_node_size.argtypes = [vp]
    lib.q3tts_node_size.restype = C.c_int32
    lib.q3tts_node_engine.argtypes = [vp, C.c_int32]
    lib.q3tts_node_engine.restype = vp
    lib.q3tts_node_shard.argtypes = [C.c_int32, C.c_int32, C.c_int32, i32p, C.c_int32]
    lib.q3tts_node_shard.restype = C.c_int32
    lib.q3tts_k_bgemm_q8.argtypes = [C.c_int32, C.c_void_p, C.c_int32, C.c_int32, C.c_void_p, C.c_void_p, C.c_int32, C.c_void_p, C.c_int32, C.c_int32, C.c_float,
                                     C.c_int32, C.c_void_p, C.c_void_p, C.c_void_p, C.c_void_p, C.c_void_p, C.c_int32, f32p]
    lib.q3tts_k_bgemm_q8a8_argmax.argtypes = [C.c_int32, C.c_void_p, C.c_void_p, C.c_int32, C.c_int32, C.c_void_p, C.c_void_p, C.c_int32, C.c_void_p, C.c_int32, C.c_int32, C.c_float, C.c_void_p]
    lib.q3tts_k_bgemm_q8a8_argmax.restype = C.c_int
    lib.q3tts_k_bgemm_q8a8.argtypes = [C.c_int32, C.c_void_p, C.c_void_p, C.c_int32, C.c_int32, C.c_void_p, C.c_void_p, C.c_int32, C.c_void_p, C.c_int32, C.c_int32, C.c_float,
                                       C.c_int32, C.c_void_p, C.c_void_p, C.c_void_p, C.c_void_p, C.c_void_p, C.c_int32, f32p]
    lib.q3tts_k_bgemm_policy.argtypes = [C.c_int32]
    lib.q3tts_k_attend_policy.argtypes = [C.c_int32, C.c_int32]
    lib.q3tts_k_bgemm_pick.argtypes = [C.c_int32, C.c_int32, C.c_int32, C.c_int32, C.c_int32, C.c_int32, i32p]
    lib.q3tts_k_alloc_upload.argtypes = [vp, C.c_int64, C.POINTER(C.c_int64)]
    lib.q3tts_k_row_buckets.argtypes = [C.c_int32, i32p, C.c_int32]
    lib.q3tts_k_bucket_steps.argtypes = [vp, C.POINTER(C.c_int64), C.c_int32]
    lib.q3tts_k_device_bytes.argtypes = [vp, C.POINTER(C.c_int64)]
    lib.q3tts_k_prefix_stats.argtypes = [vp, C.POINTER(C.c_int64)]
    lib.q3tts_k_engine_footprint.argtypes = [C.POINTER(EngineConfig), C.POINTER(C.c_int64)]
    lib.q3tts_tokenizer_load.argtypes = [C.c_char_p, C.POINTER(vp), C.c_char_p, C.c_int32]
    lib.q3tts_tokenizer_free.argtypes = [vp]
    lib.q3tts_tokenizer_free.restype = None
    lib.q3tts_tokenizer_vocab_size.argtypes = [vp]
    lib.q3tts_tokenizer_vocab_size.restype = C.c_int32
    lib.q3tts_tokenizer_encode.argtypes = [vp, C.c_char_p, C.c_int64, u32p, C.c_int32, i32p, C.c_char_p, C.c_int32]
    lib.q3tts_tokenizer_decode.argtypes = [vp, u32p, C.c_int32, C.c_char_p, C.c_int64, C.POINTER(C.c_int64), C.c_char_p, C.c_int32]
    if path is None:
        _lib = lib
    return lib


def default_config():
    cfg = EngineConfig()
    load_library().q3tts_default_config(C.byref(cfg))
    return cfg


def copy_config(cfg):
    c = EngineConfig.from_buffer_copy(cfg)
    c._source = cfg
    return c


def tiny_config(max_batch=4, n_ctx=256, with_vocoder=1):
    cfg = EngineConfig()
    m = cfg.model
# ... 92 lines not shown
```

### qwen3-tts-rust_amd/q3tts/native.py

```python
import ctypes as C
import math
import os
import weakref

import numpy as np

from . import _abi

f32p, i32p, u32p = C.POINTER(C.c_float), C.POINTER(C.c_int32), C.POINTER(C.c_uint32)


def _ptr(a, typ):
    return a.ctypes.data_as(typ)


_LANG_DEFAULT = object()


def make_prompt_desc(text_ids, spk_emb=None, lang_id=_LANG_DEFAULT, spk_id=-1, instruct_ids=None, ref_codes=None,
                     ref_text_ids=None, part="whole"):
    if part not in ("whole", "voice", "text"):
        raise ValueError(f"part must be 'whole', 'voice' or 'text', not {part!r}")
    if part == "voice" and text_ids is not None and len(text_ids) > 0:
        raise ValueError("a voice-only desc has no text: text_ids must be None or empty")
# ... 308 lines not shown
    def clone_init(self, ccfg):
        self._check(self.lib.q3tts_clone_init(self.h, C.byref(ccfg)), "q3tts_clone_init")
        self.clone_cfg = ccfg

    def clone_audio_frames(self, n_samples):
        return int(self.lib.q3tts_clone_audio_frames(self.h, int(n_samples)))

    def _clone_codebooks(self):
        c = getattr(self, "clone_cfg", None)
        return c.ae_n_codebooks if c is not None else 16

    def audio_encode(self, audio):
        a = np.ascontiguousarray(audio, dtype=np.float32)
        cap = max(self.clone_audio_frames(a.size), 1)
        ncb = self._clone_codebooks()
        out = np.zeros((cap, ncb), dtype=np.int64)
        n = C.c_int32(0)
        self._check(self.lib.q3tts_clone_audio_encode(self.h, _ptr(a, f32p) if a.size else None, a.size,
                                                      out.ctypes.data_as(C.POINTER(C.c_int64)), cap, C.byref(n)), "q3tts_clone_audio_encode")
        return out[:n.value].copy()

    def audio_latent(self, audio):
        a = np.ascontiguousarray(audio, dtype=np.float32)
        cap = max(self.clone_audio_frames(a.size), 1)
        out = np.zeros((cap, self.clone_cfg.ae_hidden), dtype=np.float32)
        n = C.c_int32(0)
        self._check(self.lib.q3tts_k_audio_latent(self.h, _ptr(a, f32p) if a.size else None, a.size, _ptr(out, f32p), cap, C.byref(n)),
                    "q3tts_k_audio_latent")
        return out[:n.value].copy()

    def speaker_encode(self, audio):
        a = np.ascontiguousarray(audio, dtype=np.float32)
        c = getattr(self, "clone_cfg", None)
        out = np.zeros(c.se_dim if c is not None else self.cfg.model.d_embed, dtype=np.float32)
        self._check(self.lib.q3tts_clone_speaker_encode(self.h, _ptr(a, f32p) if a.size else None, a.size, _ptr(out, f32p)),
                    "q3tts_clone_speaker_encode")
        return out

    def speaker_from_mel(self, mel):
        m = np.ascontiguousarray(mel, dtype=np.float32)
        out = np.zeros(self.clone_cfg.se_dim, dtype=np.float32)
        self._check(self.lib.q3tts_k_speaker_from_mel(self.h, _ptr(m, f32p), m.shape[0], _ptr(out, f32p)), "q3tts_k_speaker_from_mel")
        return out

    def probe(self, enable):
        mode = 2 if enable is True else int(enable)
        self._check(self.lib.q3tts_k_probe(self.h, mode), "q3tts_k_probe")

    def alloc_upload_mismatches(self, nbytes):
        bad = C.c_int64(-1)
        self._check(self.lib.q3tts_k_alloc_upload(self.h, int(nbytes), C.byref(bad)), "q3tts_k_alloc_upload")
        return int(bad.value)

    def talker_prefill(self, embd):
        e = np.ascontiguousarray(embd, dtype=np.float32)
        hid = np.zeros(self.cfg.model.t_d_model, dtype=np.float32)
        lg = np.zeros(self.cfg.model.t_vocab, dtype=np.float32)
        self._check(self.lib.q3tts_k_talker_prefill(self.h, _ptr(e, f32p), e.shape[0], _ptr(hid, f32p), _ptr(lg, f32p)),
                    "q3tts_k_talker_prefill")
        return hid, lg

    def talker_prefill_prefix(self, prefix, embd):
        e = np.ascontiguousarray(embd, dtype=np.float32)
        hid = np.zeros(self.cfg.model.t_d_model, dtype=np.float32)
        lg = np.zeros(self.cfg.model.t_vocab, dtype=np.float32)
        self._check(self.lib.q3tts_k_talker_prefill_prefix(self.h, prefix.h, _ptr(e, f32p), e.shape[0], _ptr(hid, f32p), _ptr(lg, f32p)),
                    "q3tts_k_talker_prefill_prefix")
        return hid, lg

    def vocoder(self, codes, chunk_frames=0):
        c = np.ascontiguousarray(codes, dtype=np.int32)
        spf = 1
        v = self.cfg.vocoder
        for i in range(v.n_upsample):
            spf *= v.upsample_ratios[i]
        for i in range(v.n_dec_blocks):
            spf *= v.dec_rates[i]
        pcm = np.zeros(c.shape[0] * spf + 16, dtype=np.float32)
        ns = C.c_int32()
        self._check(self.lib.q3tts_k_vocoder(self.h, _ptr(c, i32p), c.shape[0], chunk_frames, _ptr(pcm, f32p), C.byref(ns)),
                    "q3tts_k_vocoder")
        return pcm[:ns.value].copy()

    def vocoder_latent(self, codes, chunk_frames=0):
        c = np.ascontiguousarray(codes, dtype=np.int32)
        out = np.zeros((c.shape[0], self.cfg.vocoder.latent_dim), dtype=np.float32)
        self._check(self.lib.q3tts_k_vocoder_latent(self.h, _ptr(c, i32p), c.shape[0], chunk_frames, _ptr(out, f32p)), "q3tts_k_vocoder_latent")
        return out

    def vocoder_taps(self, codes, chunk_frames=0, tap_call=0, buf_bytes=160 << 20):
        c = np.ascontiguousarray(codes, dtype=np.int32)
        buf = np.empty(buf_bytes, dtype=np.uint8)
        recs = (_abi.VocTap * 256)()
        n = C.c_int32()
        self._check(self.lib.q3tts_k_vocoder_taps(self.h, _ptr(c, i32p), c.shape[0], chunk_frames, tap_call, buf.ctypes.data, buf.size, recs, 256,
                                                  C.byref(n)), "q3tts_k_vocoder_taps")
        out = {}
        for r in recs[:n.value]:
            H, T, K = r.hist_rows, r.rows, r.channels
            dt = np.uint16 if r.dtype else np.float32
            if r.layout:
                flat = np.frombuffer(buf, dtype=dt, count=((H + T + 15) // 16) * 16 * K, offset=r.offset)
                row, k = np.arange(H + T)[:, None], np.arange(K)[None, :]
                cc = k & 31
                off = ((((row >> 4) * (K >> 5) + (k >> 5)) * 64 + ((cc & 15) >> 2) * 16 + (row & 15)) << 3) + (cc & 3) + ((cc & 16) >> 2)
                a = flat[off]
            else:
                a = np.frombuffer(buf, dtype=dt, count=(H + T) * K, offset=r.offset).reshape(H + T, K).copy()
            out[r.name.decode()] = (a, H)
        return out


class NativePrefix:

    def __init__(self, engine: NativeEngine, h, session=None):
        self.engine, self.lib, self.h = engine, engine.lib, h
        self.session = session
        self._n_rows = int(self.lib.q3tts_prefix_rows(h))

    @property
    def n_rows(self):
        if not self._n_rows and getattr(self, "h", None):
            self._n_rows = int(self.lib.q3tts_prefix_rows(self.h))
        return self._n_rows

    @property
    def state(self):
        if not getattr(self, "h", None):
            raise _abi.Q3Error("the prefix is closed")
        return int(self.lib.q3tts_prefix_state(self.h))

    def close(self):
        if getattr(self, "h", None):
            sess = self.session
            if sess is not None and getattr(sess, "h", None):
                sess._check(self.lib.q3tts_session_prefix_release(sess.h, self.h), "q3tts_session_prefix_release")
            else:
                self.engine._check(self.lib.q3tts_prefix_destroy(self.h), "q3tts_prefix_destroy")
            self.h = None

    def __enter__(self):
        return self

    def __exit__(self, *exc):
        self.close()

    def __del__(self):
        try:
            self.close()
        except _abi.Q3Error:
            pass


class NativeSession:

    def __init__(self, engine: NativeEngine, pcm_format=_abi.PCM_F32, swap_mb=0):
        self.engine, self.lib = engine, engine.lib
        self.dtype = np.int16 if pcm_format == _abi.PCM_I16 else np.float32
        self._ctype = C.c_int16 if pcm_format == _abi.PCM_I16 else C.c_float
        self._open = set()
        self.h = C.c_void_p()
        engine._check(self.lib.q3tts_session_create(engine.h, pcm_format, C.byref(self.h)), "q3tts_session_create")
        if swap_mb:
            try:
                self.set_swap(int(swap_mb * (1 << 20)))
            except _abi.Q3Error:
# ... 536 lines not shown
        raise _abi.Q3Error(f"q3tts_k_attention_pair failed ({rc}): {lib.q3tts_last_error(None).decode()}")
    return _att_hook_ret(out, sc, kc, vc)


class PredStepState:

    def __init__(self, q, n_codebooks, keys, active, n_frames, codec_q, pproj_q, proj_b, fb, px, codes):
        c = np.ascontiguousarray
        self.keys = c(keys, dtype=np.uint64); self.active = c(active, dtype=np.int32); self.n_frames = c(n_frames, dtype=np.int32)
        self.codec_q = c(codec_q, dtype=np.float32); self.pproj_q = c(pproj_q, dtype=np.float32); self.proj_b = c(proj_b, dtype=np.float32)
        self.fb = np.array(fb, dtype=np.float32, order="C"); self.px = np.array(px, dtype=np.float32, order="C")
        self.codes = np.array(codes, dtype=np.int32, order="C")
        n = self.keys.shape[0]
        assert self.active.shape == (n,) and self.n_frames.shape == (n,) and self.fb.shape == (n, self.codec_q.shape[1])
        assert self.px.shape == (n, self.pproj_q.shape[1]) and self.codes.shape[0] == n and self.codes.shape[2] == n_codebooks
        st = _abi.PredStep()
        st.n_rows, st.q, st.n_codebooks, st.n_key_parts, st.rows_q = n, q, n_codebooks, self.keys.shape[1], self.codec_q.shape[0]
        st.d_embed, st.d_proj, st.max_steps_cap = self.codec_q.shape[1], self.pproj_q.shape[1], self.codes.shape[1]
        for name in ("keys", "active", "n_frames", "codec_q", "pproj_q", "proj_b", "fb", "px", "codes"):
            setattr(st, name, getattr(self, name).ctypes.data)
        self.st = st


def k_pred_next(state, norm_w, device=0):
    lib = _abi.load_library()
    nw = np.ascontiguousarray(norm_w, dtype=np.float32)
    n, dp = state.px.shape
    xb = np.zeros((n, dp), dtype=np.uint16); ssp = np.zeros((n, dp // 16), dtype=np.float32)
    rc = lib.q3tts_k_pred_next(device, C.byref(state.st), nw.ctypes.data, xb.ctypes.data, ssp.ctypes.data)
    if rc != 0:
        raise _abi.Q3Error(f"q3tts_k_pred_next failed ({rc}): {lib.q3tts_last_error(None).decode()}")
    return xb, ssp


def k_attention_gather(state, table, qkv, length, n_ctx, n_head, n_kv_head, head_dim, q_norm_w, k_norm_w, eps, rope_theta, sections, out_form=0,
                       want_cache=True, device=0):
    lib = _abi.load_library()
    tab = np.ascontiguousarray(table, dtype=np.float32)
    qkv = np.ascontiguousarray(qkv, dtype=np.float32)
    n = state.px.shape[0]
    ld = (n_head + 2 * n_kv_head) * head_dim
    assert qkv.shape == (n * length, ld) and tab.shape == (state.codec_q.shape[0] + 1, ld)
    qn = np.ascontiguousarray(q_norm_w, dtype=np.float32)
    kn = np.ascontiguousarray(k_norm_w, dtype=np.float32)
    sec = None if sections is None else np.ascontiguousarray(sections, dtype=np.int32)
    out, sc, kc, vc = _att_hook_out(n, n_head * head_dim, out_form, n, n_kv_head, n_ctx, head_dim, want_cache)
    rc = lib.q3tts_k_attention_gather(device, C.byref(state.st), tab.ctypes.data, qkv.ctypes.data, length, n_ctx, n_head, n_kv_head, head_dim,
                                      _ptr(qn, f32p), _ptr(kn, f32p), eps, rope_theta, None if sec is None else _ptr(sec, i32p), out_form,
                                      _dp(out), _dp(sc), _dp(kc), _dp(vc))
    if rc != 0:
        raise _abi.Q3Error(f"q3tts_k_attention_gather failed ({rc}): {lib.q3tts_last_error(None).decode()}")
    return _att_hook_ret(out, sc, kc, vc)


def k_sample(logits, limit, temperature, top_k, top_p, r=None, device=0):
    lib = _abi.load_library()
    lg = np.ascontiguousarray(logits, dtype=np.float32)
    n, ld = lg.shape
    out = np.zeros(n, dtype=np.int32)
    rr = None if r is None else np.ascontiguousarray(r, dtype=np.float32)
    rc = lib.q3tts_k_sample(device, _ptr(lg, f32p), n, ld, limit, temperature, top_k, top_p, None if rr is None else _ptr(rr, f32p),
                            _ptr(out, i32p))
    if rc != 0:
        raise _abi.Q3Error(f"q3tts_k_sample failed ({rc}): {lib.q3tts_last_error(None).decode()}")
    return out


def k_gguf_read(path, tensor=""):
    lib = _abi.load_library()
    n = C.c_int64(0); dims = (C.c_int64 * 4)(); ty = C.c_int32(0)
    rc = lib.q3tts_k_gguf_read(os.fsencode(path), tensor.encode(), None, 0, C.byref(n), dims, C.byref(ty))
    if rc != 0:
        raise _abi.Q3Error(f"q3tts_k_gguf_read: {lib.q3tts_last_error(None).decode()} (status {rc})")
    out = np.zeros(n.value, dtype=np.float32)
    rc = lib.q3tts_k_gguf_read(os.fsencode(path), tensor.encode(), _ptr(out, f32p), n.value, C.byref(n), dims, C.byref(ty))
    if rc != 0:
        raise _abi.Q3Error(f"q3tts_k_gguf_read: {lib.q3tts_last_error(None).decode()} (status {rc})")
    shape = [int(d) for d in dims if d]
    if not str(path).endswith(".npy"):
        shape = shape[::-1]
    return out.reshape(shape), int(ty.value)


GGUF_VALUE_TYPES = ("u8", "i8", "u16", "i16", "u32", "i32", "f32", "bool", "str", "array", "u64", "i64", "f64")


def k_gguf_meta(path, key):
    lib = _abi.load_library()
    vt, et, n, nb = C.c_int32(0), C.c_int32(0), C.c_int64(0), C.c_int64(0)
    rc = lib.q3tts_k_gguf_meta(os.fsencode(path), key.encode(), C.byref(vt), C.byref(et), C.byref(n), None, 0, None, 0, C.byref(nb))
    if rc != 0:
        raise _abi.Q3Error(f"q3tts_k_gguf_meta: {lib.q3tts_last_error(None).decode()} (status {rc})")
    vals = (C.c_double * max(1, n.value))(); buf = C.create_string_buffer(max(1, nb.value))
    rc = lib.q3tts_k_gguf_meta(os.fsencode(path), key.encode(), C.byref(vt), C.byref(et), C.byref(n), vals, n.value, buf, nb.value, C.byref(nb))
    if rc != 0:
        raise _abi.Q3Error(f"q3tts_k_gguf_meta: {lib.q3tts_last_error(None).decode()} (status {rc})")
    tname, ename = GGUF_VALUE_TYPES[vt.value], GGUF_VALUE_TYPES[et.value]
    raw = buf.raw[:nb.value]
    if tname == "str":
        return tname, ename, raw
    if tname != "array":
        return tname, ename, vals[0]
    if ename != "str":
        return tname, ename, list(vals[:n.value])
    out, pos = [], 0
    for _ in range(n.value):
        ln = int.from_bytes(raw[pos:pos + 8], "little")
        out.append(raw[pos + 8:pos + 8 + ln])
        pos += 8 + ln
    return tname, ename, out


def config_from_model_dir(model_dir, quant=None, base=None):
    lib = _abi.load_library()
    cfg = _abi.copy_config(base) if base is not None else _abi.default_config()
    md = os.fsencode(model_dir)
    buf = C.create_string_buffer(len(md) + 16)
    err = C.create_string_buffer(1024)
    q = None if quant is None else str(quant).encode()
    rc = lib.q3tts_config_from_model_dir(md, q, C.byref(cfg), buf, len(buf), err, len(err))
    if rc != 0:
        raise _abi.Q3Error(f"q3tts_config_from_model_dir failed ({rc}): {err.value.decode('utf-8', 'replace')}")
    cfg._path_buf = buf
    return cfg


def k_pcm_pack(src, entries, out_n, fmt=0, device=0):
    lib = _abi.load_library()
    src = np.ascontiguousarray(src, dtype=np.float32)
    rows, stride = src.shape
    e = np.asarray(entries, dtype=np.int64).reshape(-1, 4)
    er, ef, ec = (np.ascontiguousarray(e[:, i], dtype=np.int32) for i in range(3))
    ed = np.ascontiguousarray(e[:, 3], dtype=np.int64)
    out = np.zeros(max(int(out_n), 1), dtype=np.int16 if fmt else np.float32)
    rc = lib.q3tts_k_pcm_pack(device, _ptr(src, f32p), rows, stride, _ptr(er, i32p), _ptr(ef, i32p), _ptr(ec, i32p),
                              ed.ctypes.data_as(C.POINTER(C.c_int64)), len(e), fmt, out.ctypes.data, int(out_n))
    if rc != 0:
        raise _abi.Q3Error(f"q3tts_k_pcm_pack failed ({rc}): {lib.q3tts_last_error(None).decode()}")
    return out[:int(out_n)]


def k_resample_table(rate_in, rate_out):
    lib = _abi.load_library()
    L, M, H, n = C.c_int32(), C.c_int32(), C.c_int32(), C.c_int64()
    tab = np.zeros(32768, dtype=np.float32)
    rc = lib.q3tts_k_resample_table(int(rate_in), int(rate_out), C.byref(L), C.byref(M), C.byref(H), _ptr(tab, f32p), tab.size, C.byref(n))
    if rc != 0:
        e = _abi.Q3Error(f"q3tts_k_resample_table failed ({rc}): {lib.q3tts_last_error(None).decode()}")
        e.status = rc
        raise e
    return L.value, M.value, H.value, tab[:n.value].reshape(L.value, 2 * H.value + 1).copy()


def k_pcm_resample(src, row_len, row_final, entries, out_n, rate_in, rate_out, fmt=0, device=0, iters=0):
    lib = _abi.load_library()
    src = np.ascontiguousarray(src, dtype=np.float32)
    rows, stride = src.shape
    ms = C.c_float(0)
    rl, rf = np.ascontiguousarray(row_len, dtype=np.int32), np.ascontiguousarray(row_final, dtype=np.int32)
    if rl.shape != (rows,) or rf.shape != (rows,):
        raise ValueError("k_pcm_resample: row_len and row_final take one value per row of src")
    e = np.asarray(entries, dtype=np.int64).reshape(-1, 4)
    er, ef, ec = (np.ascontiguousarray(e[:, i], dtype=np.int32) for i in range(3))
    ed = np.ascontiguousarray(e[:, 3], dtype=np.int64)
    out = np.zeros(max(int(out_n), 1), dtype=np.int16 if fmt else np.float32)
    rc = lib.q3tts_k_pcm_resample(device, _ptr(src, f32p), rows, stride, _ptr(rl, i32p), _ptr(rf, i32p), _ptr(er, i32p), _ptr(ef, i32p),
# ... 178 lines not shown
```

Measured before the change: 694.5.

## Fuse input snake into vocoder resunit kernel and stage fp32 residual rows

By default the vocoder residual units now read an fp32 residual buffer (xres) and apply the first snake activation inside the fused resunit kernel, instead of consuming a precomputed bf16 snaked input. In polite mode the kernel keeps the fp32 input rows in LDS to reuse them as the residual, which avoids re-reading global memory. History buffers are added for the new fp32 inputs. New slot-batched vocoder and history-plan APIs are also added. The cost is larger fp32 history and reads, plus extra LDS in the keep variant.

After: 695.6 (median of 5 runs). About the same (+0.2%).

```diff
diff --git a/include/q3tts.h b/include/q3tts.h
--- a/include/q3tts.h
+++ b/include/q3tts.h
@@ -335,6 +335,13 @@
 } q3tts_voc_tap;
 int q3tts_k_vocoder_taps(q3tts_engine* e, const int32_t* codes, int32_t n_frames, int32_t chunk_frames, int32_t tap_call, void* buf,
                          uint64_t buf_bytes, q3tts_voc_tap* recs, int32_t rec_cap, int32_t* n_recs);
+int q3tts_k_vocoder_slots(q3tts_engine* e, const int32_t* codes, int32_t n_slots, int32_t max_frames, const int32_t* n_frames,
+                          int32_t chunk_frames, int32_t beside_decoder, float* pcm_out);
+typedef struct q3tts_voc_hist_ent {
+    char name[32];
+    int32_t hist_rows, channels, elem_bytes, rows_per_frame, saved_at_end, reserved;
+} q3tts_voc_hist_ent;
+int q3tts_k_voc_hist_plan(const q3tts_vocoder_config* c, int32_t res_bf16, int32_t no_fuse, q3tts_voc_hist_ent* out, int32_t cap, int32_t* n);
 int q3tts_k_vocoder_bench(q3tts_engine* e, int32_t n_slots, int32_t chunks, float* ms_per_chunk);
 int q3tts_k_gguf_read(const char* path, const char* tensor, float* out, int64_t cap, int64_t* nelem, int64_t* dims4, int32_t* ggml_type);
 int q3tts_k_gguf_meta(const char* path, const char* key, int32_t* value_type, int32_t* elem_type, int64_t* count, double* values,
diff --git a/qwen3-tts-rust_amd/csrc/q3_vocoder.hip b/qwen3-tts-rust_amd/csrc/q3_vocoder.hip
--- a/qwen3-tts-rust_amd/csrc/q3_vocoder.hip
+++ b/qwen3-tts-rust_amd/csrc/q3_vocoder.hip
@@ -37,7 +37,8 @@
                 VConv qkv, gu; };
 struct VUp { VConv ct, pw1, pw2; float *dw_w, *dw_b, *ln_w, *ln_b, *gamma; int r; VBuf dw_in;
              uint4 *ct_t = nullptr, *pw1_t = nullptr, *pw2_t = nullptr; };
-struct VRes { float *ea, *ib, *ea2, *ib2; VConv c1, c2; VBuf c1_in; };
+struct VRes { float *ea, *ib, *ea2, *ib2; VConv c1, c2; VBuf c1_in;
+              VBuf xres; };
 struct VBlk { float *ea, *ib; VConv ct; VRes res[3]; int r, cin, cout; VBuf ct_in; };
 
 struct VLaunch {
@@ -48,6 +49,8 @@
     auto tie() const { return std::tie(polite, no_ring, no_tap, tap_min, no_fuse, out_old, attn_old); }
     bool operator<(const VLaunch& o) const { return tie() < o.tie(); }
 };
+static const int VOC_RES_DIL[3] = {1, 3, 9};
+static bool resunit_width(int C) { return C == 32 || C == 64 || C == 96 || C == 128 || C == 192; }
 typedef std::tuple<int, int, VLaunch> VCallKey;
 static size_t voc_lds_floor(const VLaunch& vl, size_t lds) { return vl.polite ? std::max(lds, (size_t)81 * 1024) : lds; }
 
@@ -73,6 +76,8 @@
     float *x = nullptr, *xn = nullptr, *xnb = nullptr, *qkv = nullptr, *att = nullptr, *g = nullptr;
     float *t1 = nullptr, *t2 = nullptr;
     float* pcm = nullptr; size_t pcm_stride = 0;
+    bool res_f32 = true;
+    bool exp_192_alone = false;
     std::vector<int> frames_done, last_flag;
     VCall* call_dev = nullptr;
     VCall* call_host = nullptr; hipEvent_t call_ev[16] = {}; unsigned call_i = 0;
@@ -103,6 +108,7 @@
     else { tap = step / kpt; k0 = (step - tap * kpt) << 5; }
 }
 
+__device__ __forceinline__ float vsnake(float v, float ea, float ib) { const float sn = __sinf(v * ea); return v + ib * (sn * sn); }
 __device__ __forceinline__ float gelu_erf(float x) { return 0.5f * x * (1.0f + erff(x * 0.70710678118654752f)); }
 
 __device__ __forceinline__ void vepi(const VGemm& g, float v, int s, int t, int n, float yold) {
@@ -115,8 +121,7 @@
     if (g.store) *yp = v;
     if (g.y2) {
         const int c = n % g.snake_n;
-        const float sn = __sinf(v * g.ea[c]);
-        const float sv = v + g.ib[c] * (sn * sn);
+        const float sv = vsnake(v, g.ea[c], g.ib[c]);
         const size_t o2 = (size_t)s * g.y2_stride + g.y2_off + (size_t)t * nout + n;
         if (g.y2_bf16) ((__bf16*)g.y2)[o2] = (__bf16)sv; else g.y2[o2] = sv;
     }
@@ -361,10 +366,7 @@
                 if (!LITE && epi == 1) v[q] = yv[q] + sc4[q] * v[q];
                 else if (epi == 2) v[q] = yv[q] + v[q];
                 else if (!LITE && epi == 3) v[q] = gelu_erf(v[q]);
-                if (has_y2) {
-                    const float sn = __sinf(v[q] * ea4[q]);
-                    sv[q] = v[q] + ib4[q] * (sn * sn);
-                }
+                if (has_y2) sv[q] = vsnake(v[q], ea4[q], ib4[q]);
             }
             if (g.store) *(float4*)(g.y + g.y_off + n + (size_t)sl * g.y_stride + (size_t)t * nout) = make_float4(v[0], v[1], v[2], v[3]);
             if (has_y2) {
@@ -636,10 +638,12 @@
 
 struct VResUnit {
     const float* xin; size_t xin_stride;
+    const float *ea1, *ib1;
     int T, dil;
     const uint16_t *w1, *w2; const float *b1, *b2;
     const float *ea2, *ib2;
-    float* o; size_t o_stride; int store_o;
+    const float* oin; size_t oin_stride; int oin_off;
+    float* o; size_t o_stride; int o_off; int store_o;
     float* y2; size_t y2_stride; int y2_off; const float *ea3, *ib3;
 };
 #if defined(Q3_STAMPS) || defined(Q3_VOC_STAMPS)
@@ -649,8 +653,9 @@
 #define VR_STAMP(i_) do { } while (0)
 #endif
 #define VR_BARRIER() __syncthreads()
-template <int NT, int MT, int NWV>
+template <int NT, int MT, int NWV, bool XF32, bool KEEP>
 __global__ __launch_bounds__(64 * NWV) void k_voc_resunit(VResUnit g) {
+    static_assert(XF32 || !KEEP, "only the f32 staging has rows to keep");
 #if defined(Q3_STAMPS) || defined(Q3_VOC_STAMPS)
     const int stamp_wg = (blockIdx.y == 5 && (blockIdx.x == 3 || blockIdx.x == 20)) ? (blockIdx.x == 3 ? 0 : 1) : ((blockIdx.y == 40 && blockIdx.x == 11) ? 2 : -1);
 #endif
@@ -662,6 +667,8 @@
     __bf16* At = lds;
     __bf16* Zt = lds;
     __bf16* Bs = At + (size_t)(R + halo) * LDA;
+    constexpr int LDO = C + 4;
+    float* Xs = (float*)lds + max(((size_t)(R + halo) * LDA + (size_t)2 * C * 32) * 2, (size_t)R * LDO * 4) / 4;
     const int tid = threadIdx.x, wave = tid >> 6, lane = tid & 63, lr = lane & 15, kq = lane >> 4;
     const int sidx = blockIdx.y, t0 = blockIdx.x * R, T = g.T;
     const int bn = tid >> 2, bpart = tid & 3;
@@ -684,7 +691,29 @@
     } while (0)
     VR_GLOADB(ra, 0);
     VR_STAMP(1);
-    {
+    if (XF32) {
+        constexpr int c4n = C / 4, RPP = NTHR / c4n, PB = KEEP ? 20 : 12;
+        const float* xp = g.xin + (size_t)sidx * g.xin_stride + (size_t)t0 * C;
+        const int nrow = R + halo, cg = tid % c4n, r0 = tid / c4n, c = cg * 4, rlast = T + halo - 1 - t0;
+        const bool act = r0 < RPP;
+        const float4 ea = *(const float4*)(g.ea1 + c), ib = *(const float4*)(g.ib1 + c);
+        for (int p0 = 0; p0 * RPP < nrow; p0 += PB) {
+            float4 v[PB];
+#pragma unroll
+            for (int u = 0; u < PB; ++u) {
+                const int r = min(min(r0 + (p0 + u) * RPP, nrow - 1), rlast);
+                v[u] = *(const float4*)(xp + (size_t)r * C + c);
+            }
+#pragma unroll
+            for (int u = 0; u < PB; ++u) {
+                const int r = r0 + (p0 + u) * RPP;
+                if (!act || r >= nrow) continue;
+                __bf16 h[4] = {(__bf16)vsnake(v[u].x, ea.x, ib.x), (__bf16)vsnake(v[u].y, ea.y, ib.y), (__bf16)vsnake(v[u].z, ea.z, ib.z), (__bf16)vsnake(v[u].w, ea.w, ib.w)};
+                *(uint2*)(At + (size_t)r * LDA + c) = r <= rlast ? *(const uint2*)h : make_uint2(0, 0);
+                if (KEEP && r >= halo) *(float4*)(Xs + (size_t)(r - halo) * C + c) = v[u];
+            }
+        }
+    } else {
         const uint16_t* xp = (const uint16_t*)g.xin + (size_t)sidx * g.xin_stride + (size_t)t0 * C;
         const int nrow = R + halo, c8 = C / 8, total = nrow * c8;
         for (int base = tid; base < total; base += 12 * NTHR) {
@@ -726,8 +755,7 @@
                 const float bb = g.b1[n], ea = g.ea2[n], ib = g.ib2[n];                                                 \
                 _Pragma("unroll") for (int e = 0; e < 4; ++e) {                                                         \
                     const float v = acc[i][j][e] + bb;                                                                  \
-                    const float sn = __sinf(v * ea);                                                                    \
-                    Zt[(size_t)(wrow0 + i * 16 + 4 * kq + e) * LDA + n] = (__bf16)(v + ib * (sn * sn));                 \
+                    Zt[(size_t)(wrow0 + i * 16 + 4 * kq + e) * LDA + n] = (__bf16)vsnake(v, ea, ib);                    \
                     acc[i][j][e] = 0.0f;                                                                                \
                 }                                                                                                       \
             }                                                                                                           \
@@ -766,7 +794,6 @@
 #undef VR_GLOADB
 #undef VR_SSTOREB
 #undef VR_DECL
-    constexpr int LDO = C + 4;
     float* Ot = (float*)lds;
 #pragma unroll
     for (int i = 0; i < MTW; ++i)
@@ -780,18 +807,20 @@
     __syncthreads();
     {
         constexpr int c4n = C / 4, RPP = NTHR / c4n, PER = (R + RPP - 1) / RPP;
-        float* ob = g.o + (size_t)sidx * g.o_stride;
+        const float* ib_ = g.oin + (size_t)sidx * g.oin_stride + g.oin_off;
+        float* ob = g.o + (size_t)sidx * g.o_stride + g.o_off;
         __bf16* yb = (__bf16*)g.y2 + (size_t)sidx * g.y2_stride + g.y2_off;
         const int cg = tid % c4n, r0 = tid / c4n, c = cg * 4;
-        const bool act = r0 < RPP;
-        const float4 ea = *(const float4*)(g.ea3 + c), ib = *(const float4*)(g.ib3 + c);
+        const bool act = r0 < RPP, has_y2 = g.y2 != nullptr;
+        float4 ea = make_float4(0.f, 0.f, 0.f, 0.f), ib = ea;
+        if (has_y2) { ea = *(const float4*)(g.ea3 + c); ib = *(const float4*)(g.ib3 + c); }
         constexpr int PB = PER < 13 ? PER : 13;
         for (int p0 = 0; p0 < PER; p0 += PB) {
             float4 ov[PB];
 #pragma unroll
             for (int u = 0; u < PB; ++u) {
                 const int row = min(r0 + (p0 + u) * RPP, R - 1);
-                ov[u] = *(const float4*)(ob + (size_t)min(t0 + row, T - 1) * C + c);
+                ov[u] = KEEP ? *(const float4*)(Xs + (size_t)row * C + c) : *(const float4*)(ib_ + (size_t)min(t0 + row, T - 1) * C + c);
             }
 #pragma unroll
             for (int u = 0; u < PB; ++u) {
@@ -800,12 +829,10 @@
                 const float4 a = *(const float4*)&Ot[(size_t)row * LDO + c];
                 float4 v; v.x = ov[u].x + a.x; v.y = ov[u].y + a.y; v.z = ov[u].z + a.z; v.w = ov[u].w + a.w;
                 if (g.store_o) *(float4*)(ob + (size_t)t * C + c) = v;
-                float sn; __bf16 h[4];
-                sn = __sinf(v.x * ea.x); h[0] = (__bf16)(v.x + ib.x * (sn * sn));
-                sn = __sinf(v.y * ea.y); h[1] = (__bf16)(v.y + ib.y * (sn * sn));
-                sn = __sinf(v.z * ea.z); h[2] = (__bf16)(v.z + ib.z * (sn * sn));
-                sn = __sinf(v.w * ea.w); h[3] = (__bf16)(v.w + ib.w * (sn * sn));
-                *(uint2*)(yb + (size_t)t * C + c) = *(const uint2*)h;
+                if (has_y2) {
+                    __bf16 h[4] = {(__bf16)vsnake(v.x, ea.x, ib.x), (__bf16)vsnake(v.y, ea.y, ib.y), (__bf16)vsnake(v.z, ea.z, ib.z), (__bf16)vsnake(v.w, ea.w, ib.w)};
+                    *(uint2*)(yb + (size_t)t * C + c) = *(const uint2*)h;
+                }
             }
         }
     }
@@ -849,6 +876,15 @@
     *(uint2*)(dst + (size_t)s * dst_stride + i) = *(const uint2*)h;
 }
 
+__global__ void k_voc_snake_bf16(const float* src, uint16_t* dst, size_t n, int C, const float* ea, const float* ib) {
+    const size_t i = ((size_t)blockIdx.x * blockDim.x + threadIdx.x) * 4;
+    if (i >= n) return;
+    const int c = (int)(i % C);
+    const float4 v = *(const float4*)(src + i), a = *(const float4*)(ea + c), b = *(const float4*)(ib + c);
+    __bf16 h[4] = {(__bf16)vsnake(v.x, a.x, b.x), (__bf16)vsnake(v.y, a.y, b.y), (__bf16)vsnake(v.z, a.z, b.z), (__bf16)vsnake(v.w, a.w, b.w)};
+    *(uint2*)(dst + i) = *(const uint2*)h;
+}
+
 template <class E>
 __global__ void k_voc_hist(const VCall* __restrict__ clp, E* work, size_t stride, E* hist, int H, int C, int T, int save) {
     const VCall& cl = *clp;
@@ -863,7 +899,7 @@
 
 struct VHistTab {
     int n;
-    struct Ent { char* work; char* hist; unsigned long long stride_b, block_b, tail_b; } e[24];
+    struct Ent { char* work; char* hist; unsigned long long stride_b, block_b, tail_b; } e[40];
 };
 __global__ void k_voc_hist_all(const VCall* __restrict__ clp, VHistTab tab, int save) {
     const VCall& cl = *clp;
@@ -1227,6 +1263,7 @@
     Q3Voc* v = new Q3Voc();
     e->voc = v;
     v->c = c; v->B = e->B;
+    { const char* ev = getenv("Q3TTS_VOC_RES_BF16"); v->res_f32 = !(ev && atoi(ev)); ev = getenv("Q3TTS_EXP_VOC_192_ALONE"); v->exp_192_alone = ev && atoi(ev); }
     const int d = c.latent_dim, HH = c.n_head * c.head_dim;
     v->RW = c.sliding_window + VOC_FCAP;
     v->cb.resize(c.n_codebooks);
@@ -1322,12 +1359,13 @@
         VTRY(mk_buf(e, v, &k.ct_in, 1, ch, rows, 1));
         rows *= r;
         scratch = std::max(scratch, (size_t)rows * k.cout);
-        const int dil[3] = {1, 3, 9};
+        const int* dil = VOC_RES_DIL;
         for (int u = 0; u < 3; ++u) {
             VRes& s = k.res[u]; const int rc = comp + 1 + u;
             VTRY(gen_snake(e, v, VTID(rc, VW_ALPHA), VTID(rc, VW_BETA), k.cout, &s.ea, &s.ib));
             VTRY(gen_conv(e, v, &s.c1, rc, VW_W, VW_B, 7, dil[u], k.cout, k.cout, k.cout, 0.5f));
             VTRY(mk_buf(e, v, &s.c1_in, 6 * dil[u], k.cout, rows, 1));
+            if (v->res_f32 && resunit_width(k.cout)) VTRY(mk_buf(e, v, &s.xres, 6 * dil[u], k.cout, rows));
             VTRY(gen_snake(e, v, VTID(rc, VW_ALPHA2), VTID(rc, VW_BETA2), k.cout, &s.ea2, &s.ib2));
             VTRY(gen_conv(e, v, &s.c2, rc, VW_W2, VW_B2, 1, 1, k.cout, k.cout, k.cout, 0.5f));
         }
@@ -1370,7 +1408,7 @@
     add(v->pre_in);
     for (auto& u : v->U) add(u.dw_in);
     add(v->dec_in_in);
-    for (auto& b : v->Bk) { add(b.ct_in); for (auto& r : b.res) add(r.c1_in); }
+    for (auto& b : v->Bk) { add(b.ct_in); for (auto& r : b.res) { add(r.c1_in); if (r.xres.hist) add(r.xres); } }
     add(v->out_in);
     return tab;
 }
@@ -1451,27 +1489,47 @@
     else if (c.nout % 64 == 0 && (long)((c.nout + 127) / 128) * ((g.M + 127) / 128) < 192) launch_vgemm_tile<2>(vl, s, g);
     else launch_vgemm_tile<4>(vl, s, g);
 }
-static bool resunit_ok(const VLaunch& vl, int C) { return !vl.no_fuse && (C == 32 || C == 64 || C == 96 || C == 128 || C == 192); }
-template <int NT, int MT, int NWV = 4>
+static bool resunit_ok(const VLaunch& vl, int C) { return !vl.no_fuse && resunit_width(C); }
+template <int NT, int MT, int NWV = 4, bool XF32 = false, bool KEEP = false>
 static void launch_resunit_t(const VLaunch& vl, hipStream_t s, const VResUnit& g, int ns) {
     constexpr int C = NT * 16, R = 64 * MT, LDA = C + 16;
-    const size_t lds = voc_lds_floor(vl, std::max(((size_t)(R + 6 * g.dil) * LDA + (size_t)2 * C * 32) * 2, (size_t)R * (C + 4) * 4));
+    const size_t lds = voc_lds_floor(vl, std::max(((size_t)(R + 6 * g.dil) * LDA + (size_t)2 * C * 32) * 2, (size_t)R * (C + 4) * 4) + (KEEP ? (size_t)R * C * 4 : 0));
     static Q3PerDevice pd;
-    pd.ensure(1, []() { hipFuncSetAttribute((const void*)k_voc_resunit<NT, MT, NWV>, hipFuncAttributeMaxDynamicSharedMemorySize, 160 * 1024 - 1024); });
-    hipLaunchKernelGGL((k_voc_resunit<NT, MT, NWV>), dim3((g.T + R - 1) / R, ns), dim3(64 * NWV), lds, s, g);
-}
-static void launch_resunit(const VLaunch& vl, hipStream_t s, const VRes& r, int ns, int T, int C, float* o, int store_o, const VSnake& sk) {
+    pd.ensure(1, []() { hipFuncSetAttribute((const void*)k_voc_resunit<NT, MT, NWV, XF32, KEEP>, hipFuncAttributeMaxDynamicSharedMemorySize, 160 * 1024 - 1024); });
+    hipLaunchKernelGGL((k_voc_resunit<NT, MT, NWV, XF32, KEEP>), dim3((g.T + R - 1) / R, ns), dim3(64 * NWV), lds, s, g);
+}
+template <bool XF32>
+static void launch_resunit_c(const VLaunch& vl, hipStream_t s, const VResUnit& g, int ns, int C, bool alone192) {
+    constexpr bool K = XF32;
+    switch (C) {
+        case 32: if (vl.polite) launch_resunit_t<2, 4, 4, XF32, K>(vl, s, g, ns); else launch_resunit_t<2, 4, 4, XF32>(vl, s, g, ns); break;
+        case 64: if (vl.polite) launch_resunit_t<4, 3, 4, XF32, K>(vl, s, g, ns); else launch_resunit_t<4, 3, 4, XF32>(vl, s, g, ns); break;
+        case 96: if (vl.polite) launch_resunit_t<6, 2, 4, XF32, K>(vl, s, g, ns); else launch_resunit_t<6, 2, 4, XF32>(vl, s, g, ns); break;
+        case 128: if (vl.polite) launch_resunit_t<8, 1, 4, XF32, K>(vl, s, g, ns); else launch_resunit_t<8, 1, 4, XF32>(vl, s, g, ns); break;
+        default:
+            if (vl.polite || alone192) launch_resunit_t<12, 1, 4, XF32, K>(vl, s, g, ns);
+            else launch_resunit_t<12, 2, 8, XF32>(vl, s, g, ns);
+            break;
+    }
+}
+static void launch_resunit(const Q3Voc* v, const VLaunch& vl, hipStream_t s, const VBlk& k, int u, int ns, int T, float* o, int store_o, const VSnake& sk) {
+    const VRes& r = k.res[u]; const int C = k.cout;
     VResUnit g;
-    g.xin = r.c1_in.p; g.xin_stride = r.c1_in.stride(); g.T = T; g.dil = r.c1.dil;
+    g.T = T; g.dil = r.c1.dil; g.ea1 = r.ea; g.ib1 = r.ib;
     g.w1 = r.c1.w; g.w2 = r.c2.w; g.b1 = r.c1.b; g.b2 = r.c2.b; g.ea2 = r.ea2; g.ib2 = r.ib2;
-    g.o = o; g.o_stride = (size_t)T * C; g.store_o = store_o;
+    g.store_o = store_o;
     g.y2 = sk.to.p; g.y2_stride = sk.to.stride; g.y2_off = sk.to.off; g.ea3 = sk.ea; g.ib3 = sk.ib;
-    switch (C) {
-        case 32: launch_resunit_t<2, 4>(vl, s, g, ns); break;
-        case 64: launch_resunit_t<4, 3>(vl, s, g, ns); break;
-        case 96: launch_resunit_t<6, 2>(vl, s, g, ns); break;
-        case 128: launch_resunit_t<8, 1>(vl, s, g, ns); break;
-        default: if (vl.polite) launch_resunit_t<12, 1>(vl, s, g, ns); else launch_resunit_t<12, 2, 8>(vl, s, g, ns); break;
+    if (v->res_f32) {
+        const VRows in = r.xres.rows(), out = u < 2 ? k.res[u + 1].xres.rows() : in;
+        g.xin = r.xres.p; g.xin_stride = r.xres.stride();
+        g.oin = in.p; g.oin_stride = in.stride; g.oin_off = in.off;
+        g.o = out.p; g.o_stride = out.stride; g.o_off = out.off;
+        launch_resunit_c<true>(vl, s, g, ns, C, v->exp_192_alone);
+    } else {
+        g.xin = r.c1_in.p; g.xin_stride = r.c1_in.stride();
+        g.oin = o; g.oin_stride = (size_t)T * C; g.oin_off = 0;
+        g.o = o; g.o_stride = (size_t)T * C; g.o_off = 0;
+        launch_resunit_c<false>(vl, s, g, ns, C, false);
     }
 }
 static void hist(hipStream_t s, const VCall& cl, const VCall* cld, VBuf& b, int T, int save) {
@@ -1481,20 +1539,67 @@
     if (b.bf16) hipLaunchKernelGGL((k_voc_hist<uint16_t>), grid, dim3(256), 0, s, cld, (uint16_t*)b.p, b.stride(), (uint16_t*)b.hist, b.H, b.C, T, save);
     else hipLaunchKernelGGL((k_voc_hist<float>), grid, dim3(256), 0, s, cld, b.p, b.stride(), b.hist, b.H, b.C, T, save);
 }
-static void hist_all(hipStream_t s, const VCall& cl, const VCall* cld, Q3Voc* v, int nf, int save) {
+enum VHistKind { VH_PRE, VH_UP, VH_DEC_IN, VH_CT, VH_C1, VH_XRES, VH_OUT };
+struct VHistPlanEnt { VHistKind kind; int a, u, H, C, es, rpf; bool with_save; };
+static std::vector<VHistPlanEnt> voc_hist_plan(const q3tts_vocoder_config& c, bool res_f32, bool no_fuse) {
+    std::vector<VHistPlanEnt> t;
+    const int d = c.latent_dim;
+    int rpf = 1;
+    t.push_back({VH_PRE, 0, 0, c.pre_conv_kernel - 1, c.codebook_dim, 4, rpf, true});
+    for (int s = 0; s < c.n_upsample; ++s) { rpf *= c.upsample_ratios[s]; t.push_back({VH_UP, s, 0, 6, d, 4, rpf, false}); }
+    t.push_back({VH_DEC_IN, 0, 0, 6, d, 2, rpf, true});
+    int ch = c.decoder_dim;
+    for (int b = 0; b < c.n_dec_blocks; ++b) {
+        t.push_back({VH_CT, b, 0, 1, ch, 2, rpf, true});
+        rpf *= c.dec_rates[b]; ch /= 2;
+        const bool f32 = res_f32 && !no_fuse && resunit_width(ch);
+        for (int u = 0; u < 3; ++u) t.push_back({f32 ? VH_XRES : VH_C1, b, u, 6 * VOC_RES_DIL[u], ch, f32 ? 4 : 2, rpf, true});
+    }
+    t.push_back({VH_OUT, 0, 0, 6, ch, 2, rpf, true});
+    t.erase(std::remove_if(t.begin(), t.end(), [](const VHistPlanEnt& p) { return p.H <= 0; }), t.end());
+    return t;
+}
+static const VBuf& voc_hist_buf(const Q3Voc* v, const VHistPlanEnt& p) {
+    switch (p.kind) {
+        case VH_PRE: return v->pre_in;
+        case VH_UP: return v->U[p.a].dw_in;
+        case VH_DEC_IN: return v->dec_in_in;
+        case VH_CT: return v->Bk[p.a].ct_in;
+        case VH_C1: return v->Bk[p.a].res[p.u].c1_in;
+        case VH_XRES: return v->Bk[p.a].res[p.u].xres;
+        default: return v->out_in;
+    }
+}
+static void hist_all(hipStream_t s, const VLaunch& vl, const VCall& cl, const VCall* cld, Q3Voc* v, int nf, int save) {
     VHistTab tab; tab.n = 0;
-    auto add = [&](const VBuf& b, int T, bool with_save) {
-        if (b.H == 0 || (save && !with_save) || tab.n >= 24) return;
-        const size_t es = b.bf16 ? 2 : 4;
-        tab.e[tab.n++] = {(char*)b.p, (char*)b.hist, (unsigned long long)(b.stride() * es), (unsigned long long)((size_t)b.H * b.C * es), (unsigned long long)((size_t)T * b.C * es)};
-    };
-    int T = nf;
-    add(v->pre_in, T, true);
-    for (auto& p : v->U) { T *= p.r; add(p.dw_in, T, false); }
-    add(v->dec_in_in, T, true);
-    for (auto& k : v->Bk) { add(k.ct_in, T, true); T *= k.r; for (auto& r : k.res) add(r.c1_in, T, true); }
-    add(v->out_in, T, true);
+    for (const VHistPlanEnt& p : voc_hist_plan(v->c, v->res_f32, vl.no_fuse)) {
+        if (save && !p.with_save) continue;
+        const VBuf& b = voc_hist_buf(v, p);
+        const size_t es = b.bf16 ? 2 : 4, T = (size_t)nf * p.rpf;
+        tab.e[tab.n++] = {(char*)b.p, (char*)b.hist, (unsigned long long)(b.stride() * es), (unsigned long long)((size_t)b.H * b.C * es), (unsigned long long)(T * b.C * es)};
+    }
     if (tab.n) hipLaunchKernelGGL(k_voc_hist_all, dim3(16, cl.ns, tab.n), dim3(256), 0, s, cld, tab, save);
+}
+extern "C" int q3tts_k_voc_hist_plan(const q3tts_vocoder_config* c, int32_t res_bf16, int32_t no_fuse, q3tts_voc_hist_ent* out, int32_t cap, int32_t* n) {
+    if (!c || !out || !n || c->n_upsample < 0 || c->n_upsample > Q3TTS_MAX_UPSAMPLE || c->n_dec_blocks < 0 || c->n_dec_blocks > Q3TTS_MAX_DEC_BLOCKS) return Q3TTS_ERR_INVALID;
+    const std::vector<VHistPlanEnt> t = voc_hist_plan(*c, !res_bf16, no_fuse != 0);
+    if ((int)t.size() > cap) return Q3TTS_ERR_INVALID;
+    for (size_t i = 0; i < t.size(); ++i) {
+        const VHistPlanEnt& p = t[i]; q3tts_voc_hist_ent& r = out[i];
+        memset(&r, 0, sizeof(r));
+        switch (p.kind) {
+            case VH_PRE: snprintf(r.name, sizeof(r.name), "pre.in"); break;
+            case VH_UP: snprintf(r.name, sizeof(r.name), "up%d.raw", p.a); break;
+            case VH_DEC_IN: snprintf(r.name, sizeof(r.name), "dec_in.in"); break;
+            case VH_CT: snprintf(r.name, sizeof(r.name), "b%d.ct_in", p.a); break;
+            case VH_C1: snprintf(r.name, sizeof(r.name), "b%d.r%d.c1_in", p.a, p.u); break;
+            case VH_XRES: snprintf(r.name, sizeof(r.name), "b%d.r%d.x", p.a, p.u); break;
+            default: snprintf(r.name, sizeof(r.name), "out.in"); break;
+        }
+        r.hist_rows = p.H; r.channels = p.C; r.elem_bytes = p.es; r.rows_per_frame = p.rpf; r.saved_at_end = p.with_save ? 1 : 0;
+    }
+    *n = (int32_t)t.size();
+    return Q3TTS_OK;
 }
 static void voc_launch_attn(const VLaunch& vl, hipStream_t s, const VCall* cld, Q3Voc* v, float* kr, float* vr, int ns, int nf, int tiled) {
     const q3tts_vocoder_config& c = v->c;
@@ -1605,15 +1710,20 @@
           VOpt().snake_to(snake_into(v->Bk[0].ct_in, v->Bk[0].ea, v->Bk[0].ib, ch)).no_store());
     for (size_t bi = 0; bi < v->Bk.size(); ++bi) {
         VBlk& k = v->Bk[bi]; const int b = (int)bi;
-        vgemm(vl, s, k.ct, k.ct_in.rows(), ns, T, VBuf::flat(o, T * k.r, k.cout), VEPI_STORE, VOpt().snake_to(snake_into(k.res[0].c1_in, k.res[0].ea, k.res[0].ib, k.cout)));
+        const bool chain = v->res_f32 && resunit_ok(vl, k.cout);
+        if (chain) vgemm(vl, s, k.ct, k.ct_in.rows(), ns, T, k.res[0].xres.rows());
+        else vgemm(vl, s, k.ct, k.ct_in.rows(), ns, T, VBuf::flat(o, T * k.r, k.cout), VEPI_STORE, VOpt().snake_to(snake_into(k.res[0].c1_in, k.res[0].ea, k.res[0].ib, k.cout)));
         T *= k.r; ch = k.cout;
-        vtap(v, s, o, VT_F32, T, ch, "b%d.o_ct", b);
+        vtap(v, s, chain ? k.res[0].xres.p + k.res[0].xres.rows().off : o, VT_F32, T, ch, "b%d.o_ct", b);
         for (int u = 0; u < 3; ++u) {
             VRes& r = k.res[u];
-            const VSnake next = snake_next(v, bi, u);
+            const VSnake next = (chain && u < 2) ? VSnake() : snake_next(v, bi, u);
             const int store_o = u < 2 ? 1 : 0;
-            if (resunit_ok(vl, ch)) launch_resunit(vl, s, r, ns, T, ch, o, store_o, next);
-            else {
+            if (resunit_ok(vl, ch)) {
+                launch_resunit(v, vl, s, k, u, ns, T, o, store_o, next);
+                if (store_o) vtap(v, s, chain ? k.res[u + 1].xres.p + k.res[u + 1].xres.rows().off : o, VT_F32, T, ch, "b%d.r%d.o", b, u);
+                continue;
+            } else {
                 const VRows zf = VBuf::flat(z, T, ch), zb = zf.as_bf16(), orows = VBuf::flat(o, T, ch);
                 vgemm(vl, s, r.c1, r.c1_in.rows(), ns, T, zf, VEPI_STORE, VOpt().snake_to({zb, r.ea2, r.ib2, ch}).no_store());
                 vtap(v, s, z, VT_BF16, T, ch, "b%d.r%d.z", b, u);
@@ -1641,7 +1751,7 @@
     Q3Voc* v = e->voc;
     const q3tts_vocoder_config& c = v->c;
     const int nf = cl.nf, d = c.latent_dim, M = cl.ns * nf;
-    hist_all(s, cl, v->call_dev, v, nf, 0);
+    hist_all(s, vl, cl, v->call_dev, v, nf, 0);
     voc_embed_pre(e, vl, cl, s);
     for (int l = 0; l < c.n_layer; ++l) VTRY(voc_tfm_layer(e, vl, cl, s, l));
     hipLaunchKernelGGL(k_voc_rmsnorm, dim3(M), dim3(64), 0, s, v->x, v->final_norm, c.rms_eps, d, v->up_bg ? v->xnb : v->xn, v->up_bg ? 2 : 0);
@@ -1661,12 +1771,19 @@
             VBlk& k = v->Bk[bi];
             vtap_buf(v, s, k.ct_in, Tb, "b%d.ct_in", (int)bi);
             Tb *= k.r;
-            for (int u = 0; u < 3; ++u) vtap_buf(v, s, k.res[u].c1_in, Tb, "b%d.r%d.c1_in", (int)bi, u);
+            for (int u = 0; u < 3; ++u) {
+                const VRes& r = k.res[u];
+                if (v->res_f32 && resunit_ok(vl, k.cout)) {
+                    const size_t n = (size_t)(r.xres.H + Tb) * k.cout;
+                    hipLaunchKernelGGL(k_voc_snake_bf16, dim3((unsigned)((n / 4 + 255) / 256)), dim3(256), 0, s, r.xres.p, (uint16_t*)r.c1_in.p, n, k.cout, r.ea, r.ib);
+                }
+                vtap_buf(v, s, r.c1_in, Tb, "b%d.r%d.c1_in", (int)bi, u);
+            }
         }
         vtap_buf(v, s, v->out_in, Tb, "out.in");
         vtap(v, s, v->pcm + (size_t)cl.slot[0] * v->pcm_stride + (size_t)cl.pos[0] * v->spf, VT_F32, Tb, 1, "pcm");
     }
-    hist_all(s, cl, v->call_dev, v, nf, 1);
+    hist_all(s, vl, cl, v->call_dev, v, nf, 1);
     Q3_HIP(e, hipGetLastError());
     return Q3TTS_OK;
 }
@@ -1786,6 +1903,41 @@
         return Q3TTS_OK;
     }));
     *n_samples_out = ns;
+    return Q3TTS_OK;
+}
+
+extern "C" int q3tts_k_vocoder_slots(q3tts_engine* e, const int32_t* codes, int32_t n_slots, int32_t max_frames, const int32_t* n_frames, int32_t chunk_frames,
+                                     int32_t beside_decoder, float* pcm_out) {
+    Q3_NOT_IN_SESSION(e);
+    if (!e || !codes || !n_frames || !pcm_out || n_slots <= 0 || max_frames <= 0) return q3_set_err(e, Q3TTS_ERR_INVALID, "null argument");
+    if (!e->voc) return q3_set_err(e, Q3TTS_ERR_STATE, "engine created with with_vocoder = 0");
+    if (n_slots > e->B || n_slots > VOC_MAX_NS || max_frames > e->cfg.max_steps_cap) return q3_set_err(e, Q3TTS_ERR_INVALID, "vocoder slots: shape exceeds the engine's");
+    for (int i = 0; i < n_slots; ++i) if (n_frames[i] <= 0 || n_frames[i] > max_frames) return q3_set_err(e, Q3TTS_ERR_INVALID, "vocoder slots: n_frames");
+    Q3_HIP(e, hipSetDevice(e->cfg.device));
+    hipStream_t s = e->stream;
+    const int ncb = e->cfg.model.n_codebooks, nf = chunk_frames > 0 ? std::min(chunk_frames, VOC_FCAP) : VOC_FCAP, spf = e->voc->spf;
+    for (int i = 0; i < n_slots; ++i) {
+        Q3_HIP(e, hipMemcpyAsync(e->codes + (size_t)i * e->cfg.max_steps_cap * ncb, codes + (size_t)i * max_frames * ncb, sizeof(int32_t) * (size_t)n_frames[i] * ncb, hipMemcpyHostToDevice, s));
+        VTRY(q3_voc_reset(e, i));
+    }
+    int rc = Q3TTS_OK;
+    for (;;) {
+        std::vector<int> slots, real;
+        for (int i = 0; i < n_slots; ++i) {
+            const int left = n_frames[i] - e->voc->frames_done[i];
+            if (left > 0) { slots.push_back(i); real.push_back(std::min(left, nf)); }
+        }
+        if (slots.empty()) break;
+        rc = q3_voc_decode_batch(e, slots.data(), real.data(), (int)slots.size(), nf, s, beside_decoder);
+        if (rc != Q3TTS_OK) break;
+    }
+    for (int i = 0; i < n_slots && rc == Q3TTS_OK; ++i) {
+        q3_voc_mark_last(e, i);
+        if (hipMemcpyAsync(pcm_out + (size_t)i * max_frames * spf, q3_voc_pcm(e, i), sizeof(float) * (size_t)n_frames[i] * spf, hipMemcpyDeviceToHost, s) != hipSuccess) rc = q3_set_err(e, Q3TTS_ERR_DEVICE, "vocoder slots: copy");
+    }
+    const hipError_t er = hipStreamSynchronize(s);
+    if (rc < 0) return rc;
+    Q3_HIP(e, er);
     return Q3TTS_OK;
 }
 
diff --git a/qwen3-tts-rust_amd/q3tts/_abi.py b/qwen3-tts-rust_amd/q3tts/_abi.py
--- a/qwen3-tts-rust_amd/q3tts/_abi.py
+++ b/qwen3-tts-rust_amd/q3tts/_abi.py
@@ -100,6 +100,13 @@
     ]
 
 
+class VocHistEnt(C.Structure):
+    _fields_ = [
+        ("name", C.c_char * 32), ("hist_rows", C.c_int32), ("channels", C.c_int32), ("elem_bytes", C.c_int32), ("rows_per_frame", C.c_int32),
+        ("saved_at_end", C.c_int32), ("reserved", C.c_int32),
+    ]
+
+
 class VocTap(C.Structure):
     _fields_ = [
         ("name", C.c_char * 32), ("dtype", C.c_int32), ("layout", C.c_int32), ("hist_rows", C.c_int32), ("rows", C.c_int32),
@@ -153,7 +160,7 @@
     "q3tts_set_max_steps", "q3tts_build_prompt", "q3tts_free", "q3tts_generate", "q3tts_generate_batch",
     "q3tts_result_free", "q3tts_stream_begin", "q3tts_stream_poll", "q3tts_stream_end",
     "q3tts_get_timings", "q3tts_k_gemm_exact", "q3tts_k_attention", "q3tts_k_attention_decode", "q3tts_k_sample", "q3tts_k_talker_prefill",
-    "q3tts_k_vocoder", "q3tts_k_vocoder_latent", "q3tts_k_vocoder_taps", "q3tts_k_vocoder_bench", "q3tts_set_device_pcm", "q3tts_get_device_pcm", "q3tts_k_rng_f32", "q3tts_k_probe", "q3tts_k_gguf_read", "q3tts_mel_frames", "q3tts_mel",
+    "q3tts_k_vocoder", "q3tts_k_vocoder_latent", "q3tts_k_vocoder_taps", "q3tts_k_voc_hist_plan", "q3tts_k_vocoder_slots", "q3tts_k_vocoder_bench", "q3tts_set_device_pcm", "q3tts_get_device_pcm", "q3tts_k_rng_f32", "q3tts_k_probe", "q3tts_k_gguf_read", "q3tts_mel_frames", "q3tts_mel",
     "q3tts_clone_default_config", "q3tts_clone_init", "q3tts_clone_audio_frames", "q3tts_clone_audio_encode",
     "q3tts_clone_speaker_encode", "q3tts_k_speaker_from_mel", "q3tts_k_audio_latent",
     "q3tts_node_create", "q3tts_node_destroy", "q3tts_node_generate_batch", "q3tts_node_get_timings", "q3tts_node_last_error", "q3tts_node_size", "q3tts_node_engine", "q3tts_node_shard", "q3tts_k_bgemm_q8", "q3tts_k_bgemm_q8a8_argmax", "q3tts_k_bgemm_q8a8", "q3tts_k_alloc_upload", "q3tts_k_bgemm_policy", "q3tts_k_attend_policy", "q3tts_k_bgemm_pick", "q3tts_k_mfma_bf16", "q3tts_k_bgemm", "q3tts_k_bgemm_voc", "q3tts_k_project", "q3tts_k_norm_inputs", "q3tts_tokenizer_load", "q3tts_tokenizer_free", "q3tts_tokenizer_vocab_size", "q3tts_tokenizer_encode", "q3tts_tokenizer_decode",
@@ -352,6 +359,8 @@
     lib.q3tts_k_vocoder.argtypes = [vp, i32p, C.c_int32, C.c_int32, f32p, i32p]
     lib.q3tts_k_vocoder_latent.argtypes = [vp, i32p, C.c_int32, C.c_int32, f32p]
     lib.q3tts_k_vocoder_taps.argtypes = [vp, i32p, C.c_int32, C.c_int32, C.c_int32, C.c_void_p, C.c_uint64, C.POINTER(VocTap), C.c_int32, i32p]
+    lib.q3tts_k_vocoder_slots.argtypes = [vp, i32p, C.c_int32, C.c_int32, i32p, C.c_int32, C.c_int32, f32p]
+    lib.q3tts_k_voc_hist_plan.argtypes = [C.POINTER(VocoderConfig), C.c_int32, C.c_int32, C.POINTER(VocHistEnt), C.c_int32, i32p]
     lib.q3tts_k_vocoder_bench.argtypes = [vp, C.c_int32, C.c_int32, f32p]
     lib.q3tts_set_device_pcm.argtypes = [vp, C.c_int32]
     lib.q3tts_get_device_pcm.argtypes = [vp, C.POINTER(f32p), C.POINTER(C.c_int64), i32p]
diff --git a/qwen3-tts-rust_amd/q3tts/native.py b/qwen3-tts-rust_amd/q3tts/native.py
--- a/qwen3-tts-rust_amd/q3tts/native.py
+++ b/qwen3-tts-rust_amd/q3tts/native.py
@@ -414,6 +414,17 @@
                     "q3tts_k_vocoder")
         return pcm[:ns.value].copy()
 
+    def vocoder_slots(self, codes, n_frames, chunk_frames=0, beside_decoder=False):
+        c = np.ascontiguousarray(codes, dtype=np.int32)
+        nfr = np.ascontiguousarray(n_frames, dtype=np.int32)
+        assert c.ndim == 3 and c.shape[0] == nfr.size and c.shape[2] == self.cfg.model.n_codebooks
+        v = self.cfg.vocoder
+        spf = int(np.prod([v.upsample_ratios[i] for i in range(v.n_upsample)]) * np.prod([v.dec_rates[i] for i in range(v.n_dec_blocks)]))
+        pcm = np.zeros((c.shape[0], c.shape[1] * spf), dtype=np.float32)
+        self._check(self.lib.q3tts_k_vocoder_slots(self.h, _ptr(c, i32p), c.shape[0], c.shape[1], _ptr(nfr, i32p), chunk_frames, int(bool(beside_decoder)),
+                                                   _ptr(pcm, f32p)), "q3tts_k_vocoder_slots")
+        return [pcm[i, :int(nfr[i]) * spf].copy() for i in range(c.shape[0])]
+
     def vocoder_latent(self, codes, chunk_frames=0):
         c = np.ascontiguousarray(codes, dtype=np.int32)
         out = np.zeros((c.shape[0], self.cfg.vocoder.latent_dim), dtype=np.float32)
@@ -1116,6 +1127,17 @@
     return out.reshape(shape), int(ty.value)
 
 
+def k_voc_hist_plan(vocoder_cfg, res_bf16=False, no_fuse=False):
+    lib = _abi.load_library()
+    ents = (_abi.VocHistEnt * 64)()
+    n = C.c_int32(0)
+    rc = lib.q3tts_k_voc_hist_plan(C.byref(vocoder_cfg), int(bool(res_bf16)), int(bool(no_fuse)), ents, 64, C.byref(n))
+    if rc != 0:
+        raise _abi.Q3Error(f"q3tts_k_voc_hist_plan: status {rc}")
+    return [dict(name=e.name.decode(), hist_rows=e.hist_rows, channels=e.channels, elem_bytes=e.elem_bytes, rows_per_frame=e.rows_per_frame,
+                 saved_at_end=bool(e.saved_at_end)) for e in ents[:n.value]]
+
+
 GGUF_VALUE_TYPES = ("u8", "i8", "u16", "i16", "u32", "i32", "f32", "bool", "str", "array", "u64", "i64", "f64")
 
 
```
